# wangxiaohit/GNNPN-SC

Measured on AMD Instinct MI355X. Metric: service-composition problems/sec (ML+2PN inference), higher is better.
Workload: dtype f32-split3xf16 (f32 operands and results; recurrent W_hh.h products: fp32 operands split exactly into 3 x f16, six f16-matrix-core products per term, f32 accumulate; everything else f32 arithmetic)

## Files before the change

### gnnpn-sc_amd/_lib.py

```python
import ctypes
import os
from ctypes import c_char_p, c_double, c_float, c_int, c_int32, c_int64, c_uint32, c_void_p

import torch

_HERE = os.path.dirname(os.path.abspath(__file__))
LIB_PATH = os.environ.get("GNNPN_LIB") or os.path.join(_HERE, "libgnnpn_hip.so")
ABI_VERSION = 9

ACT_NONE, ACT_RELU, ACT_SIGMOID = 0, 1, 2
E_UNSUP = -2
WOA_OK, WOA_ROWS_MISMATCH, WOA_INDEX_ERROR, WOA_NO_SLOTS = 0, 1, 2, 3

_P = c_void_p
_SIGNATURES = {
    "gnnpn_abi_version": (c_int, []),
    "gnnpn_last_error": (c_char_p, []),
    "gnnpn_linear_f32": (c_int, [_P, c_int64, _P, c_int64, _P, _P, _P, c_int, _P, c_int64, c_int64, c_int, c_int, _P]),
    "gnnpn_embed_concat_f32": (c_int, [_P, _P, c_int, c_int, c_int, _P, c_int64, _P]),
    "gnnpn_csr_aggregate_f32": (c_int, [_P, _P, _P, _P, c_int64, _P, _P, _P, _P, c_int, _P, c_int64, c_int32,
                                        c_int32, _P]),
    "gnnpn_csr_aggregate_blocks_f32": (c_int, [_P, _P, _P, _P, c_int64, _P, _P, _P, _P, c_int, _P, c_int64, c_int32,
                                               c_int32, c_int32, _P, _P]),
    "gnnpn_csr_block_row_order": (c_int, [_P, c_int32, c_int32, _P, _P]),
    "gnnpn_csr_tile_plan_geometry": (c_int, [c_int32, c_int32, _P]),
    "gnnpn_csr_tile_plan_rows": (c_int, [_P, _P, _P, c_int32, c_int32, _P, _P, _P, _P, _P, _P]),
    "gnnpn_csr_tile_plan_fill": (c_int, [_P, _P, c_int32, c_int32, _P, _P, _P, _P, c_int64, _P]),
    "gnnpn_csr_aggregate_tiled_f32": (c_int, [_P, _P, _P, _P, _P, c_int64, _P, _P, _P, _P, c_int, _P, c_int64, c_int32, c_int32,
                                              c_int32, _P]),
    "gnnpn_gcn_norm_f32": (c_int, [_P, _P, _P, _P, _P, c_int32, _P]),
    "gnnpn_segment_mean_f32": (c_int, [_P, _P, c_int64, _P, c_int64, c_int32, c_int32, _P]),
    "gnnpn_gin_layer_f32": (c_int, [_P, _P, _P, c_int64, c_int32, _P, _P, _P, _P, _P, c_int32, _P, _P, _P, _P, c_int32, _P, _P, c_int32,
                                    _P, c_int64, c_int64, _P]),
    "gnnpn_split_weights_bytes": (c_int64, [c_int32, c_int32]),
    "gnnpn_lstm_split_weights_bytes": (c_int64, []),
    "gnnpn_lstm_pack_split_weights_f32": (c_int, [_P, _P, _P]),
    "gnnpn_pack_split_weights_f16": (c_int, [_P, c_int64, c_int32, c_int32, _P, _P, _P]),
    "gnnpn_gin_layer_split": (c_int, [_P, _P, _P, c_int64, c_int32, _P, _P, _P, _P, _P, _P, c_int32, _P, _P, _P, _P, _P, c_int32,
                                      _P, _P, _P, c_int32, _P, c_int64, c_int64, _P]),
    "gnnpn_request_branch_f32": (c_int, [_P, c_int32, _P, c_int32, c_int32, _P, _P, _P, c_int32, c_int32, c_int32, _P, c_int32,
                                         _P, _P, _P, _P]),
    "gnnpn_select_candidates": (c_int, [_P, c_int64, _P, _P, _P, _P, _P, _P, _P, c_int32, c_int32, c_int32, _P]),
    "gnnpn_rank_rows": (c_int, [_P, c_int64, _P, c_int32, c_int32, _P]),
    "gnnpn_precision_at_k": (c_int, [_P, c_int64, _P, c_int64, c_int32, c_int32, _P, c_int32, _P, _P]),
    "gnnpn_lstm_encode_f32": (c_int, [c_int, _P, c_int32, c_int32, c_int32, c_int32, c_int32, _P, _P, c_int64, _P]),
    "gnnpn_lstm_encode_workspace_bytes": (c_int64, []),
    "gnnpn_set_option": (c_int, [c_char_p, c_int]),
    "gnnpn_decode_diag": (c_int, [_P, c_int32, c_int32]),
    "gnnpn_coop_reset_staffing": (c_int, []),
    "gnnpn_last_launch_units": (c_int64, []),
    "gnnpn_lds_footprint_kb": (c_int, [c_int]),
    "gnnpn_coop_staffing_count": (c_int, []),
    "gnnpn_bn_train_forward_f32": (c_int, [_P, c_int64, c_int32, _P, _P, c_float, c_float, c_int, _P, _P, _P, _P, _P, _P]),
    "gnnpn_bn_train_backward_f32": (c_int, [_P, _P, _P, _P, _P, c_int64, c_int32, c_int, _P, _P, _P, _P]),
    "gnnpn_bce_sigmoid_f32": (c_int, [_P, _P, c_int64, _P, _P, _P]),
    "gnnpn_dot_f32": (c_int, [_P, _P, c_int64, _P, _P]),
    "gnnpn_embed_grad_f32": (c_int, [_P, c_int64, _P, c_int64, c_int64, c_int32, c_int32, _P, _P]),
    "gnnpn_pointer_decode_f32": (c_int, [c_int, _P, _P, c_float, c_int, c_int32, c_int32, c_int32, c_int32, c_int32,
                                         _P, _P, c_int64, _P]),
    "gnnpn_pointer_decode_workspace_bytes": (c_int64, [c_int32, c_int32, c_int32]),
    "gnnpn_pointer_decode_replicas_f32": (c_int, [_P, _P, c_float, c_int, c_int32, c_int32, c_int32, ctypes.c_uint64, c_int32, c_int32,
                                                  c_int32, _P, _P, c_int64, _P]),
    "gnnpn_replica_seed": (ctypes.c_uint64, [ctypes.c_uint64, c_int32]),
    "gnnpn_best_of_select_f32": (c_int, [c_int32, c_int32, c_int32, _P, _P, _P, _P, _P, _P, _P, _P, _P, _P, _P, _P, _P, _P]),
    "gnnpn_pointer_decode_attn_f32": (c_int, [_P, _P, _P, c_float, c_int, c_int32, c_int32, c_int32, c_int32, _P]),
    "gnnpn_attention_logits_f32": (c_int, [_P, _P, c_int64, _P, c_float, c_int, _P, c_int32, c_int32, c_int32,
                                           c_int32, c_int32, _P]),
    "gnnpn_attention_logits_bahdanau_f32": (c_int, [_P, _P, c_int64, _P, _P, c_float, c_int, _P, c_int32, c_int32, c_int32, c_int32, c_int32, _P]),
    "gnnpn_qos_reward_f32": (c_int, [_P, _P, c_int32, c_int32, c_int, _P]),
    "gnnpn_split3_pieces_f32": (c_int, [_P, c_int64, c_int32, _P, _P, _P, _P]),
    "gnnpn_recurrent_product_f32": (c_int, [_P, _P, c_int32, _P, _P, _P]),
    "gnnpn_gemm_f32": (c_int, [_P, c_int64, c_int, _P, c_int64, c_int, _P, c_int64, c_int64, c_int, c_int, c_int, _P]),
    "gnnpn_colsum_chunks_f32": (c_int, [_P, c_int64, c_int64, c_int32, c_int64, _P, _P]),
    "gnnpn_lstm_train_forward_f32": (c_int, [_P, _P, _P, _P, _P, _P, c_int32, c_int32, c_int32, _P]),
    "gnnpn_decode_train_forward_f32": (c_int, [_P, c_int32, c_int32, c_int32, c_int32, c_float, c_int, _P]),
    "gnnpn_decode_train_backward_f32": (c_int, [_P, _P, _P, _P, _P, _P, _P, c_int32, c_int32, c_int32, c_int32, c_float, c_int, _P]),
    "gnnpn_lstm_train_backward_f32": (c_int, [_P, _P, _P, _P, _P, _P, _P, c_int32, c_int32, c_int32, _P]),
    "gnnpn_decode_attn_train_forward_f32": (c_int, [_P, c_int32, c_int32, c_int32, c_int32, c_float, c_int, _P]),
    "gnnpn_decode_attn_train_backward_f32": (c_int, [_P, _P, _P, _P, _P, _P, _P, c_int32, c_int32, c_int32, c_int32, c_float, c_int, _P]),
    "gnnpn_colsum_f32": (c_int, [_P, c_int64, c_int64, c_int32, _P, _P]),
    "gnnpn_scatter_dx_f32": (c_int, [_P, _P, _P, c_int32, c_int32, c_int32, c_int32, _P]),
    "gnnpn_sumsq_f32": (c_int, [_P, c_int64, _P, _P]),
    "gnnpn_adam_step_f32": (c_int, [_P, _P, _P, _P, c_int64, _P, c_float, c_float, c_float, c_float, c_float, c_int32, _P]),
    "gnnpn_eswoa_f64": (c_int, [c_int32, c_int32, _P, _P, _P, _P, _P, c_int32, c_int32, _P, c_int32, _P, _P, _P, _P, _P]),
    "gnnpn_eswoa_wide_workspace_bytes": (c_int64, [c_int32, c_int32, c_int32]),
    "gnnpn_eswoa_wide_f64": (c_int, [c_int32, c_int32, _P, _P, _P, _P, _P, c_int32, c_int32, _P, _P, c_int64, _P, _P, _P, _P, _P]),
    "gnnpn_eswoa_ragged_workspace_bytes": (c_int64, [c_int32, c_int32, c_int32, c_int32]),
    "gnnpn_eswoa_ragged_f64": (c_int, [c_int32, _P, c_int32, c_int32, c_int32, _P, _P, _P, _P, _P, c_int32, c_int32, _P, c_int32, _P,
                                       c_int64, _P, _P, _P, _P, _P, _P]),
    "gnnpn_woa_candidates_workspace_bytes": (c_int64, [c_int32, c_int32, c_int32]),
    "gnnpn_woa_candidates_count": (c_int, [c_int32, c_int32, _P, c_int32, _P, _P, _P, c_int32, _P, _P, _P, c_int32, c_int32, c_double,
                                           _P, c_int32, c_int32, _P, c_int64, _P, _P, _P, _P, _P, _P]),
    "gnnpn_woa_candidates_fill": (c_int, [c_int32, c_int32, _P, _P, _P, c_int32, _P, c_int64, _P, _P, c_int32, c_int32, _P, _P, _P, _P,
                                          _P]),
    "gnnpn_debug_round5_f64": (c_int, [_P, _P, c_int64, _P]),
    "gnnpn_debug_cell_activations": (c_int, [_P, _P, _P, c_int64, _P]),
    "gnnpn_debug_lds_interferer": (c_int, [c_int32, c_int32, c_int32, _P]),
    "gnnpn_gate_wait": (c_int, [_P, c_uint32, c_int32, _P]),
    "gnnpn_debug_mfma_f16": (c_int, [_P, _P, _P, _P, _P]),
}
EXPORTS = tuple(_SIGNATURES)

class DecodeNet(ctypes.Structure):
    _fields_ = [(n, _P) for n in ("embedded", "enc_out", "h0", "c0", "start", "wih_packed", "whh_packed", "bih",
                                  "bhh", "latent_win", "emb_w", "emb_b", "xw_fold", "xb_fold", "start_fold", "idx", "win_logits", "pick_prob", "actions",
                                  "queries")] + \
               [("latent_from", c_int32), ("sample", c_int32), ("sample_seed", ctypes.c_uint64), ("whh_split", _P)]


class Attention(ctypes.Structure):
    _fields_ = [("attention", c_int32), ("n_glimpses", c_int32)] + \
               [(n, _P) for n in ("pointer_wq", "pointer_bq", "pointer_ref", "pointer_v", "glimpse_wq", "glimpse_bq",
                                  "glimpse_ref", "glimpse_v")]


class LaunchOpts(ctypes.Structure):
    _fields_ = [("impl", c_int32), ("lds_kb", c_int32), ("write_through", c_int32), ("paired_start", c_int32),
                ("sticky_status", _P)]


class TilePlanGeom(ctypes.Structure):
    _fields_ = [(n, c_int32) for n in ("n_blocks", "src_tiles", "src_tile_rows", "dst_tiles", "dst_tile_rows", "units", "wavefronts",
# ... 104 lines not shown
```

### gnnpn-sc_amd/build.py

```python
import os
import subprocess
import sys
from concurrent.futures import ThreadPoolExecutor

HERE = os.path.dirname(os.path.abspath(__file__))
ROOT = os.path.dirname(HERE)
CSRC = os.path.join(HERE, "csrc")
LIB = os.path.join(HERE, "libgnnpn_hip.so")
SOURCES = ["api.hip", "dense.hip", "graph.hip", "graph_tiled.hip", "gin_layer.hip", "gin_layer_split.hip", "request_branch.hip", "select.hip", "lstm.hip", "lstm_coop.hip", "decode.hip", "decode_coop.hip", "decode_lean.hip", "train.hip", "train_attn.hip", "train_ml.hip", "decode_glimpse.hip", "woa.hip", "woa_prep.hip", "split_probe.hip"]
HEADERS = [os.path.join(CSRC, "common.h"), os.path.join(CSRC, "graph_lds.h"), os.path.join(CSRC, "recurrent.h"), os.path.join(CSRC, "lstm_shared.h"), os.path.join(CSRC, "decode_shared.h"), os.path.join(CSRC, "coop_common.h"), os.path.join(CSRC, "train_common.h"),
           os.path.join(ROOT, "include", "gnnpn_hip.h")]
FLAGS = ["-O3", "--offload-arch=gfx950", "-ffp-contract=off", "-fPIC", "-std=c++17",
         "-I" + os.path.join(ROOT, "include"), "-I" + CSRC] + os.environ.get("GNNPN_EXTRA_HIPCC_FLAGS", "").split()


def _stale(target, deps):
    if not os.path.exists(target):
        return True
    t = os.path.getmtime(target)
    return any(os.path.getmtime(d) > t for d in deps)


def _compile(src):
    obj = os.path.join(HERE, "build", src.replace(".hip", ".o"))
    path = os.path.join(CSRC, src)
    if _stale(obj, [path] + HEADERS):
        subprocess.run(["hipcc"] + FLAGS + ["-c", path, "-o", obj], check=True)
    return obj


def _check_compiler():
    try:
        out = subprocess.run(["hipcc", "--version"], capture_output=True, text=True, check=True).stdout
    except (OSError, subprocess.CalledProcessError):
        return
    with open(os.path.join(HERE, "build", "compiler.txt"), "w") as f:
        f.write(out)


def build(force=False):
    os.makedirs(os.path.join(HERE, "build"), exist_ok=True)
    _check_compiler()
    if force:
        for f in os.listdir(os.path.join(HERE, "build")):
            if os.path.isfile(os.path.join(HERE, "build", f)):
                os.remove(os.path.join(HERE, "build", f))
    with ThreadPoolExecutor(max_workers=4) as ex:
        objs = list(ex.map(_compile, SOURCES))
    if force or _stale(LIB, objs):
        subprocess.run(["hipcc", "--offload-arch=gfx950", "-shared", "-fPIC", "-o", LIB] + objs, check=True)
    build_torch_ops(force)
    return LIB


TORCH_LIB = os.path.join(HERE, "libgnnpn_torch.so")


def build_torch_ops(force=False):
    src = os.path.join(CSRC, "torch_ops.cpp")
    if not (force or _stale(TORCH_LIB, [src, os.path.join(ROOT, "include", "gnnpn_hip.h"), LIB])):
        return TORCH_LIB
    import torch
    from torch.utils import cpp_extension
# ... 14 lines not shown
```

### gnnpn-sc_amd/csrc/decode.hip

```cpp
#include <atomic>

#include "common.h"
#include <string.h>
#include "recurrent.h"
#include "decode_shared.h"
#include "lstm_shared.h"

template <int H, int BT, bool REP = false>
__global__ __launch_bounds__((H < 64 ? 64 : H)) void pointer_decode_kernel(
    const float* __restrict__ embedded, const float* __restrict__ enc_out, const float* __restrict__ h0,
    const float* __restrict__ c0, const float* __restrict__ start, const float* __restrict__ wih,
    const float* __restrict__ whh, const float* __restrict__ bih, const float* __restrict__ bhh,
    const float* __restrict__ latent_win, const float* __restrict__ inputs, float tanh_c, int use_tanh,
    int32_t* __restrict__ idx_out, float* __restrict__ win_logits, float* __restrict__ pick_prob,
    float* __restrict__ actions, float* __restrict__ queries, int32_t B, int32_t T, int32_t n_per, int sample,
    unsigned long long sample_seed, int rep_R, int rep_first) {
    constexpr int NT = H < 64 ? 64 : H;
    constexpr int NW = NT / 64;
    __shared__ __attribute__((aligned(16))) float xs[BT][H];
    __shared__ __attribute__((aligned(16))) float hs[2][BT][H];
    __shared__ float lg[BT][64];
    __shared__ int sel[BT];

    const int j = threadIdx.x;
    const bool owner = j < H;
    const int lane = j & 63, wave = j >> 6;
    const int b0 = blockIdx.x * BT;
    const int L = T * n_per;
    const float4* __restrict__ Wi = reinterpret_cast<const float4*>(wih);
    const float4* __restrict__ Wh = reinterpret_cast<const float4*>(whh);
    auto prob_of = [rep_R](int b) { return REP ? b / rep_R : b; };

    float bi[4], bh[4], c[BT], h[BT];
#pragma unroll
    for (int g = 0; g < 4; ++g) {
        bi[g] = owner ? bih[g * H + j] : 0.0f;
        bh[g] = owner ? bhh[g * H + j] : 0.0f;
    }
#pragma unroll
    for (int p = 0; p < BT; ++p) {
        const bool ok = owner && (b0 + p < B);
        c[p] = ok ? c0[(int64_t)prob_of(b0 + p) * H + j] : 0.0f;
        h[p] = ok ? h0[(int64_t)prob_of(b0 + p) * H + j] : 0.0f;
        if (owner) {
            hs[0][p][j] = h[p];
            xs[p][j] = start[j];
        }
    }
    __syncthreads();

    int cur = 0;
    for (int k = 0; k < T; ++k) {
        if (owner) {
            float ai[BT][4], ah[BT][4];
#pragma unroll
            for (int p = 0; p < BT; ++p)
#pragma unroll
                for (int g = 0; g < 4; ++g) ai[p][g] = ah[p][g] = 0.0f;
// ... 38 lines not shown
        __syncthreads();

#pragma unroll
        for (int p = 0; p < BT; ++p) {
            if (b0 + p < B) {
                const int64_t row = (int64_t)prob_of(b0 + p) * L + sel[p];
                if (owner) xs[p][j] = embedded[row * H + j];
                if (j < 8) actions[((int64_t)(b0 + p) * T + k) * 8 + j] = inputs[row * 8 + j];
            }
        }
        __syncthreads();
    }
}

template <int H, bool REP = false>
static void launch_decode(const DecodeArgs& args, const DecodeNet& d, const float* latent, hipStream_t s,
                          ReplicaMap rep = ReplicaMap{0, 0}) {
    constexpr int NT = H < 64 ? 64 : H;
    const int32_t B = args.B;
    int bt = 1;
    while (bt < 4 && B / (bt * 2) >= 256) bt *= 2;
    dim3 grid((B + bt - 1) / bt), block(NT);
#define GNNPN_LAUNCH_DEC(BT_)                                                                                                    \
    hipLaunchKernelGGL((pointer_decode_kernel<H, BT_, REP>), grid, block, 0, s, d.embedded, d.enc_out, d.h0, d.c0, d.start, d.wih, \
                       d.whh, d.bih, d.bhh, latent, args.inputs, args.tanh_c, args.use_tanh, d.idx, d.win_logits, d.pick_prob,   \
                       d.actions, d.queries, B, args.T, args.K, d.sample, (unsigned long long)d.sample_seed, rep.R, rep.first)
    switch (bt) {
        case 1: GNNPN_LAUNCH_DEC(1); break;
        case 2: GNNPN_LAUNCH_DEC(2); break;
        default: GNNPN_LAUNCH_DEC(4); break;
    }
#undef GNNPN_LAUNCH_DEC
}

extern "C" int gnnpn_pointer_decode_f32(int n_nets, const gnnpn_decode_net_t* nets, const float* inputs,
                                        float tanh_c, int use_tanh, int32_t B, int32_t T, int32_t n_per, int32_t H,
                                        int32_t precision, const gnnpn_launch_opts_t* opts_in, void* workspace,
                                        int64_t workspace_bytes, void* stream) {
    g_gnnpn_last_units = 0;
    GNNPN_REQUIRE(B >= 0 && T > 0, "pointer_decode: bad shape");
    if (B == 0) return GNNPN_OK;
    GNNPN_REQUIRE(nets && inputs, "pointer_decode: null input");
    const CoopOpts opts = coop_opts(opts_in);
    GNNPN_REQUIRE(opts.impl >= 0 && opts.impl <= 4 && opts.impl != 3, "pointer_decode: opts.impl must be 0 (auto), 1 (streaming), 2 (cooperative, 8-CU groups) or 4 (8-CU groups, 256-register build) — the 16-CU-group form (3) was removed in ABI version 7");
    GNNPN_REQUIRE(opts.lds_kb >= 0 && opts.lds_kb <= 160, "pointer_decode: opts.lds_kb must be 0..160");
    GNNPN_REQUIRE(precision == GNNPN_PREC_F32 || precision == GNNPN_PREC_SPLIT, "pointer_decode: precision must be GNNPN_PREC_F32 or GNNPN_PREC_SPLIT, got %d", precision);
    GNNPN_REQUIRE(n_nets >= 1 && n_nets <= GNNPN_MAX_DECODE_NETS, "pointer_decode: n_nets must be 1..%d",
                  GNNPN_MAX_DECODE_NETS);
    GNNPN_REQUIRE(n_per >= 1 && n_per <= 64, "pointer_decode: n_per must be in [1,64], got %d", n_per);
    if (H != 256 && H != 32) GNNPN_FAIL(GNNPN_E_UNSUP, "pointer_decode: hidden size %d not built (256, 32)", H);
    DecodeArgs args{};
    for (int n = 0; n < n_nets; ++n) {
        const gnnpn_decode_net_t& d = nets[n];
        if (const int rc = decode_net_check(d, "pointer_decode", n)) return rc;
        GNNPN_REQUIRE(d.embedded || (d.emb_w && d.emb_b) || d.xw_fold,
                      "pointer_decode: net %d needs embedded, (emb_w, emb_b) or the folded input side", n);
        GNNPN_REQUIRE(d.latent_from < n && d.latent_from >= -1, "pointer_decode: latent_from of net %d must name an "
                      "earlier net of the call", n);
        GNNPN_REQUIRE(!(d.latent_win && d.latent_from >= 0), "pointer_decode: net %d has two latent sources", n);
        GNNPN_REQUIRE(!d.whh_split || gnnpn_aligned(d.whh_split, 16), "pointer_decode: whh_split must be 16-byte aligned");
        static_assert(sizeof(DecodeNet) == sizeof(gnnpn_decode_net_t), "layout");
        memcpy(&args.net[n], &d, sizeof(DecodeNet));
    }
    args.inputs = inputs;
    args.tanh_c = tanh_c;
    args.use_tanh = use_tanh;
    args.B = B;
    args.T = T;
    args.K = n_per;
    hipStream_t s = (hipStream_t)stream;
    bool any_sample = false;
    for (int n = 0; n < n_nets; ++n) any_sample |= nets[n].sample != 0;
    if (any_sample && (precision != GNNPN_PREC_F32 || opts.impl > 2))
        GNNPN_FAIL(GNNPN_E_UNSUP, "pointer_decode: sampling is built in the streaming and the 8-CU-group fp32 forms (impl 0-2, "
                   "GNNPN_PREC_F32)");
    const int impl = opts.impl;
    if (impl != 1 && gnnpn_decode_coop_supported(H, n_per) && (workspace != nullptr || impl >= 2)) {
        const int rc = gnnpn_launch_decode_coop(args, n_nets, precision, impl == 4, opts, workspace, workspace_bytes, s);
        const bool fall_through = rc == GNNPN_E_UNSUP && impl == 0 && precision == GNNPN_PREC_F32;
        if (rc != GNNPN_OK && !fall_through) return rc;
        if (fall_through) {
            static std::atomic<bool> said{false};
            if (!said.exchange(true))
                fprintf(stderr, "[gnnpn] pointer_decode: %s — taking the per-workgroup streaming form (about 10 x slower per step)\n", gnnpn_last_error());
        }
        if (rc == GNNPN_OK) {
            GNNPN_CHECK_LAUNCH("pointer_decode_f32(coop)");
            return GNNPN_OK;
        }
    }
    if (precision == GNNPN_PREC_SPLIT)
        GNNPN_FAIL(GNNPN_E_UNSUP, "pointer_decode: the split-operand precision needs the cooperative form (H = 256)");
    for (int n = 0; n < n_nets; ++n) {
        const DecodeNet& d = args.net[n];
        if (!d.embedded) GNNPN_FAIL(GNNPN_E_UNSUP, "pointer_decode: the streaming form needs the embedded tensor");
        const float* latent = d.latent_from >= 0 ? args.net[d.latent_from].win_logits : d.latent_win;
        GNNPN_FOR_H(H, launch_decode<HH>(args, d, latent, s));
    }
    GNNPN_CHECK_LAUNCH("pointer_decode_f32");
    return GNNPN_OK;
}

extern "C" uint64_t gnnpn_replica_seed(uint64_t seed, int32_t replica) {
    return replica_seed(seed, (unsigned long long)(long long)replica);
}

extern "C" int gnnpn_pointer_decode_replicas_f32(const gnnpn_decode_net_t* net, const float* inputs, float tanh_c, int use_tanh,
                                                 int32_t B, int32_t R, int32_t first, uint64_t seed, int32_t T, int32_t n_per,
                                                 int32_t H, const gnnpn_launch_opts_t* opts_in, void* workspace,
                                                 int64_t workspace_bytes, void* stream) {
    g_gnnpn_last_units = 0;
    GNNPN_REQUIRE(R >= 1, "pointer_decode_replicas: R must be >= 1, got %d", R);
    GNNPN_REQUIRE(first >= 0, "pointer_decode_replicas: first replica must be >= 0, got %d", first);
    GNNPN_REQUIRE(B >= 0 && T > 0 && n_per >= 1 && n_per <= 64, "pointer_decode_replicas: bad shape (B %d, T %d, n_per %d)", B, T, n_per);
    const int64_t rows = (int64_t)B * R;
    GNNPN_REQUIRE(rows <= (1 << 30), "pointer_decode_replicas: B*R = %lld rows exceed 2^30", (long long)rows);
    if (H != 256 && H != 32) GNNPN_FAIL(GNNPN_E_UNSUP, "pointer_decode_replicas: hidden size %d not built (256, 32)", H);
    if (B == 0) return GNNPN_OK;
    GNNPN_REQUIRE(net && inputs, "pointer_decode_replicas: null input");
    const CoopOpts opts = coop_opts(opts_in);
    GNNPN_REQUIRE(opts.impl >= 0 && opts.impl <= 2, "pointer_decode_replicas: opts.impl must be 0 (auto), 1 (streaming) or 2 (cooperative)");
    GNNPN_REQUIRE(opts.lds_kb >= 0 && opts.lds_kb <= 160, "pointer_decode_replicas: opts.lds_kb must be 0..160");
    const gnnpn_decode_net_t& d = *net;
    if (const int rc = decode_net_check(d, "pointer_decode_replicas", 0)) return rc;
    GNNPN_REQUIRE(d.embedded || d.xw_fold, "pointer_decode_replicas: the net needs embedded or the folded input side");
    GNNPN_REQUIRE(!d.queries, "pointer_decode_replicas: queries are not written (must be NULL)");
    GNNPN_REQUIRE(d.latent_from == -1, "pointer_decode_replicas: latent_from must be -1 (Low's window logits come from latent_win)");
    DecodeArgs args{};
    memcpy(&args.net[0], &d, sizeof(DecodeNet));
    args.net[0].sample = 1;
    args.net[0].sample_seed = seed;
    args.net[0].whh_split = nullptr;
// ... 62 lines not shown
    if (use_tanh) u = __fmul_rn(tanh_c, tanhf(u));
    if (lane == 0) logits[row] = u;
}

__global__ void mask_logits_kernel(const int32_t* __restrict__ masked_idx, float* __restrict__ logits, int32_t B,
                                   int32_t L, int32_t n_masked, int32_t ld_idx) {
    const int i = blockIdx.x * blockDim.x + threadIdx.x;
    if (i >= B * n_masked) return;
    const int b = i / n_masked, m = i - b * n_masked;
    const int pos = masked_idx[(int64_t)b * ld_idx + m];
    if (pos >= 0 && pos < L) logits[(int64_t)b * L + pos] = -INFINITY;
}

extern "C" int gnnpn_attention_logits_f32(const float* enc_out, const float* queries, int64_t ld_q,
                                          const int32_t* masked_idx, float tanh_c, int use_tanh, float* logits,
                                          int32_t B, int32_t L, int32_t H, int32_t n_masked, int32_t ld_idx,
                                          void* stream) {
    GNNPN_REQUIRE(B >= 0 && L > 0 && H > 0 && H % 4 == 0 && ld_q >= H && ld_q % 4 == 0, "attention_logits: bad shape");
    if (B == 0) return GNNPN_OK;
    GNNPN_REQUIRE(enc_out && queries && logits, "attention_logits: null operand");
    GNNPN_REQUIRE(n_masked == 0 || (masked_idx && ld_idx >= n_masked), "attention_logits: bad mask list");
    GNNPN_REQUIRE(gnnpn_aligned(enc_out, 16) && gnnpn_aligned(queries, 16), "attention_logits: 16-byte alignment");
    if (B == 0) return GNNPN_OK;
    hipStream_t s = (hipStream_t)stream;
    const int64_t n_rows = (int64_t)B * L;
    hipLaunchKernelGGL(attention_logits_kernel, dim3((unsigned)((n_rows + 3) / 4)), dim3(256), 0, s, enc_out, queries,
                       ld_q, tanh_c, use_tanh, logits, n_rows, L, H);
    if (n_masked > 0)
        hipLaunchKernelGGL(mask_logits_kernel, dim3((B * n_masked + 255) / 256), dim3(256), 0, s, masked_idx, logits,
                           B, L, n_masked, ld_idx);
    GNNPN_CHECK_LAUNCH("attention_logits_f32");
    return GNNPN_OK;
}

extern "C" int gnnpn_attention_logits_bahdanau_f32(const float* ref, const float* qp, int64_t ld_q, const float* v,
                                                   const int32_t* masked_idx, float tanh_c, int use_tanh, float* logits, int32_t B,
                                                   int32_t L, int32_t H, int32_t n_masked, int32_t ld_idx, void* stream) {
    GNNPN_REQUIRE(ref && qp && v && logits && B >= 0 && L > 0 && H > 0 && ld_q >= H, "attention_logits_bahdanau: bad argument");
    GNNPN_REQUIRE(n_masked == 0 || (masked_idx && ld_idx >= n_masked), "attention_logits_bahdanau: bad mask");
    if (B == 0) return GNNPN_OK;
    hipStream_t s = (hipStream_t)stream;
    const int64_t n_rows = (int64_t)B * L;
    hipLaunchKernelGGL(attention_logits_bahdanau_kernel, dim3((unsigned)((n_rows + 3) / 4)), dim3(256), 0, s, ref, qp, ld_q, v,
                       tanh_c, use_tanh, logits, n_rows, L, H);
    if (n_masked > 0)
        hipLaunchKernelGGL(mask_logits_kernel, dim3((B * n_masked + 255) / 256), dim3(256), 0, s, masked_idx, logits, B, L,
                           n_masked, ld_idx);
    GNNPN_CHECK_LAUNCH("attention_logits_bahdanau_f32");
    return GNNPN_OK;
}

__global__ __launch_bounds__(256) void qos_reward_kernel(const float* __restrict__ actions, float* __restrict__ R, int32_t B,
                                                        int32_t T, int level) {
    const int lane = threadIdx.x & 63;
    const int b = blockIdx.x * 4 + (threadIdx.x >> 6);
    if (b >= B) return;
    const float* a = actions + (int64_t)b * T * 8;
    const float lo0 = a[4], hi0 = a[5], lo1 = a[6], hi1 = a[7];
    float prod2 = 1.0f, prod3 = 1.0f, mn = INFINITY;
    double sum0 = 0.0;
    int n_real = 0;
    auto fetch = [&](int t) { return *reinterpret_cast<const float4*>(a + (int64_t)min(t, T - 1) * 8); };
    auto consume = [&](float4 q, int t0) {
        if (t0 + lane >= T) q = make_float4(0.0f, INFINITY, 1.0f, 1.0f);
        n_real += q.x > 0.0f;
        mn = fminf(mn, q.y);
        const double xd = (double)q.x;
        const int lo = __double2loint(xd), hi = __double2hiint(xd);
        const int zi = __float_as_int(q.z), wi = __float_as_int(q.w);
        const int cnt = min(64, T - t0);
#define GNNPN_REWARD_STEP(i)                                                                                      \
    prod2 = __fmul_rn(prod2, __int_as_float(__builtin_amdgcn_readlane(zi, i)));                                   \
    prod3 = __fmul_rn(prod3, __int_as_float(__builtin_amdgcn_readlane(wi, i)));                                   \
    sum0 += __hiloint2double(__builtin_amdgcn_readlane(hi, i), __builtin_amdgcn_readlane(lo, i));
        if (cnt == 64) {
#pragma unroll
            for (int i = 0; i < 64; ++i) { GNNPN_REWARD_STEP(i) }
        } else {
            for (int i = 0; i < cnt; ++i) { GNNPN_REWARD_STEP(i) }
        }
#undef GNNPN_REWARD_STEP
    };
    float4 qa = fetch(lane), qb;
    for (int t0 = 0; t0 < T; t0 += 128) {
        qb = fetch(t0 + 64 + lane);
        consume(qa, t0);
        if (t0 + 64 >= T) break;
        qa = fetch(t0 + 128 + lane);
        consume(qb, t0 + 64);
    }
#pragma unroll
    for (int off = 32; off > 0; off >>= 1) {
        n_real += __shfl_xor(n_real, off, 64);
        mn = fminf(mn, __shfl_xor(mn, off, 64));
    }
    if (lane != 0) return;
    int violate = 0;
    if (prod2 < lo0 || prod2 > hi0) ++violate;
    if (prod3 < lo1 || prod3 > hi1) ++violate;
    if (level == 0) {
        R[b] = (float)violate;
        return;
    }
    float obj = (float)sum0 / (float)n_real;
    obj = __fadd_rn(obj, 1.0f);
    obj = __fsub_rn(obj, mn);
    obj = obj / 2.0f;
    const double v = (double)violate + (double)obj;
    R[b] = (float)(rint(v * 1e5) / 1e5);
}

extern "C" int gnnpn_qos_reward_f32(const float* actions, float* R, int32_t B, int32_t T, int level,
                                    void* stream) {
    GNNPN_REQUIRE(B >= 0 && T > 0 && (level == 0 || level == 1), "qos_reward: bad argument");
    if (B == 0) return GNNPN_OK;
    GNNPN_REQUIRE(actions && R, "qos_reward: null operand");
    hipLaunchKernelGGL(qos_reward_kernel, dim3((B + 3) / 4), dim3(256), 0, (hipStream_t)stream, actions, R, B, T,
                       level);
    GNNPN_CHECK_LAUNCH("qos_reward_f32");
    return GNNPN_OK;
}

__global__ __launch_bounds__(256) void best_of_select_kernel(int32_t B, int32_t N, int32_t T, const float* __restrict__ R0,
                                                             const int32_t* __restrict__ idx0, const float* __restrict__ act0,
                                                             const float* __restrict__ prob0, const float* __restrict__ Rs,
                                                             const int32_t* __restrict__ idxs, const float* __restrict__ acts,
                                                             const float* __restrict__ probs, float* __restrict__ R_out,
                                                             int32_t* __restrict__ idx_out, float* __restrict__ act_out,
                                                             float* __restrict__ prob_out, int32_t* __restrict__ winner) {
    const int lane = threadIdx.x & 63;
    const int b = blockIdx.x * 4 + (threadIdx.x >> 6);
    if (b >= B) return;
    const int S = N - 1;
    unsigned long long best = ~0ull;
    for (int j = lane; j < N; j += 64) {
        float r = j == 0 ? R0[b] : Rs[(int64_t)b * S + (j - 1)];
        if (r == 0.0f) r = 0.0f;
        const unsigned hi = r != r ? 0xFFFFFFFFu : float_order_key(r);
        const unsigned long long key = ((unsigned long long)hi << 32) | (unsigned)j;
        best = key < best ? key : best;
    }
#pragma unroll
    for (int off = 32; off > 0; off >>= 1) {
        const unsigned lo = __shfl_xor((unsigned)(best & 0xffffffffu), off, 64);
        const unsigned hi = __shfl_xor((unsigned)(best >> 32), off, 64);
        const unsigned long long o = ((unsigned long long)hi << 32) | lo;
        best = o < best ? o : best;
    }
    const int w = (int)(best & 0xffffffffu);
    const int64_t src = w == 0 ? (int64_t)b : (int64_t)b * S + (w - 1);
    const int32_t* si = (w == 0 ? idx0 : idxs) + src * T;
    const float* sp = (w == 0 ? prob0 : probs) + src * T;
    const float* sa = (w == 0 ? act0 : acts) + src * T * 8;
    for (int t = lane; t < T; t += 64) {
        idx_out[(int64_t)b * T + t] = si[t];
        prob_out[(int64_t)b * T + t] = sp[t];
    }
    for (int i = lane; i < T * 8; i += 64) act_out[(int64_t)b * T * 8 + i] = sa[i];
    if (lane == 0) {
        winner[b] = w;
        R_out[b] = w == 0 ? R0[b] : Rs[src];
    }
// ... 17 lines not shown
```

### gnnpn-sc_amd/csrc/decode_lean.hip

```cpp
#include "common.h"
#include "recurrent.h"
#include "decode_shared.h"
#include "coop_common.h"
#include "lstm_shared.h"

namespace {
constexpr int H = COOP_H;
constexpr int G = COOP_G;
constexpr int ROWS = COOP_ROWS;
constexpr int UNITS = H / G;
constexpr int KW = 16;
constexpr unsigned SPIN_LIMIT = 400000;
constexpr int XP_GRANULES = ROWS * KW * G;

typedef unsigned u32x2 __attribute__((ext_vector_type(2)));
constexpr int AUX_SC1 = 16;


__device__ __forceinline__ __amdgpu_buffer_rsrc_t make_rsrc(const void* p, unsigned bytes) {
    return __builtin_amdgcn_make_buffer_rsrc(const_cast<void*>(p), 0, (int)bytes, 0x00020000);
}
__device__ __forceinline__ float dpp_ror(float v, int n) {
    switch (n) {
        case 1: return __int_as_float(__builtin_amdgcn_update_dpp(0, __float_as_int(v), 0x121, 0xF, 0xF, true));
        case 2: return __int_as_float(__builtin_amdgcn_update_dpp(0, __float_as_int(v), 0x122, 0xF, 0xF, true));
        case 4: return __int_as_float(__builtin_amdgcn_update_dpp(0, __float_as_int(v), 0x124, 0xF, 0xF, true));
        default: return __int_as_float(__builtin_amdgcn_update_dpp(0, __float_as_int(v), 0x128, 0xF, 0xF, true));
    }
}
__device__ __forceinline__ void store_granule(__amdgpu_buffer_rsrc_t r, unsigned voff, unsigned soff, u64 g, bool same_xcd) {
    const u32x2 v = {(unsigned)g, (unsigned)(g >> 32)};
    if (same_xcd) __builtin_amdgcn_raw_buffer_store_b64(v, r, voff, soff, 0);
    else __builtin_amdgcn_raw_buffer_store_b64(v, r, voff, soff, AUX_SC1);
}
__device__ __forceinline__ void record_failure(unsigned* diag, const unsigned* err, int group, int member, int tile, int k, int wave,
                                               unsigned tag, unsigned h_miss, unsigned p_miss, unsigned l_miss, int gpx) {
    if ((threadIdx.x & 63) != 0 || !diag) return;
    const unsigned n = atomicAdd(diag, 1u);
    if (n >= 31) return;
    unsigned* rec = diag + 16 * (n + 1);
    const unsigned* cnt = err + COOP_XCDCNT_OFFSET / 4;
    unsigned c0 = 0, c1 = 0;
    for (int x = 0; x < 4; ++x) {
        c0 |= (cnt[COOP_XCD_STRIDE * x] & 0xffu) << (8 * x);
        c1 |= (cnt[COOP_XCD_STRIDE * (4 + x)] & 0xffu) << (8 * x);
    }
    const unsigned long long t = __builtin_amdgcn_s_memrealtime();
    rec[0] = group; rec[1] = member; rec[2] = tile; rec[3] = k; rec[4] = wave; rec[5] = tag;
    rec[6] = h_miss; rec[7] = p_miss; rec[8] = l_miss; rec[9] = c0; rec[10] = c1;
    rec[11] = (unsigned)t; rec[12] = (unsigned)(t >> 32); rec[13] = gpx; rec[14] = blockIdx.x; rec[15] = err[0];
}
}

template <bool SPLIT, int OCC, int EVH, bool DIAG = false>
__global__ __launch_bounds__(256, OCC) void pointer_decode_lean_kernel(DecodeArgs a, u64* xh, u64* xp,
// ... 328 lines not shown
                    __builtin_amdgcn_raw_buffer_store_b32(__float_as_uint(hl.x), r_q, vo_q, (unsigned)k * (H * 4), 0);
                    __builtin_amdgcn_raw_buffer_store_b32(__float_as_uint(hl.y), r_q, vo_q, (unsigned)(k + T) * (H * 4), 0);
                }
            }
            if constexpr (DIAG) {
                asm volatile("" ::"v"(hl.y));
                st[6] = phase_stamp();
            }
            __syncthreads();
            {
                float p = 0.0f;
                if (pdot) {
#pragma unroll
                    for (int j = 0; j < EVN; ++j) {
                        const float4 hv = *reinterpret_cast<const float4*>(&hsl[prow][phalf * (4 * EVN) + 4 * j]);
                        p = fmaf(__uint_as_float(ev[j].x), hv.x, p);
                        p = fmaf(__uint_as_float(ev[j].y), hv.y, p);
                        p = fmaf(__uint_as_float(ev[j].z), hv.z, p);
                        p = fmaf(__uint_as_float(ev[j].w), hv.w, p);
                    }
                }
                if constexpr (EVH == 2)
                    p = __fadd_rn(p, __int_as_float(__builtin_amdgcn_update_dpp(0, __float_as_int(p), 0xB1 , 0xF, 0xF, false)));
                if (pdot && phalf == 0)
                    store_granule(r_p, vo_ppub, (step & 1) * (XP_GRANULES * 8), ((u64)(step + 1) << 32) | __float_as_uint(p), same_xcd);
            }
            if (wr_live) {
                *reinterpret_cast<u32x4*>(&win[wr_row][wr_cand][0]) = wv0;
                *reinterpret_cast<u32x4*>(&win[wr_row][wr_cand][4]) = wv1;
            }
            if constexpr (DIAG) {
                st[7] = phase_stamp();
                if (blockIdx.x == 0 && tid == 0 && k > 0) {
                    u64* prof = reinterpret_cast<u64*>(err) + 4;
                    prof[0] += st[1] - st[0];
                    prof[1] += st[2] - st[1];
                    prof[2] += st[3] - st[2];
                    prof[3] += st[4] - st[3];
                    prof[4] += st[5] - st[4];
                    prof[5] += st[6] - st[5];
                    prof[6] += st[7] - st[6];
                    prof[7] += 1;
                }
            }
            ++step;
        }
        if (abort_flag) break;
        ++tiles_done;
    }
    if (tid == 0) {
        if (abort_flag) coop_raise(err, sticky, 2u, seats);
        coop_note_finished(sticky, GNNPN_STATUS_DEC_FINISHED, tiles_done);
    }
}

struct PickProbArgs {
    const float* win[2];
    const float* lat[2];
    const int32_t* idx[2];
    float* out[2];
};
__global__ __launch_bounds__(256) void pick_prob_kernel(PickProbArgs a, int64_t rows, int T, int K) {
    const int net = blockIdx.y;
    const float* __restrict__ win = a.win[net];
    const float* __restrict__ lat = a.lat[net];
    const int32_t* __restrict__ idx = a.idx[net];
    float* __restrict__ out = a.out[net];
    const int64_t row = blockIdx.x * 256ll + threadIdx.x;
    if (row >= rows) return;
    const unsigned t_base = (unsigned)__builtin_amdgcn_readfirstlane((int)((blockIdx.x * 256ll) % T));
    const int t = (int)((t_base + threadIdx.x) % (unsigned)T);
    float v[16];
#pragma unroll
    for (int j = 0; j < 16; ++j) {
        v[j] = 0.0f;
        if (j < K) {
            v[j] = win[row * K + j];
            if (lat) v[j] = __fadd_rn(v[j], lat[row * K + j]);
        }
    }
    const int pick_r = min(max(idx[row] - t * K, 0), 15);
    float best = v[0];
#pragma unroll
    for (int j = 1; j < 16; ++j) best = j == pick_r ? v[j] : best;
#pragma unroll
    for (int j = 0; j < 16; ++j) v[j] = j < K ? expf(__fsub_rn(v[j], best)) : 0.0f;
#pragma unroll
    for (int n = 8; n >= 1; n >>= 1)
#pragma unroll
        for (int j = 0; j < n; ++j) v[j] = __fadd_rn(v[j], v[j + n]);
    out[row] = 1.0f / v[0];
}

static DecodeWorkspace lean_workspace(int64_t groups, int64_t rows, int32_t T, int32_t K) {
    return decode_workspace(groups, rows, T, K, XP_GRANULES);
}

int64_t gnnpn_decode_lean_workspace_bytes(int32_t B, int32_t T, int32_t n_per) { return lean_workspace(64, B, T, n_per).total(); }

int gnnpn_launch_decode_lean(const DecodeArgs& args, int n_nets, int precision, bool shared_cu, const CoopOpts& opts,
                             void* workspace, int64_t workspace_bytes, hipStream_t s) {
    if (args.K > KW) GNNPN_FAIL(GNNPN_E_UNSUP, "pointer_decode: the cooperative form is built for n_per <= %d", KW);
    if ((int64_t)ROWS * args.T * args.K * H * 4 >= (1ll << 32) || (int64_t)args.T * ROWS * args.K * 8 >= (1ll << 32))
        GNNPN_FAIL(GNNPN_E_UNSUP, "pointer_decode: a tile of 16 problems must stay below 4 GB of encoder output");
    const bool split = precision == GNNPN_PREC_SPLIT;
    const bool wide = args.K > 8;
    const bool stamps = (gnnpn_option_lstm_ablate() & 0x800) != 0;
    if (stamps && wide) GNNPN_FAIL(GNNPN_E_UNSUP, "pointer_decode: the stamped build exists for n_per <= 8");
    CoopLaunch c;
    const auto need = [&](int groups) { return lean_workspace(groups, args.B, args.T, args.K).total(); };
    if (const int rc = coop_begin("pointer_decode", n_nets, args.B, need, GNNPN_STATUS_DEC_EXPECTED, opts, workspace, workspace_bytes, s, c))
        return rc;
    const DecodeWorkspace w = lean_workspace(c.groups, args.B, args.T, args.K);
    u64* p_h = reinterpret_cast<u64*>(c.buffers);
    u64* p_p = reinterpret_cast<u64*>(c.buffers + w.h_bytes);
    u64* p_l = reinterpret_cast<u64*>(c.buffers + w.h_bytes + w.p_bytes);
    static unsigned* p_diag = gnnpn_decode_diag_buffer();
    const int wt = (opts.write_through ? 1 : 0) | (opts.paired_start ? 2 : 0);
#define GNNPN_LEAN(SPLIT_, OCC_, EVH_, ...)                                                                                           \
    hipLaunchKernelGGL((pointer_decode_lean_kernel<SPLIT_, OCC_, EVH_, ##__VA_ARGS__>), dim3(COOP_OVERSUB * c.groups * G), dim3(256),       \
                       gnnpn_lds_padding((const void*)pointer_decode_lean_kernel<SPLIT_, OCC_, EVH_, ##__VA_ARGS__>, opts.lds_kb), s, args, \
                       p_h, p_p, p_l, c.status, opts.sticky, n_nets, c.groups_per_net, c.gpx, wt, c.seats, p_diag)
    if (stamps) {
        if (split) GNNPN_LEAN(true, 1, 2, true);
        else GNNPN_LEAN(false, 1, 2, true);
    } else if (split && shared_cu && wide) GNNPN_LEAN(true, 2, 1);
    else if (split && shared_cu) GNNPN_LEAN(true, 2, 2);
    else if (split && wide) GNNPN_LEAN(true, 1, 1);
    else if (split) GNNPN_LEAN(true, 1, 2);
    else if (shared_cu && wide) GNNPN_LEAN(false, 2, 1);
    else if (shared_cu) GNNPN_LEAN(false, 2, 2);
    else if (wide) GNNPN_LEAN(false, 1, 1);
    else GNNPN_LEAN(false, 1, 2);
#undef GNNPN_LEAN
    if (hipGetLastError() != hipSuccess) GNNPN_FAIL(GNNPN_E_LAUNCH, "pointer_decode: launch of the cooperative kernel failed");
    const int64_t rows = (int64_t)args.B * args.T;
    for (int n0 = 0; n0 < n_nets; n0 += 2) {
        PickProbArgs pa = {};
        const int cnt = n_nets - n0 < 2 ? n_nets - n0 : 2;
        for (int n = 0; n < cnt; ++n) {
            const DecodeNet& d = args.net[n0 + n];
            pa.win[n] = d.win_logits;
            pa.lat[n] = d.latent_from >= 0 ? args.net[d.latent_from].win_logits : d.latent_win;
            pa.idx[n] = d.idx;
            pa.out[n] = d.pick_prob;
        }
        hipLaunchKernelGGL(pick_prob_kernel, dim3((unsigned)((rows + 255) / 256), (unsigned)cnt), dim3(256), 0, s, pa, rows, args.T, args.K);
    }
    return GNNPN_OK;
}
```

### gnnpn-sc_amd/csrc/decode_shared.h

```cpp
#pragma once
#include "common.h"
#include "lstm_shared.h"

struct DecodeNet {
    const float* embedded;
    const float* enc_out;
    const float* h0;
    const float* c0;
    const float* start;
    const float* wih;
    const float* whh;
    const float* bih;
    const float* bhh;
    const float* latent_win;
    const float* emb_w;
    const float* emb_b;
    const float* xw_fold;
    const float* xb_fold;
    const float* start_fold;
    int32_t* idx;
    float* win_logits;
    float* pick_prob;
    float* actions;
    float* queries;
    int32_t latent_from;
    int32_t sample;
    uint64_t sample_seed;
    const void* whh_split;
};
static_assert(sizeof(DecodeNet) == sizeof(gnnpn_decode_net_t), "DecodeNet must mirror gnnpn_decode_net_t");

inline int decode_net_check(const gnnpn_decode_net_t& d, const char* who, int n) {
    GNNPN_REQUIRE(d.enc_out && d.h0 && d.c0 && d.start && d.wih_packed && d.whh_packed && d.bih && d.bhh,
                  "%s: null input of net %d (enc_out, h0, c0, start and the decoder weights are required)", who, n);
    GNNPN_REQUIRE(d.idx && d.win_logits && d.pick_prob && d.actions, "%s: null output of net %d", who, n);
    GNNPN_REQUIRE((d.xw_fold != nullptr) == (d.xb_fold != nullptr) && (d.xw_fold != nullptr) == (d.start_fold != nullptr),
                  "%s: net %d: xw_fold, xb_fold and start_fold go together", who, n);
    GNNPN_REQUIRE(d.sample == 0 || d.sample == 1, "%s: net %d: sample must be 0 (greedy) or 1 (multinomial)", who, n);
    GNNPN_REQUIRE(gnnpn_aligned(d.wih_packed, 16) && gnnpn_aligned(d.whh_packed, 16) && gnnpn_aligned(d.enc_out, 16) &&
                      (!d.embedded || gnnpn_aligned(d.embedded, 16)),
                  "%s: weights / enc_out / embedded must be 16-byte aligned", who);
    return GNNPN_OK;
}

template <int H>
__device__ __forceinline__ float lane_dot4(const float* __restrict__ row, const float* q) {
    float part = 0.0f;
    for (int e = (threadIdx.x & 63) * 4; e < H; e += 256) {
        const float4 rv = *reinterpret_cast<const float4*>(row + e);
        const float4 qv = *reinterpret_cast<const float4*>(q + e);
        part = fmaf(rv.x, qv.x, part);
        part = fmaf(rv.y, qv.y, part);
        part = fmaf(rv.z, qv.z, part);
        part = fmaf(rv.w, qv.w, part);
    }
    return part;
}

__device__ __forceinline__ int window_pick(float* lg, int K, float tanh_c, int use_tanh, float* __restrict__ win_logits, int64_t wbase,
                                           const float* __restrict__ latent_win, int64_t lbase, int sample, unsigned long long seed,
                                           unsigned long long ctr, float& prob) {
    float best = 0.0f;
    int best_r = -1;
    for (int r = 0; r < K; ++r) {
        float v = lg[r];
        if (use_tanh) v = __fmul_rn(tanh_c, tanhf(v));
        win_logits[wbase + r] = v;
        if (latent_win) v = __fadd_rn(v, latent_win[lbase + r]);
        lg[r] = v;
        if (best_r < 0 || v > best) {
            best = v;
            best_r = r;
        }
    }
    float denom = 0.0f;
    for (int r = 0; r < K; ++r) denom = __fadd_rn(denom, expf(__fsub_rn(lg[r], best)));
    prob = 1.0f / denom;
    if (sample) {
        const float u = stream_uniform24(seed, ctr);
        float cdf = 0.0f;
        int pick = -1, last_pos = 0;
        for (int r = 0; r < K; ++r) {
            const float pr = expf(__fsub_rn(lg[r], best)) / denom;
            cdf = __fadd_rn(cdf, pr);
            if (pr > 0.0f) last_pos = r;
            if (pick < 0 && u < cdf) pick = r;
        }
        if (pick < 0) pick = last_pos;
// ... 30 lines not shown
```

### gnnpn-sc_amd/csrc/dense.hip

```cpp
#include "common.h"

typedef float f32x16 __attribute__((ext_vector_type(16)));

template <int BM, int BN>
struct DenseCfg {
    static constexpr int BK = 32;
    static constexpr int LDA = BM + 1;
    static constexpr int LDB = BN + 1;
    static constexpr int A_F4 = BM * BK / 4 / 256;
    static constexpr int B_F4 = BN * BK / 4 / 256;
    static constexpr int TM = BM / 64;
    static constexpr int TN = BN / 64;
};

struct __attribute__((packed, aligned(4))) f4_align4 { float v[4]; };

template <int NF4>
__device__ __forceinline__ void tile_load(const float* __restrict__ P, int64_t ld, int64_t r0,
                                          int64_t n_rows, int k0, int K, bool vec_ok, float4 (&reg)[NF4]) {
#pragma unroll
    for (int i = 0; i < NF4; ++i) {
        int f = threadIdx.x + i * 256;
        int r = f >> 3, kc = f & 7;
        int64_t row = r0 + r;
        int k = k0 + kc * 4;
        float4 v = make_float4(0.f, 0.f, 0.f, 0.f);
        if (row < n_rows) {
            const float* src = P + row * ld + k;
            if (vec_ok && k + 3 < K) {
                const f4_align4 t = *reinterpret_cast<const f4_align4*>(src);
                v = make_float4(t.v[0], t.v[1], t.v[2], t.v[3]);
            } else {
                if (k + 0 < K) v.x = src[0];
                if (k + 1 < K) v.y = src[1];
                if (k + 2 < K) v.z = src[2];
                if (k + 3 < K) v.w = src[3];
            }
        }
        reg[i] = v;
    }
}

template <int NF4, int LD>
__device__ __forceinline__ void tile_store(float* S, const float4 (&reg)[NF4]) {
#pragma unroll
    for (int i = 0; i < NF4; ++i) {
        int f = threadIdx.x + i * 256;
        int r = f >> 3, kc = f & 7;
        S[(kc * 4 + 0) * LD + r] = reg[i].x;
        S[(kc * 4 + 1) * LD + r] = reg[i].y;
        S[(kc * 4 + 2) * LD + r] = reg[i].z;
        S[(kc * 4 + 3) * LD + r] = reg[i].w;
    }
}

template <int BM, int BN>
__global__ __launch_bounds__(256) void linear_f32_kernel(
    const float* __restrict__ A, int64_t lda, const float* __restrict__ W, int64_t ldw,
    const float* __restrict__ bias, const float* __restrict__ scale, const float* __restrict__ shift,
    int act, float* __restrict__ C, int64_t ldc, int64_t M, int N, int K, int vec_a, int vec_w) {
    using Cfg = DenseCfg<BM, BN>;
    __shared__ float As[Cfg::BK * Cfg::LDA];
    __shared__ float Bs[Cfg::BK * Cfg::LDB];

    const int wave = threadIdx.x >> 6, lane = threadIdx.x & 63;
    const int wm = wave >> 1, wn = wave & 1;
    const int64_t m0 = (int64_t)blockIdx.y * BM;
    const int n0 = blockIdx.x * BN;

    f32x16 acc[Cfg::TM][Cfg::TN];
#pragma unroll
    for (int i = 0; i < Cfg::TM; ++i)
#pragma unroll
        for (int j = 0; j < Cfg::TN; ++j)
#pragma unroll
            for (int r = 0; r < 16; ++r) acc[i][j][r] = 0.0f;

    float4 ra[Cfg::A_F4], rb[Cfg::B_F4];
    tile_load<Cfg::A_F4>(A, lda, m0, M, 0, K, vec_a, ra);
    tile_load<Cfg::B_F4>(W, ldw, n0, N, 0, K, vec_w, rb);

    const int half = lane >> 5, l32 = lane & 31;
    for (int k0 = 0; k0 < K; k0 += Cfg::BK) {
        tile_store<Cfg::A_F4, Cfg::LDA>(As, ra);
        tile_store<Cfg::B_F4, Cfg::LDB>(Bs, rb);
        __syncthreads();
        if (k0 + Cfg::BK < K) {
            tile_load<Cfg::A_F4>(A, lda, m0, M, k0 + Cfg::BK, K, vec_a, ra);
            tile_load<Cfg::B_F4>(W, ldw, n0, N, k0 + Cfg::BK, K, vec_w, rb);
        }
#pragma unroll
        for (int kk = 0; kk < Cfg::BK; kk += 2) {
            float a[Cfg::TM], b[Cfg::TN];
#pragma unroll
            for (int i = 0; i < Cfg::TM; ++i)
                a[i] = As[(kk + half) * Cfg::LDA + wm * (BM / 2) + i * 32 + l32];
#pragma unroll
            for (int j = 0; j < Cfg::TN; ++j)
                b[j] = Bs[(kk + half) * Cfg::LDB + wn * (BN / 2) + j * 32 + l32];
#pragma unroll
            for (int i = 0; i < Cfg::TM; ++i)
#pragma unroll
                for (int j = 0; j < Cfg::TN; ++j)
                    acc[i][j] = __builtin_amdgcn_mfma_f32_32x32x2f32(a[i], b[j], acc[i][j], 0, 0, 0);
        }
        __syncthreads();
    }
// ... 165 lines not shown
```

### gnnpn-sc_amd/csrc/select.hip

```cpp
#include <vector>

#include "common.h"

__device__ __forceinline__ unsigned long long rank_key(float score, uint32_t id) {
    return ((unsigned long long)float_order_key(score) << 32) | (0xffffffffu - id);
}

__global__ __launch_bounds__(256) void select_candidates_kernel(
    const float* __restrict__ scores, int64_t ld_scores, const int32_t* __restrict__ cat_ptr,
    const double* __restrict__ qos, const double* __restrict__ local_bounds, const uint8_t* __restrict__ present,
    const double* __restrict__ global_bounds, float* __restrict__ out_rows, int32_t* __restrict__ out_ids,
    int32_t B, int32_t T, int32_t n_per) {
    const int lane = threadIdx.x & 63;
    const int64_t seg = (int64_t)blockIdx.x * 4 + (threadIdx.x >> 6);
    if (seg >= (int64_t)B * T) return;
    const int b = (int)(seg / T), c = (int)(seg - (int64_t)b * T);
    const int s_begin = cat_ptr[c], s_end = cat_ptr[c + 1];
    const bool pres = present[seg] != 0;
    const double* lb = local_bounds + seg * 4;
    const double lo_c = lb[0], hi_c = lb[1], lo_q = lb[2], hi_q = lb[3];
    const float* srow = scores + (int64_t)b * ld_scores;

    unsigned long long last = ~0ull;
    int my_pick = -1;
    int n_found = 0;
    if (pres) {
        for (int r = 0; r < n_per; ++r) {
            unsigned long long best = 0ull;
            for (int s = s_begin + lane; s < s_end; s += 64) {
                const double cost = qos[(int64_t)s * 4 + 2], qual = qos[(int64_t)s * 4 + 3];
                const bool feas = lo_c <= cost && cost <= hi_c && lo_q <= qual && qual <= hi_q;
                const unsigned long long key = rank_key(srow[s], (uint32_t)s);
                if (feas && key < last && key > best) best = key;
            }
            best = wave_max_u64(best);
            if (best == 0ull) break;
            if (lane == r) my_pick = (int)(0xffffffffu - (uint32_t)(best & 0xffffffffu));
            last = best;
            ++n_found;
        }
    }
    const int src_lane = n_found > 0 ? lane % n_found : 0;
    const int id = __shfl(my_pick, src_lane, 64);
    if (lane < n_per) {
        const int64_t pos = (int64_t)b * T * n_per + (int64_t)c * n_per + lane;
        float4 q, tail = make_float4(0.f, 0.f, 0.f, 0.f);
        if (n_found > 0) {
            const double* qs = qos + (int64_t)id * 4;
            q = make_float4((float)qs[0], (float)qs[1], (float)qs[2], (float)qs[3]);
        } else {
            q = make_float4(0.f, 1.f, 1.f, 1.f);
        }
        if (c == 0) {
            const double* g = global_bounds + (int64_t)b * 4;
            tail = make_float4((float)g[0], (float)g[1], (float)g[2], (float)g[3]);
        }
        float4* dst = reinterpret_cast<float4*>(out_rows + pos * 8);
        dst[0] = q;
        dst[1] = tail;
        out_ids[pos] = n_found > 0 ? id : -1;
    }
}

__device__ __forceinline__ unsigned long long row16_max_u64(unsigned long long v) {
#define GNNPN_MAX_STEP(CTRL)                                                                                       \
    {                                                                                                              \
        const unsigned lo = __builtin_amdgcn_update_dpp(0, (int)(unsigned)v, CTRL, 0xF, 0xF, true);                \
        const unsigned hi = __builtin_amdgcn_update_dpp(0, (int)(unsigned)(v >> 32), CTRL, 0xF, 0xF, true);        \
        const unsigned long long o = ((unsigned long long)hi << 32) | lo;                                          \
        v = o > v ? o : v;                                                                                         \
    }
    GNNPN_MAX_STEP(0x121) GNNPN_MAX_STEP(0x122) GNNPN_MAX_STEP(0x124) GNNPN_MAX_STEP(0x128)
    return v;
}
__device__ __forceinline__ unsigned long long row8_max_u64(unsigned long long v) {
    GNNPN_MAX_STEP(0xB1) GNNPN_MAX_STEP(0x4E) GNNPN_MAX_STEP(0x141)
    return v;
#undef GNNPN_MAX_STEP
}

template <int W>
__global__ __launch_bounds__(256) void select_candidates16_kernel(
    const float* __restrict__ scores, int64_t ld_scores, const int32_t* __restrict__ cat_ptr,
    const double* __restrict__ qos, const double* __restrict__ local_bounds, const uint8_t* __restrict__ present,
    const double* __restrict__ global_bounds, float* __restrict__ out_rows, int32_t* __restrict__ out_ids,
    int32_t B, int32_t T, int32_t n_per) {
    const int lane = threadIdx.x & 63, sub = lane & (W - 1);
    const int64_t seg = ((int64_t)blockIdx.x * 4 + (threadIdx.x >> 6)) * (64 / W) + lane / W;
    if (seg >= (int64_t)B * T) return;
    const int b = (int64_t)B * T <= 0x7fffffffll ? (int)((unsigned)seg / (unsigned)T) : (int)(seg / T);
    const int c = (int)(seg - (int64_t)b * T);
    const int s_begin = cat_ptr[c], s_end = cat_ptr[c + 1];
    const bool pres = present[seg] != 0;
    const double* lb = local_bounds + seg * 4;
    const double lo_c = lb[0], hi_c = lb[1], lo_q = lb[2], hi_q = lb[3];
    const float* srow = scores + (int64_t)b * ld_scores;

    auto group_max = [](unsigned long long v) { return W == 16 ? row16_max_u64(v) : row8_max_u64(v); };
    unsigned long long last = ~0ull;
    int my_pick = -1;
    int n_found = 0;
    const bool small = s_end - s_begin <= W;
    float4 own = make_float4(0.f, 1.f, 1.f, 1.f);
    if (pres && small) {
        unsigned long long key = 0ull;
        const int s = s_begin + sub;
        if (s < s_end) {
            const double* qs = qos + (int64_t)s * 4;
            const double q0 = qs[0], q1 = qs[1], cost = qs[2], qual = qs[3];
            own = make_float4((float)q0, (float)q1, (float)cost, (float)qual);
            if (lo_c <= cost && cost <= hi_c && lo_q <= qual && qual <= hi_q) key = rank_key(srow[s], (uint32_t)s);
        }
        for (int r = 0; r < n_per; ++r) {
            const unsigned long long best = group_max(key < last ? key : 0ull);
            if (best == 0ull) break;
            if (sub == r) my_pick = (int)(0xffffffffu - (uint32_t)(best & 0xffffffffu));
            last = best;
            ++n_found;
        }
    } else if (pres) {
        for (int r = 0; r < n_per; ++r) {
            unsigned long long best = 0ull;
            for (int s = s_begin + sub; s < s_end; s += W) {
                const double cost = qos[(int64_t)s * 4 + 2], qual = qos[(int64_t)s * 4 + 3];
                const bool feas = lo_c <= cost && cost <= hi_c && lo_q <= qual && qual <= hi_q;
                const unsigned long long key = rank_key(srow[s], (uint32_t)s);
                if (feas && key < last && key > best) best = key;
            }
            best = group_max(best);
            if (best == 0ull) break;
            if (sub == r) my_pick = (int)(0xffffffffu - (uint32_t)(best & 0xffffffffu));
            last = best;
            ++n_found;
        }
    }
    const int src_lane = (lane & ~(W - 1)) + (n_found > 0 ? sub % n_found : 0);
    const int id = __shfl(my_pick, src_lane, 64);
    float4 q = make_float4(0.f, 1.f, 1.f, 1.f);
    if (small) {
        const int owner = n_found > 0 ? (lane & ~(W - 1)) + (id - s_begin) : lane;
        const float4 g = make_float4(__shfl(own.x, owner, 64), __shfl(own.y, owner, 64), __shfl(own.z, owner, 64), __shfl(own.w, owner, 64));
        if (n_found > 0) q = g;
    } else if (n_found > 0 && sub < n_per) {
        const double* qs = qos + (int64_t)id * 4;
        q = make_float4((float)qs[0], (float)qs[1], (float)qs[2], (float)qs[3]);
    }
    if (sub < n_per) {
        const int64_t pos = (int64_t)b * T * n_per + (int64_t)c * n_per + sub;
        float4 tail = make_float4(0.f, 0.f, 0.f, 0.f);
        if (c == 0) {
            const double* g = global_bounds + (int64_t)b * 4;
            tail = make_float4((float)g[0], (float)g[1], (float)g[2], (float)g[3]);
        }
        float4* dst = reinterpret_cast<float4*>(out_rows + pos * 8);
        dst[0] = q;
        dst[1] = tail;
        out_ids[pos] = n_found > 0 ? id : -1;
    }
}

extern "C" int gnnpn_select_candidates(const float* scores, int64_t ld_scores, const int32_t* cat_ptr,
                                       const double* qos, const double* local_bounds, const uint8_t* present,
                                       const double* global_bounds, float* out_rows, int32_t* out_ids, int32_t B,
                                       int32_t T, int32_t n_per, void* stream) {
    GNNPN_REQUIRE(B >= 0 && T > 0, "select_candidates: bad shape");
    if (B == 0) return GNNPN_OK;
    GNNPN_REQUIRE(scores && cat_ptr && qos && local_bounds && present && global_bounds && out_rows && out_ids,
                  "select_candidates: null operand");
    GNNPN_REQUIRE(n_per >= 1 && n_per <= 64, "select_candidates: n_per must be in [1,64], got %d", n_per);
    GNNPN_REQUIRE(gnnpn_aligned(out_rows, 16), "select_candidates: out_rows must be 16-byte aligned");
    if (B == 0) return GNNPN_OK;
    const int64_t n_seg = (int64_t)B * T;
    if (n_per <= 8 && ld_scores <= 8ll * T)
        hipLaunchKernelGGL(select_candidates16_kernel<8>, dim3((unsigned)((n_seg + 31) / 32)), dim3(256), 0,
                           (hipStream_t)stream, scores, ld_scores, cat_ptr, qos, local_bounds, present, global_bounds,
                           out_rows, out_ids, B, T, n_per);
    else if (n_per <= 16)
        hipLaunchKernelGGL(select_candidates16_kernel<16>, dim3((unsigned)((n_seg + 15) / 16)), dim3(256), 0,
                           (hipStream_t)stream, scores, ld_scores, cat_ptr, qos, local_bounds, present, global_bounds,
                           out_rows, out_ids, B, T, n_per);
    else
        hipLaunchKernelGGL(select_candidates_kernel, dim3((unsigned)((n_seg + 3) / 4)), dim3(256), 0,
                           (hipStream_t)stream, scores, ld_scores, cat_ptr, qos, local_bounds, present, global_bounds,
                           out_rows, out_ids, B, T, n_per);
    GNNPN_CHECK_LAUNCH("select_candidates");
    return GNNPN_OK;
}

__global__ __launch_bounds__(1024) void rank_rows_kernel(const float* __restrict__ scores, int64_t ld_scores,
                                                         int32_t* __restrict__ ranking, int32_t S, int32_t P) {
    extern __shared__ __attribute__((aligned(16))) unsigned long long keys[];
    const float* srow = scores + (int64_t)blockIdx.x * ld_scores;
    for (int i = threadIdx.x; i < P; i += blockDim.x) keys[i] = i < S ? rank_key(srow[i], (uint32_t)i) : 0ull;
    __syncthreads();
    for (int k = 2; k <= P; k <<= 1) {
        for (int j = k >> 1; j > 0; j >>= 1) {
            for (int t = threadIdx.x; t < (P >> 1); t += blockDim.x) {
                const int i = 2 * t - (t & (j - 1));
                const int p = i + j;
                const bool desc = (i & k) == 0;
                const unsigned long long a = keys[i], b = keys[p];
                if ((a < b) == desc) {
                    keys[i] = b;
                    keys[p] = a;
                }
            }
            __syncthreads();
        }
    }
    int32_t* out = ranking + (int64_t)blockIdx.x * S;
    for (int i = threadIdx.x; i < S; i += blockDim.x) out[i] = (int32_t)(0xffffffffu - (uint32_t)(keys[i] & 0xffffffffu));
}

__global__ __launch_bounds__(1024) void rank_rows_indirect_kernel(const float* __restrict__ scores, int64_t ld_scores,
                                                                  int32_t* __restrict__ ranking, int32_t S, int32_t P) {
    extern __shared__ __attribute__((aligned(16))) unsigned int ids[];
    const float* srow = scores + (int64_t)blockIdx.x * ld_scores;
    auto key_of = [&](unsigned int i) { return i < (unsigned)S ? rank_key(srow[i], i) : 0ull; };
    for (int i = threadIdx.x; i < P; i += blockDim.x) ids[i] = (unsigned)i;
    __syncthreads();
    for (int k = 2; k <= P; k <<= 1) {
        for (int j = k >> 1; j > 0; j >>= 1) {
            for (int t = threadIdx.x; t < (P >> 1); t += blockDim.x) {
                const int i = 2 * t - (t & (j - 1));
                const int p = i + j;
                const bool desc = (i & k) == 0;
                const unsigned int ia = ids[i], ib = ids[p];
                if ((key_of(ia) < key_of(ib)) == desc) {
                    ids[i] = ib;
                    ids[p] = ia;
                }
            }
            __syncthreads();
        }
    }
    int32_t* out = ranking + (int64_t)blockIdx.x * S;
    for (int i = threadIdx.x; i < S; i += blockDim.x) out[i] = (int32_t)ids[i];
}
// ... 66 lines not shown
```

### gnnpn-sc_amd/csrc/torch_ops.cpp

```cpp
#include <ATen/ATen.h>
#include <c10/core/DeviceGuard.h>
#include <c10/hip/HIPStream.h>
#include <torch/library.h>

#include <string>
#include <vector>

#include "gnnpn_hip.h"

namespace {

using at::Tensor;
using OptTensor = std::optional<Tensor>;

#define GNNPN_ON_DEVICE_OF(t)                          \
    TORCH_CHECK((t).is_cuda(), "gnnpn: expected a CUDA tensor (the hot path has no CPU implementation)"); \
    const c10::DeviceGuard device_guard_((t).device()); \
    void* const stream_ = (void*)c10::hip::getCurrentHIPStream((t).device().index()).stream()
#define cur_stream() stream_

void check_rc(int rc, const char* what) { TORCH_CHECK(rc == GNNPN_OK, what, " failed (", rc, "): ", gnnpn_last_error()); }

template <typename T>
const T* cptr(const Tensor& t, at::ScalarType dt, const char* name) {
// ... 129 lines not shown
                 const OptTensor& w3, const OptTensor& b3) {
    GNNPN_ON_DEVICE_OF(x);
    rows2d(x, "gin_layer.x");
    const int64_t n = x.size(0), c_in = x.size(1);
    const bool lin3 = w3.has_value() && w3->defined();
    TORCH_CHECK(w1.dim() == 3 && w2.dim() == 3 && (!lin3 || w3->dim() == 3) && w1.size(1) * 2 == (c_in + 31) / 32 * 32,
                "gin_layer: weights must be packed with ops.pack_mfma_b32 (and w1 for this many input channels)");
    const int64_t h1 = w1.size(0) * 32, h2 = w2.size(0) * 32, h3 = lin3 ? w3->size(0) * 32 : 0;
    Tensor out = new_f32(x, {n, lin3 ? h3 : h2});
    check_rc(gnnpn_gin_layer_f32(i32(rowptr, "rowptr"), i32(col, "col"), f32(x, "x"), c_in, (int32_t)c_in, f32(eps, "eps"), f32(w1, "w1"),
                                 f32(b1, "b1"), f32(a1, "a1"), f32(s1, "s1"), (int32_t)h1, f32(w2, "w2"), f32(b2, "b2"), f32(a2, "a2"),
                                 f32(s2, "s2"), (int32_t)h2, f32(w3, "w3"), f32(b3, "b3"), (int32_t)h3, out_f32(out), out.size(1), n,
                                 cur_stream()), "gnnpn_gin_layer_f32");
    return out;
}

Tensor gin_layer_split(const Tensor& rowptr, const Tensor& col, const Tensor& x, const Tensor& eps, const Tensor& w1, const Tensor& i1,
                       const OptTensor& b1, const OptTensor& a1, const OptTensor& s1, const Tensor& w2, const Tensor& i2, const OptTensor& b2,
                       const OptTensor& a2, const OptTensor& s2, const OptTensor& w3, const OptTensor& i3, const OptTensor& b3) {
    GNNPN_ON_DEVICE_OF(x);
    rows2d(x, "gin_layer_split.x");
    const int64_t n = x.size(0), c_in = x.size(1), k1 = (c_in + 31) / 32 * 32;
    const bool lin3 = w3.has_value() && w3->defined();
    const int64_t h1 = i1.numel(), h2 = i2.numel(), h3 = lin3 ? (i3.has_value() ? i3->numel() : 0) : 0;
    TORCH_CHECK(w1.numel() == gnnpn_split_weights_bytes((int32_t)h1, (int32_t)k1) && w2.numel() == gnnpn_split_weights_bytes((int32_t)h2, (int32_t)h1) &&
                    (!lin3 || w3->numel() == gnnpn_split_weights_bytes((int32_t)h3, (int32_t)h2)),
                "gin_layer_split: packed weights do not chain (c_in -> h1 -> h2 [-> h3]); pack with ops.pack_split_weights");
    Tensor out = new_f32(x, {n, lin3 ? h3 : h2});
    check_rc(gnnpn_gin_layer_split(i32(rowptr, "rowptr"), i32(col, "col"), f32(x, "x"), c_in, (int32_t)c_in, f32(eps, "eps"),
                                   cptr<uint8_t>(w1, at::kByte, "w1"), f32(i1, "i1"), f32(b1, "b1"), f32(a1, "a1"), f32(s1, "s1"), (int32_t)h1,
                                   cptr<uint8_t>(w2, at::kByte, "w2"), f32(i2, "i2"), f32(b2, "b2"), f32(a2, "a2"), f32(s2, "s2"), (int32_t)h2,
                                   cptr<uint8_t>(w3, at::kByte, "w3"), f32(i3, "i3"), f32(b3, "b3"), (int32_t)h3, out_f32(out), out.size(1), n,
                                   cur_stream()), "gnnpn_gin_layer_split");
    return out;
}

std::tuple<Tensor, Tensor> segment_topk_feasible(const Tensor& scores, const Tensor& cat_ptr, const Tensor& qos, const Tensor& local_bounds,
                                                 const Tensor& present, const Tensor& global_bounds, int64_t n_per) {
    GNNPN_ON_DEVICE_OF(scores);
    rows2d(scores, "select.scores");
    const int64_t B = scores.size(0), S = scores.size(1), T = cat_ptr.numel() - 1;
    TORCH_CHECK(qos.sizes() == at::IntArrayRef({S, 4}) && local_bounds.sizes() == at::IntArrayRef({B, T, 4}) &&
                    present.sizes() == at::IntArrayRef({B, T}) && global_bounds.sizes() == at::IntArrayRef({B, 4}),
                "select_candidates: inconsistent shapes");
    Tensor rows = new_f32(scores, {B, T * n_per, 8}), ids = new_i32(scores, {B, T * n_per});
    check_rc(gnnpn_select_candidates(f32(scores, "scores"), S, i32(cat_ptr, "cat_ptr"), cptr<double>(qos, at::kDouble, "qos"),
                                     cptr<double>(local_bounds, at::kDouble, "local_bounds"), cptr<uint8_t>(present, at::kByte, "present"),
                                     cptr<double>(global_bounds, at::kDouble, "global_bounds"), out_f32(rows),
                                     static_cast<int32_t*>(ids.data_ptr()), (int32_t)B, (int32_t)T, (int32_t)n_per, cur_stream()),
             "gnnpn_select_candidates");
    return {rows, ids};
}

Tensor rank_rows(const Tensor& scores) {
    GNNPN_ON_DEVICE_OF(scores);
    rows2d(scores, "rank_rows.scores");
    const int64_t B = scores.size(0), S = scores.size(1);
    Tensor ranking = new_i32(scores, {B, S});
    check_rc(gnnpn_rank_rows(f32(scores, "scores"), S, static_cast<int32_t*>(ranking.data_ptr()), (int32_t)B, (int32_t)S, cur_stream()),
             "gnnpn_rank_rows");
    return ranking;
}

Tensor precision_at_k(const Tensor& ranking, const Tensor& labels, at::IntArrayRef ks) {
    GNNPN_ON_DEVICE_OF(labels);
    const int64_t B = labels.size(0), S = labels.size(1);
    std::vector<int32_t> k32(ks.begin(), ks.end());
    Tensor kt = at::tensor(k32, at::TensorOptions().dtype(at::kInt)).to(labels.device());
    Tensor out = new_f32(labels, {B, (int64_t)ks.size()});
    check_rc(gnnpn_precision_at_k(i32(ranking, "ranking"), ranking.size(1), f32(labels, "labels"), S, (int32_t)B, (int32_t)S, i32(kt, "ks"),
                                  (int32_t)ks.size(), out_f32(out), cur_stream()), "gnnpn_precision_at_k");
    return out;
}

Tensor attention_logits(const Tensor& enc_out, const Tensor& queries, int64_t step, const Tensor& idx, double tanh_c, bool use_tanh) {
    GNNPN_ON_DEVICE_OF(enc_out);
    const int64_t B = enc_out.size(0), L = enc_out.size(1), H = enc_out.size(2), T = queries.size(1);
    f32(enc_out, "enc_out"), f32(queries, "queries");
    Tensor out = new_f32(enc_out, {B, L});
    check_rc(gnnpn_attention_logits_f32(f32(enc_out, "enc_out"), static_cast<const float*>(queries.data_ptr()) + step * H, T * H,
                                        i32(idx, "idx"), (float)tanh_c, use_tanh ? 1 : 0, out_f32(out), (int32_t)B, (int32_t)L, (int32_t)H,
                                        (int32_t)step, (int32_t)T, cur_stream()), "gnnpn_attention_logits_f32");
    return out;
}

Tensor qos_reward(const Tensor& actions, int64_t level) {
    GNNPN_ON_DEVICE_OF(actions);
    const int64_t B = actions.size(0), T = actions.size(1);
    Tensor R = new_f32(actions, {B});
    check_rc(gnnpn_qos_reward_f32(f32(actions, "actions"), out_f32(R), (int32_t)B, (int32_t)T, (int)level, cur_stream()), "gnnpn_qos_reward_f32");
    return R;
}

int precision_code(const std::string& p, const char* what) {
    if (p == "f32") return GNNPN_PREC_F32;
    if (p == "f16") return GNNPN_PREC_F16;
    if (p == "split") return GNNPN_PREC_SPLIT;
    TORCH_CHECK(false, what, ": unknown precision '", p, "'");
}
bool coop_supported(int64_t H, int64_t n_per, int64_t impl) { return H == 256 && n_per <= 16 && impl != 1; }
gnnpn_launch_opts_t launch_opts(int64_t impl, int64_t lds_kb, bool write_through, bool paired_start, const OptTensor& status) {
    gnnpn_launch_opts_t o{};
    o.impl = (int32_t)impl, o.lds_kb = (int32_t)lds_kb, o.write_through = write_through ? 1 : 0, o.paired_start = paired_start ? 1 : 0;
    TORCH_CHECK(!(status.has_value() && status->defined()) || status->numel() >= GNNPN_STATUS_WORDS,
                "status: a block of ", GNNPN_STATUS_WORDS, " int32 words (ops.Workspaces.status)");
    o.sticky_status = (status.has_value() && status->defined())
                          ? const_cast<uint32_t*>(reinterpret_cast<const uint32_t*>(cptr<int32_t>(*status, at::kInt, "status")))
                          : nullptr;
    return o;
}

std::vector<Tensor> lstm_encode(const c10::List<OptTensor>& net_tensors, int64_t n_nets, std::string precision, int64_t impl, int64_t lds_kb,
                                bool write_through, const OptTensor& workspace, const OptTensor& status, bool paired_start) {
    constexpr size_t EK = 7;
    TORCH_CHECK(n_nets >= 1 && net_tensors.size() == EK * (size_t)n_nets, "lstm_encode: seven tensors per net (custom_ops.ENCODE_KEYS)");
    std::vector<OptTensor> t(net_tensors.size());
    for (size_t i = 0; i < t.size(); ++i) t[i] = net_tensors.get(i);
    auto has = [&](size_t i) { return t[i].has_value() && t[i]->defined(); };
    TORCH_CHECK(has(5), "lstm_encode: nets[0].bhh required");
    GNNPN_ON_DEVICE_OF(*t[5]);
    const int64_t H = t[5]->numel() / 4;
    const Tensor& first = has(0) ? *t[0] : *t[1];
    TORCH_CHECK(first.dim() == 3, "lstm_encode: pregates / inputs must be [B, L, .]");
    const int64_t B = first.size(0), L = first.size(1);
    const bool coop = coop_supported(H, 1, impl);
    const int prec = precision_code(precision, "lstm_encode");
    TORCH_CHECK(prec == GNNPN_PREC_F32 || coop, "lstm_encode: precision='", precision, "' needs the cooperative form (H = 256)");
    std::vector<gnnpn_encode_net_t> nets(n_nets);
    std::vector<Tensor> enc, hn, cn, keep;
    for (int64_t i = 0; i < n_nets; ++i)
        if (has(EK * i + 6) && has(EK * i + 4)) lstm_split(*t[EK * i + 6], *t[EK * i + 4], "nets.whh_split");
    for (int64_t i = 0; i < n_nets; ++i) {
        const size_t o = EK * i;
        Tensor pre = has(o) ? *t[o] : Tensor();
        if (!pre.defined() && !coop) {
            TORCH_CHECK(has(o + 1) && has(o + 2) && has(o + 3), "lstm_encode: nets[", i, "] needs pregates or inputs + w_in + b_in");
            const Tensor& x = *t[o + 1];
            pre = linear(x.reshape({B * L, x.size(2)}), *t[o + 2], t[o + 3], std::nullopt, std::nullopt, 0).view({B, L, 4 * H});
            keep.push_back(pre);
        }
        enc.push_back(new_f32(first, {B, L, H})), hn.push_back(new_f32(first, {B, H})), cn.push_back(new_f32(first, {B, H}));
        gnnpn_encode_net_t& a = nets[i];
        a = gnnpn_encode_net_t{};
        a.pregates = pre.defined() ? f32(pre, "nets.pregates") : nullptr;
        if (!pre.defined()) {
            TORCH_CHECK(has(o + 1) && has(o + 2) && has(o + 3), "lstm_encode: nets[", i, "] needs pregates or inputs + w_in + b_in");
            a.inputs = f32(*t[o + 1], "nets.inputs"), a.w_in = f32(*t[o + 2], "nets.w_in"), a.b_in = f32(*t[o + 3], "nets.b_in");
        }
        TORCH_CHECK(has(o + 4) && has(o + 5), "lstm_encode: nets[", i, "].whh / bhh required");
        a.whh_packed = f32(*t[o + 4], "nets.whh"), a.bhh = f32(*t[o + 5], "nets.bhh");
        a.whh_split = has(o + 6) ? lstm_split(*t[o + 6], *t[o + 4], "nets.whh_split") : nullptr;
        a.enc_out = out_f32(enc.back()), a.h_n = out_f32(hn.back()), a.c_n = out_f32(cn.back());
    }
    const bool ws = coop && workspace.has_value() && workspace->defined();
    TORCH_CHECK(!coop || ws, "lstm_encode: the cooperative form (H = 256) needs a workspace (ops.Workspaces.encode())");
    const gnnpn_launch_opts_t opts = launch_opts(impl, lds_kb, write_through, paired_start, coop ? status : OptTensor());
    check_rc(gnnpn_lstm_encode_f32((int)n_nets, nets.data(), (int32_t)B, (int32_t)L, (int32_t)H, 8, prec, &opts,
                                   ws ? const_cast<uint8_t*>(cptr<uint8_t>(*workspace, at::kByte, "workspace")) : nullptr,
                                   ws ? workspace->numel() : 0, cur_stream()), "gnnpn_lstm_encode_f32");
    std::vector<Tensor> out;
    out.insert(out.end(), enc.begin(), enc.end()), out.insert(out.end(), hn.begin(), hn.end()), out.insert(out.end(), cn.begin(), cn.end());
    return out;
}

std::vector<Tensor> pointer_decode(const c10::List<OptTensor>& net_tensors, at::IntArrayRef latent_from, const Tensor& inputs, int64_t n_cat,
                                   int64_t n_per, double tanh_c, bool use_tanh, bool want_queries, std::string precision, int64_t impl,
                                   int64_t lds_kb, bool write_through, const OptTensor& workspace, const OptTensor& status,
                                   at::IntArrayRef sample_seeds, bool paired_start) {
    GNNPN_ON_DEVICE_OF(inputs);
    constexpr size_t NK = 16;
    const size_t n_nets = latent_from.size();
    TORCH_CHECK(n_nets >= 1 && n_nets <= 2 && net_tensors.size() == NK * n_nets, "pointer_decode: sixteen tensors per net (custom_ops.DECODE_KEYS), 1 or 2 nets");
    std::vector<OptTensor> t(net_tensors.size());
    for (size_t i = 0; i < t.size(); ++i) t[i] = net_tensors.get(i);
    auto has = [&](size_t i) { return t[i].has_value() && t[i]->defined(); };
    TORCH_CHECK(has(0) && t[0]->dim() == 3, "pointer_decode: nets[0].enc_out [B, L, H] required");
    const int64_t B = t[0]->size(0), L = t[0]->size(1), H = t[0]->size(2);
    const int prec = precision_code(precision, "pointer_decode");
    TORCH_CHECK(L == n_cat * n_per, "pointer_decode: seq_len ", L, " != ", n_cat, "*", n_per);
    const bool coop = coop_supported(H, n_per, impl);
    for (size_t i = 0; i < n_nets; ++i)
        if (has(NK * i + 15) && has(NK * i + 5)) lstm_split(*t[NK * i + 15], *t[NK * i + 5], "whh_split");
    std::vector<gnnpn_decode_net_t> nets(n_nets);
    std::vector<Tensor> out, keep;
    for (size_t i = 0; i < n_nets; ++i) {
        const size_t o = NK * i;
        gnnpn_decode_net_t& a = nets[i];
        a = gnnpn_decode_net_t{};
        for (size_t j = 0; j < 8; ++j) TORCH_CHECK(has(o + j), "pointer_decode: nets[", i, "] operand ", j, " required");
        a.enc_out = f32(*t[o + 0], "enc_out"), a.h0 = f32(*t[o + 1], "h0"), a.c0 = f32(*t[o + 2], "c0"), a.start = f32(*t[o + 3], "start");
        a.wih_packed = f32(*t[o + 4], "wih"), a.whh_packed = f32(*t[o + 5], "whh"), a.bih = f32(*t[o + 6], "bih"), a.bhh = f32(*t[o + 7], "bhh");
        if (has(o + 11) && coop) {
            TORCH_CHECK(has(o + 12) && has(o + 13), "pointer_decode: xw_fold needs xb_fold and start_fold");
            a.xw_fold = f32(*t[o + 11], "xw_fold"), a.xb_fold = f32(*t[o + 12], "xb_fold"), a.start_fold = f32(*t[o + 13], "start_fold");
        }
        Tensor emb = has(o + 8) ? *t[o + 8] : Tensor();
        if (!emb.defined() && !coop) {
            TORCH_CHECK(has(o + 9) && has(o + 10), "pointer_decode: nets[", i, "] needs embedded or emb_w + emb_b");
            emb = linear(inputs.reshape({B * L, inputs.size(2)}), *t[o + 9], t[o + 10], std::nullopt, std::nullopt, 0).view({B, L, H});
            keep.push_back(emb);
        }
        a.embedded = emb.defined() ? f32(emb, "embedded") : nullptr;
        if (!emb.defined()) {
            TORCH_CHECK(has(o + 9) && has(o + 10), "pointer_decode: nets[", i, "] needs embedded or emb_w + emb_b");
            a.emb_w = f32(*t[o + 9], "emb_w"), a.emb_b = f32(*t[o + 10], "emb_b");
        }
        a.latent_win = has(o + 14) ? f32(*t[o + 14], "latent_win") : nullptr;
        a.whh_split = has(o + 15) ? lstm_split(*t[o + 15], *t[o + 5], "whh_split") : nullptr;
        a.latent_from = (int32_t)latent_from[i];
        const int64_t seed = i < sample_seeds.size() ? sample_seeds[i] : -1;
        a.sample = seed >= 0 ? 1 : 0;
        a.sample_seed = seed >= 0 ? (uint64_t)seed : 0;
        Tensor idx = new_i32(inputs, {B, n_cat}), win = new_f32(inputs, {B, n_cat, n_per}), prob = new_f32(inputs, {B, n_cat});
        Tensor actions = new_f32(inputs, {B, n_cat, 8}), q = want_queries ? new_f32(inputs, {B, n_cat, H}) : new_f32(inputs, {0});
        a.idx = static_cast<int32_t*>(idx.data_ptr()), a.win_logits = out_f32(win), a.pick_prob = out_f32(prob), a.actions = out_f32(actions);
        a.queries = want_queries ? out_f32(q) : nullptr;
        out.push_back(idx), out.push_back(win), out.push_back(prob), out.push_back(actions), out.push_back(q);
    }
    const bool ws = coop && workspace.has_value() && workspace->defined();
    TORCH_CHECK(!coop || ws, "pointer_decode: the cooperative form needs a workspace (ops.Workspaces.decode(B, T, n_per))");
    const gnnpn_launch_opts_t opts = launch_opts(impl, lds_kb, write_through, paired_start, coop ? status : OptTensor());
    check_rc(gnnpn_pointer_decode_f32((int)n_nets, nets.data(), f32(inputs, "inputs"), (float)tanh_c, use_tanh ? 1 : 0, (int32_t)B, (int32_t)n_cat,
                                      (int32_t)n_per, (int32_t)H, prec == GNNPN_PREC_SPLIT ? GNNPN_PREC_SPLIT : GNNPN_PREC_F32, &opts,
                                      ws ? const_cast<uint8_t*>(cptr<uint8_t>(*workspace, at::kByte, "workspace")) : nullptr,
                                      ws ? workspace->numel() : 0, cur_stream()), "gnnpn_pointer_decode_f32");
    return out;
}

}

TORCH_LIBRARY(gnnpn, m) {
    m.def("linear(Tensor a, Tensor weight, Tensor? bias=None, Tensor? scale=None, Tensor? shift=None, int act=0) -> Tensor");
    m.def("embed_concat(Tensor x, Tensor table) -> Tensor");
    m.def("csr_aggregate(Tensor rowptr, Tensor col, Tensor? w, Tensor x, Tensor? self_coef=None, Tensor? bias=None, Tensor? scale=None, "
          "Tensor? shift=None, int act=0) -> Tensor");
    m.def("csr_aggregate_blocks(Tensor rowptr, Tensor col, Tensor? w, Tensor x, Tensor? self_coef, Tensor? bias, Tensor? scale, "
          "Tensor? shift, int act, int block_rows, Tensor? row_order=None) -> Tensor");
    m.def("csr_aggregate_tiled(Tensor header, Tensor order, Tensor selfw, Tensor batches, Tensor x, Tensor? self_coef, Tensor? bias, "
          "Tensor? scale, Tensor? shift, int act, int n_rows, int block_rows) -> Tensor");
    m.def("gcn_norm(Tensor rowptr, Tensor col, Tensor w_raw) -> Tensor");
    m.def("segment_mean(Tensor segptr, Tensor x) -> Tensor");
    m.def("request_branch(Tensor x, Tensor table, Tensor rowptr, Tensor col, Tensor seg_ptr, int max_nodes, Tensor[] layer_tensors, "
          "Tensor lin_w_packed, Tensor lin_b, int hidden) -> Tensor");
    m.def("gin_layer(Tensor rowptr, Tensor col, Tensor x, Tensor eps, Tensor w1, Tensor? b1, Tensor? a1, Tensor? s1, Tensor w2, Tensor? b2, "
          "Tensor? a2, Tensor? s2, Tensor? w3=None, Tensor? b3=None) -> Tensor");
    m.def("gin_layer_split(Tensor rowptr, Tensor col, Tensor x, Tensor eps, Tensor w1, Tensor i1, Tensor? b1, Tensor? a1, Tensor? s1, "
          "Tensor w2, Tensor i2, Tensor? b2, Tensor? a2, Tensor? s2, Tensor? w3=None, Tensor? i3=None, Tensor? b3=None) -> Tensor");
    m.def("segment_topk_feasible(Tensor scores, Tensor cat_ptr, Tensor qos, Tensor local_bounds, Tensor present, Tensor global_bounds, "
          "int n_per) -> (Tensor, Tensor)");
    m.def("rank_rows(Tensor scores) -> Tensor");
    m.def("precision_at_k(Tensor ranking, Tensor labels, int[] ks) -> Tensor");
    m.def("attention_logits(Tensor enc_out, Tensor queries, int step, Tensor idx, float tanh_c, bool use_tanh) -> Tensor");
    m.def("qos_reward(Tensor actions, int level) -> Tensor");
    m.def("lstm_encode(Tensor?[] net_tensors, int n_nets, str precision='f32', int impl=0, int lds_kb=0, bool write_through=False, "
          "Tensor? workspace=None, Tensor? status=None, bool paired_start=False) -> Tensor[]");
    m.def("pointer_decode(Tensor?[] net_tensors, int[] latent_from, Tensor inputs, int n_cat, int n_per, float tanh_c=10.0, "
          "bool use_tanh=True, bool want_queries=False, str precision='f32', int impl=0, int lds_kb=0, bool write_through=False, "
          "Tensor? workspace=None, Tensor? status=None, int[] sample_seeds=[], bool paired_start=False) -> Tensor[]");
}

TORCH_LIBRARY_IMPL(gnnpn, CUDA, m) {
    m.impl("linear", linear);
    m.impl("embed_concat", embed_concat);
    m.impl("csr_aggregate", csr_aggregate);
    m.impl("csr_aggregate_blocks", csr_aggregate_blocks);
    m.impl("csr_aggregate_tiled", csr_aggregate_tiled);
    m.impl("gcn_norm", gcn_norm);
    m.impl("segment_mean", segment_mean);
    m.impl("request_branch", request_branch);
    m.impl("gin_layer", gin_layer);
    m.impl("gin_layer_split", gin_layer_split);
    m.impl("segment_topk_feasible", segment_topk_feasible);
    m.impl("rank_rows", rank_rows);
    m.impl("precision_at_k", precision_at_k);
    m.impl("attention_logits", attention_logits);
    m.impl("qos_reward", qos_reward);
    m.impl("lstm_encode", lstm_encode);
    m.impl("pointer_decode", pointer_decode);
}
```

### gnnpn-sc_amd/custom_ops.py

```python
import os

import torch

from . import _lib, ops

DECODE_KEYS = ("enc_out", "h0", "c0", "start", "wih", "whh", "bih", "bhh", "embedded", "emb_w", "emb_b",
               "xw_fold", "xb_fold", "start_fold", "latent_win", "whh_split")
DECODE_OUTS = ("idx", "win_logits", "pick_prob", "actions", "queries")
ENCODE_KEYS = ("pregates", "inputs", "w_in", "b_in", "whh", "bhh", "whh_split")
REQUEST_LAYER_KEYS = ("w0p", "b0", "a1", "s1", "w3p", "b3", "a2", "s2", "eps")

TORCH_LIB_PATH = os.environ.get("GNNPN_TORCH_LIB") or os.path.join(os.path.dirname(os.path.abspath(__file__)), "libgnnpn_torch.so")


def _load():
    _lib.load()
    if not os.path.exists(TORCH_LIB_PATH):
        raise _lib.GnnpnError(f"{TORCH_LIB_PATH} is missing: build it with `python gnnpn-sc_amd/build.py` (the gnnpn:: operators are "
                              "registered from C++; there is no Python or CPU fallback)")
    torch.ops.load_library(TORCH_LIB_PATH)


_load()



def _gnnpn_errors(fn):
    import functools

    @functools.wraps(fn)
    def call(*a, **k):
        try:
            return fn(*a, **k)
        except _lib.GnnpnError:
            raise
        except RuntimeError as e:
            raise _lib.GnnpnError(str(e).split("\nException raised from")[0]) from None
    return call


def _coop_ws(device, H, n_per, impl, ws):
    return ops.workspaces(device, ws) if ops.coop_supported(H, n_per, impl) else None


@_gnnpn_errors
def lstm_encode(nets, precision="f32", impl=0, lds_kb=0, write_through=False, ws=None, paired_start=False):
    flat = [d.get(k) for d in nets for k in ENCODE_KEYS]
    first = nets[0]["pregates"] if nets[0].get("pregates") is not None else nets[0]["inputs"]
    wsp = _coop_ws(first.device, nets[0]["bhh"].numel() // 4, 1, impl, ws)
    out = torch.ops.gnnpn.lstm_encode(flat, len(nets), precision, impl, lds_kb, bool(write_through),
                                      None if wsp is None else wsp.encode(), None if wsp is None else wsp.status, bool(paired_start))
    if wsp is not None:
        wsp.note_launch(0, _lib.load().gnnpn_last_launch_units())
    n = len(nets)
    return out[:n], out[n:2 * n], out[2 * n:]


@_gnnpn_errors
def pointer_decode(nets, inputs, n_cat, n_per, tanh_c=10.0, use_tanh=True, want_queries=False, precision="f32", impl=0,
                   lds_kb=0, write_through=False, ws=None, paired_start=False):
    flat = [d.get(k) for d in nets for k in DECODE_KEYS]
    lf = [int(d.get("latent_from", -1)) for d in nets]
    seeds = [int(d["sample_seed"]) & 0x7FFFFFFFFFFFFFFF if d.get("sample") else -1 for d in nets]
    B, L, H = nets[0]["enc_out"].shape
    wsp = _coop_ws(inputs.device, H, n_per, impl, ws)
    out = torch.ops.gnnpn.pointer_decode(flat, lf, inputs, n_cat, n_per, float(tanh_c), bool(use_tanh), bool(want_queries),
                                         precision, impl, lds_kb, bool(write_through),
                                         None if wsp is None else wsp.decode(B, n_cat, n_per), None if wsp is None else wsp.status,
                                         seeds, bool(paired_start))
    if wsp is not None:
        wsp.note_launch(1, _lib.load().gnnpn_last_launch_units())
    m = len(DECODE_OUTS)
    res = []
    for i in range(len(nets)):
        d = dict(zip(DECODE_OUTS, out[i * m:(i + 1) * m]))
        if d["queries"].numel() == 0 and not want_queries:
            d["queries"] = None
        res.append(d)
    return res


@_gnnpn_errors
def request_branch(x, table, rowptr, col, seg_ptr, max_nodes, layers, lin_w_packed, lin_b, hidden):
    flat = [lp[k] for lp in layers for k in REQUEST_LAYER_KEYS]
    return torch.ops.gnnpn.request_branch(x, table, rowptr, col, seg_ptr, int(max_nodes), flat, lin_w_packed, lin_b, int(hidden))


@_gnnpn_errors
def csr_aggregate(rowptr, col, w, x, self_coef=None, bias=None, scale=None, shift=None, act=0, block_rows=0):
    form, aux = ops.csr_aggregate_form(rowptr, col, w, x, block_rows)
    if form == "tiled":
        return torch.ops.gnnpn.csr_aggregate_tiled(aux.header, aux.order, aux.selfw, aux.batches, x, self_coef, bias, scale, shift, act,
                                                   aux.n_rows, aux.block_rows)
    if form == "blocks":
        return torch.ops.gnnpn.csr_aggregate_blocks(rowptr, col, w, x, self_coef, bias, scale, shift, act, int(block_rows), aux)
    return torch.ops.gnnpn.csr_aggregate(rowptr, col, w, x, self_coef, bias, scale, shift, act)
```

### gnnpn-sc_amd/modelML.py

```python
import os

import torch
from torch import nn

from . import custom_ops, graph, ops
from .ops import ACT_NONE, ACT_RELU, ACT_SIGMOID

BN_EPS = 1e-5


class NodeEncoder(nn.Module):

    def __init__(self, hiddenChannels, vocab=100):
        super().__init__()
        self.embeddings = nn.ModuleList(nn.Embedding(vocab, hiddenChannels) for _ in range(9))

    def reset_parameters(self):
        for e in self.embeddings:
            e.reset_parameters()


class GINConv(nn.Module):

    def __init__(self, mlp):
# ... 140 lines not shown
        n_lin = self.nodeLin.weight.shape[0]
        fused = self.fuse_gin_layers and h.shape[0] >= 4096 and all(
            "w0q" in lp and ops.gin_layer_supported(lp["w0"].shape[1], lp["w0"].shape[0], lp["w3"].shape[0]) for lp in p["gin"])
        last = len(p["gin"]) - 1
        lin_done = False
        prec = self.dense_precision if dense_precision is None else dense_precision
        if prec not in ("f32", "split"):
            raise ops.GnnpnError(f"dense_precision must be 'f32' or 'split', got {prec!r}")
        split = fused and prec == "split" and all("w0s" in lp for lp in p["gin"])
        for i, lp in enumerate(p["gin"]):
            if fused:
                with_lin = i == last and "nodeLin_q" in p and ops.gin_layer_supported(lp["w0"].shape[1], 256, 128, n_lin)
                if split and ops.gin_layer_split_supported(lp["w0"].shape[1], 256, 128):
                    with_lin = with_lin and "nodeLin_s" in p
                    h = torch.ops.gnnpn.gin_layer_split(wf_csr.rowptr, wf_csr.col, h, lp["eps"], *lp["w0s"], lp["b0"], lp["a1"], lp["s1"],
                                                        *lp["w3s"], lp["b3"], lp["a2"], lp["s2"],
                                                        *(p["nodeLin_s"] if with_lin else (None, None)),
                                                        p["nodeLin"][1] if with_lin else None)
                    lin_done = with_lin
                    continue
                h = torch.ops.gnnpn.gin_layer(wf_csr.rowptr, wf_csr.col, h, lp["eps"], lp["w0q"], lp["b0"], lp["a1"], lp["s1"],
                                              lp["w3q"], lp["b3"], lp["a2"], lp["s2"],
                                              p["nodeLin_q"] if with_lin else None, p["nodeLin"][1] if with_lin else None)
                lin_done = with_lin
                continue
            agg = torch.ops.gnnpn.csr_aggregate(wf_csr.rowptr, wf_csr.col, None, h, self_coef=lp["eps"])
            t = torch.ops.gnnpn.linear(agg, lp["w0"], lp["b0"], lp["a1"], lp["s1"], ACT_RELU)
            h = torch.ops.gnnpn.linear(t, lp["w3"], lp["b3"], lp["a2"], lp["s2"], ACT_RELU)
        if not lin_done:
            h = torch.ops.gnnpn.linear(h, *p["nodeLin"])
        return torch.ops.gnnpn.segment_mean(seg_ptr, h)

    @torch.no_grad()
    def service_embedding(self, x_service, svc_csr):
        p = self.prepared(x_service.device)
        xs = torch.ops.gnnpn.embed_concat(x_service, p["service_table"])
        if not self.isService:
            for lp in p["nolin"]:
                xs = torch.ops.gnnpn.linear(xs, lp["w"], lp["bias"], lp["a"], lp["s"], ACT_RELU)
            return torch.ops.gnnpn.linear(xs, *p["serviceLin"])
        norm = getattr(svc_csr, "_gcn_norm", None)
        if norm is None:
            norm = torch.ops.gnnpn.gcn_norm(svc_csr.rowptr, svc_csr.col, svc_csr.w)
            if not torch.cuda.is_current_stream_capturing():
                svc_csr._gcn_norm = norm
        for lp in p["gcn"]:
            xw = torch.ops.gnnpn.linear(xs, lp["wt"])
            xs = custom_ops.csr_aggregate(svc_csr.rowptr, svc_csr.col, norm, xw, bias=lp["bias"], scale=lp["a"],
                                          shift=lp["s"], act=ACT_RELU, block_rows=svc_csr.block_rows)
        return torch.ops.gnnpn.linear(xs, *p["serviceLin"])

    @torch.no_grad()
    def scores(self, x, wf_csr, seg_ptr, x_service, svc_csr, service_emb=None, max_nodes=0, dense_precision=None):
        if service_emb is not None:
            xr = self.request_embedding(x, wf_csr, seg_ptr, max_nodes, dense_precision)
            return torch.ops.gnnpn.linear(xr, service_emb, act=ACT_SIGMOID)
        if not self.parallel_branches:
            xr = self.request_embedding(x, wf_csr, seg_ptr, max_nodes, dense_precision)
            xs = self.service_embedding(x_service, svc_csr)
            return torch.ops.gnnpn.linear(xr, xs, act=ACT_SIGMOID)
        cur = torch.cuda.current_stream(x.device)
        side = self._side_streams.get(x.device)
        if side is None:
            side = self._side_streams[x.device] = torch.cuda.Stream(x.device)
        side.wait_stream(cur)
        with torch.cuda.stream(side):
            xs = self.service_embedding(x_service, svc_csr)
        xr = self.request_embedding(x, wf_csr, seg_ptr, max_nodes, dense_precision)
        cur.wait_stream(side)
        xs.record_stream(cur)
        return torch.ops.gnnpn.linear(xr, xs, act=ACT_SIGMOID)

    def forward(self, data):
        if self.training:
            raise NotImplementedError("Net.forward is the inference forward; the training step (BatchNorm on batch statistics, "
                                      "BCE, backward, Adam) is gnnpn_sc_amd.trainML.ml_train_step / TrainML.train")
        x = data.x.squeeze().float().contiguous()
        cache = getattr(data, "_gnnpn_csr", None)
        if cache is None:
            S = self.outChannels
            n_graphs = int(data.batch.max().item()) + 1
            xs = data.x_service.squeeze().float().contiguous()
            n_svc = xs.shape[0]
            if n_svc != S and n_svc != n_graphs * S:
                raise ValueError(f"x_service has {n_svc} rows: expected outChannels = {S} (one copy) or one copy per "
                                 f"graph = {n_graphs * S}")
            copies = n_svc // S
            b = data.batch.long()
            inside = bool((b[data.edge_index[0].long()] == b[data.edge_index[1].long()]).all().item()) if data.edge_index.numel() else True
            cache = {"wf": graph.csr_by_destination(data.edge_index, x.shape[0]),
                     "seg": graph.segment_ptr(data.batch, n_graphs),
                     "svc": graph.gcn_csr(data.edge_index_service, data.edge_attr_service, n_svc),
                     "xs": xs, "copies": copies,
                     "max_nodes": int(torch.bincount(b).max().item()) if inside else 0}
            if graph.block_local(data.edge_index_service, S):
                cache["svc"].block_rows = S
            if copies > 1:
                dev = xs.device
                cache["mean_rowptr"] = (torch.arange(S + 1, device=dev, dtype=torch.int32) * copies).contiguous()
                cache["mean_col"] = (torch.arange(S, device=dev, dtype=torch.int32).view(S, 1) +
                                     S * torch.arange(copies, device=dev, dtype=torch.int32).view(1, copies)).reshape(-1).contiguous()
            try:
                data._gnnpn_csr = cache
            except AttributeError:
                pass
        if cache["copies"] == 1:
            return self.scores(x, cache["wf"], cache["seg"], cache["xs"], cache["svc"], max_nodes=cache["max_nodes"])
        emb_all = self.service_embedding(cache["xs"], cache["svc"])
        total = torch.ops.gnnpn.csr_aggregate(cache["mean_rowptr"], cache["mean_col"], None, emb_all)
        emb = total / float(cache["copies"])
        return self.scores(x, cache["wf"], cache["seg"], None, None, service_emb=emb, max_nodes=cache["max_nodes"])
```

### gnnpn-sc_amd/modelPN.py

```python
import math

import os

import torch
from torch import nn

from . import custom_ops, ops

FOLD_INPUT_PROJECTION = True

qosandcons = 8
qosNum = 4
consNum = 2


class LatentWindows:

    def __init__(self, win, idx, enc_out, queries, tanh_c, use_tanh, bahdanau=None):
        self.win, self.idx = win, idx
        self._enc_out, self._queries = enc_out, queries
        self._tanh_c, self._use_tanh = tanh_c, use_tanh
        self._bahdanau, self._ref = bahdanau, None

    def __len__(self):
        return self.win.shape[1]

    def __getitem__(self, k):
        if isinstance(k, slice):
            return [self[i] for i in range(*k.indices(len(self)))]
        if k < 0:
            k += len(self)
        if self._bahdanau is not None:
            from . import ops
            a = {n: v.detach().float().contiguous() for n, v in self._bahdanau.items()}
            B, L, H = self._enc_out.shape
            if self._ref is None:
                self._ref = ops.linear(self._enc_out.reshape(B * L, H), a["wref"].reshape(H, H).contiguous(), a["bref"]).view(B, L, H)
            qp = ops.linear(self._queries[:, k, :].contiguous(), a["wq"], a["bq"])
            return ops.attention_logits_bahdanau(self._ref, qp, a["v"], k, self.idx, self._tanh_c, self._use_tanh)
        return torch.ops.gnnpn.attention_logits(self._enc_out, self._queries, k, self.idx, self._tanh_c, self._use_tanh)

    def __iter__(self):
        return (self[k] for k in range(len(self)))

    def copy(self):
        return self


def _window_tensor(latent, n_cat, n_per):
    if latent is None:
        return None
    if isinstance(latent, LatentWindows):
        return latent.win
    if len(latent) != n_cat:
        raise ValueError(f"latent has {len(latent)} steps, expected {n_cat}")
    return torch.stack([latent[k][:, k * n_per:(k + 1) * n_per] for k in range(n_cat)], 1).contiguous()


class Attention(nn.Module):

    def __init__(self, hidden_size, use_tanh=False, C=10, name="Bahdanau", use_cuda=True):
        super().__init__()
# ... 228 lines not shown
        out = self.actor.run(inputs, latent, want_queries=True,
                             sample_seed=None if sample == "greedy" else self.actor.next_sample_seed())
        T = self.serCategory
        action_idxs = [out["idx"][:, k].long() for k in range(T)]
        actions = [out["actions"][:, k, :] for k in range(T)]
        action_probs = [out["pick_prob"][:, k] for k in range(T)]
        latent_p = LatentWindows(out["win_logits"], out["idx"], out["enc_out"], out["queries"], self.actor.C,
                                 self.actor.use_tanh, self.actor.pointer.side())
        if training == "RL":
            R = self.reward(actions, labs, self.serCategory, USE_CUDA=self.use_cuda, level=self.level,
                            embedding_size=self.embedding_size)
            return R, action_probs, actions, action_idxs, latent_p
        return (_ProbList(out, latent, T, self.sNumber), action_probs, actions, action_idxs, latent_p)


@torch.no_grad()
def default_precision(low, high, fold=None, sampling=False, decode_impl=0):
    la, ha = low.actor, high.actor
    fits = all(a.hidden_size == 256 and a.serNumber <= 16 and a.embedding_size == 0 and not a.general for a in (la, ha))
    folded = FOLD_INPUT_PROJECTION if fold is None else bool(fold)
    return "split" if fits and folded and not sampling and decode_impl != 1 else "f32"


def two_level_greedy(low, high, inputs, fold=None, precision=None, decode_impl=0, lds_kb=0, write_through=False, ws=None,
                     sample_high_seed=None, paired_start=False):
    inputs = inputs.contiguous()
    la, ha = low.actor, high.actor
    if precision is None:
        precision = default_precision(low, high, fold, sample_high_seed is not None, decode_impl)
    if la.general or ha.general or la.embedding_size != 0 or ha.embedding_size != 0:
        dl = la.run(inputs, None, fold=fold, encoder_precision=precision)
        dh = ha.run(inputs, LatentWindows(dl["win_logits"], dl["idx"], None, None, la.C, la.use_tanh), fold=fold,
                    sample_seed=sample_high_seed, encoder_precision=precision)
        R = torch.ops.gnnpn.qos_reward(dh["actions"][..., -qosandcons:].contiguous(), 0 if high.level == "Low" else 1)
        return {"idx_low": dl["idx"], "idx_high": dh["idx"], "R": R, "actions": dh["actions"],
                "action_probs": dh["pick_prob"], "win_low": dl["win_logits"], "win_high_raw": dh["win_logits"]}
    for name in ("C", "use_tanh", "serNumber", "serCategory", "hidden_size", "seq_len"):
        if getattr(la, name) != getattr(ha, name):
            raise ops.GnnpnError(f"two_level_greedy: Low and High nets differ in {name} ({getattr(la, name)!r} vs "
                                 f"{getattr(ha, name)!r}); decode them with separate CombinatorialRL.forward calls")
    return _two_level_fused(low, high, inputs, fold, precision, decode_impl, lds_kb, write_through, ws, sample_high_seed,
                            paired_start)[0]


def _two_level_fused(low, high, inputs, fold, precision, decode_impl, lds_kb, write_through, ws, sample_high_seed, paired_start):
    la, ha = low.actor, high.actor
    la.check_precision(precision)
    ha.check_precision(precision)
    enc_l, emb_l = la.encode_args(inputs, fold)
    enc_h, emb_h = ha.encode_args(inputs, fold)
    enc, h_n, c_n = custom_ops.lstm_encode([enc_l, enc_h], precision=precision, lds_kb=lds_kb, write_through=write_through, ws=ws,
                                           paired_start=paired_start)
    del enc_l, enc_h
    dl, dh = custom_ops.pointer_decode([la.decode_args(emb_l, enc[0], h_n[0], c_n[0], fold=fold),
                                 ha.decode_args(emb_h, enc[1], h_n[1], c_n[1], latent_from=0, fold=fold,
                                                sample_seed=sample_high_seed)],
                                inputs, la.serCategory, la.serNumber, la.C, la.use_tanh,
                                precision="split" if precision == "split" else "f32", impl=decode_impl, lds_kb=lds_kb,
                                write_through=write_through, ws=ws, paired_start=paired_start)
    R = torch.ops.gnnpn.qos_reward(dh["actions"], 0 if high.level == "Low" else 1)
    return ({"idx_low": dl["idx"], "idx_high": dh["idx"], "R": R, "actions": dh["actions"],
             "action_probs": dh["pick_prob"], "win_low": dl["win_logits"], "win_high_raw": dh["win_logits"]},
            (enc[1], h_n[1], c_n[1], emb_h))


def fresh_seed():
    return int.from_bytes(os.urandom(8), "little") & 0x7FFFFFFFFFFFFFFF


def two_level_best_of(low, high, inputs, samples, seed=None, precision=None, fold=None, decode_impl=0, lds_kb=0, write_through=False,
                      ws=None):
    samples = int(samples)
    if samples < 1:
        raise ops.GnnpnError(f"two_level_best_of: samples must be >= 1, got {samples}")
    seed = fresh_seed() if seed is None else int(seed)
    inputs = inputs.contiguous()
    la, ha = low.actor, high.actor
    B = inputs.shape[0]
    T, K = ha.serCategory, ha.serNumber
    level = 0 if high.level == "Low" else 1
    general = la.general or ha.general or la.embedding_size != 0 or ha.embedding_size != 0
    if general:
        g = two_level_greedy(low, high, inputs, fold=fold, precision=precision, decode_impl=decode_impl, lds_kb=lds_kb,
                             write_through=write_through, ws=ws)
        if precision is None:
            precision = default_precision(low, high, fold, False, decode_impl)
        rep = None
        if samples > 1:
            lat = LatentWindows(g["win_low"], g["idx_low"], None, None, la.C, la.use_tanh)
            outs = [ha.run(inputs, lat, fold=fold, sample_seed=ops.replica_seed(seed, j), encoder_precision=precision)
                    for j in range(1, samples)]
            rep = {"idx": torch.stack([o["idx"] for o in outs], 1).contiguous(),
                   "actions": torch.stack([o["actions"] for o in outs], 1).contiguous(),
                   "pick_prob": torch.stack([o["pick_prob"] for o in outs], 1).contiguous()}
    else:
        if precision is None:
            precision = default_precision(low, high, fold, False, decode_impl)
        g, (enc_h, h_h, c_h, emb_h) = _two_level_fused(low, high, inputs, fold, precision, decode_impl, lds_kb, write_through, ws,
                                                        None, False)
        rep = None
        if samples > 1:
            net = ha.decode_args(emb_h, enc_h, h_h, c_h, latent_win=g["win_low"], fold=fold)
            rep = ops.pointer_decode_replicas(net, inputs, T, K, samples - 1, seed, first=1, tanh_c=ha.C, use_tanh=ha.use_tanh,
                                              impl=decode_impl, lds_kb=lds_kb, write_through=write_through, ws=ws)
    sam = None
    if rep is not None:
        act = rep["actions"]
        R_s = torch.ops.gnnpn.qos_reward(act[..., -qosandcons:].reshape(B * (samples - 1), T, qosandcons).contiguous(), level)
        sam = {"R": R_s.view(B, samples - 1), "idx": rep["idx"], "actions": act, "probs": rep["pick_prob"]}
    sel = _select(g, sam, g["actions"].shape[-1])
    if ops.coop_supported(ha.hidden_size, K, decode_impl):
        ops.workspaces(inputs.device, ws).check()
    out = dict(g)
# ... 22 lines not shown
```

### gnnpn-sc_amd/ops.py

```python
import itertools
import weakref

import torch

from . import _lib
from ._lib import ACT_NONE, ACT_RELU, ACT_SIGMOID, GnnpnError, check, dev_ptr, ptr_array, stream_ptr

F32, I32, F64, U8 = torch.float32, torch.int32, torch.float64, torch.uint8


def _rows2d(t, name):
    if t.dim() != 2:
        raise GnnpnError(f"{name}: expected a 2-D tensor, got shape {tuple(t.shape)}")
    return t


def linear(a, weight, bias=None, scale=None, shift=None, act=ACT_NONE, out=None):
    a, weight = _rows2d(a, "linear.a"), _rows2d(weight, "linear.weight")
    M, K = a.shape
    N = weight.shape[0]
    if weight.shape[1] != K:
        raise GnnpnError(f"linear: K mismatch {a.shape} x {weight.shape}")
    if out is None:
        out = torch.empty((M, N), dtype=F32, device=a.device)
# ... 215 lines not shown
    if (w1.numel() != lib.gnnpn_split_weights_bytes(h1, k1) or w2.numel() != lib.gnnpn_split_weights_bytes(h2, h1) or
            (w3 is not None and w3.numel() != lib.gnnpn_split_weights_bytes(h3, h2))):
        raise GnnpnError("gin_layer_split: packed weights do not chain (c_in -> h1 -> h2 [-> h3])")
    out = torch.empty((n, h3 if w3 is not None else h2), dtype=F32, device=x.device)
    u8 = lambda t, name, opt=False: None if (t is None and opt) else dev_ptr(t, torch.uint8, name)
    check(lib.gnnpn_gin_layer_split(
        dev_ptr(rowptr, I32, "rowptr"), dev_ptr(col, I32, "col"), dev_ptr(x, F32, "x"), c_in, c_in, dev_ptr(eps, F32, "eps"),
        u8(w1, "w1"), dev_ptr(i1, F32, "i1"), dev_ptr(b1, F32, "b1", True), dev_ptr(a1, F32, "a1", True), dev_ptr(s1, F32, "s1", True), h1,
        u8(w2, "w2"), dev_ptr(i2, F32, "i2"), dev_ptr(b2, F32, "b2", True), dev_ptr(a2, F32, "a2", True), dev_ptr(s2, F32, "s2", True), h2,
        u8(w3, "w3", True), dev_ptr(i3, F32, "i3", True), dev_ptr(b3, F32, "b3", True), h3, dev_ptr(out, F32, "out"), out.shape[1], n,
        stream_ptr()), "gnnpn_gin_layer_split")
    return out


def gin_layer_split_supported(c_in, h1, h2, h3=None):
    return h1 == 256 and h2 == 128 and (h3 is None or h3 == 128) and 0 < c_in <= 128 and (c_in % 4 == 0 or c_in <= 32)


def gin_layer_supported(c_in, h1, h2, h3=None):
    return h1 == 256 and h2 == 128 and (h3 is None or h3 == 128) and 0 < c_in <= 256


def pack_mfma_b32(w):
    N, K = w.shape
    if N % 32:
        raise GnnpnError(f"pack_mfma_b32: output features {N} must be a multiple of 32")
    Kp = (K + 31) // 32 * 32
    wp = torch.zeros((N, Kp), dtype=w.dtype, device=w.device)
    wp[:, :K] = w
    v = wp.view(N // 32, 32, Kp // 2, 2)
    return v.permute(0, 2, 3, 1).reshape(N // 32, Kp // 2, 64).contiguous()


REQUEST_BRANCH_MAX_NODES = 16


def request_branch(x, table, rowptr, col, seg_ptr, max_nodes, layers, lin_w_packed, lin_b, hidden):
    x = _rows2d(x, "request_branch.x")
    vocab, emb = table.shape
    B = seg_ptr.numel() - 1
    out = torch.empty((B, hidden), dtype=F32, device=x.device)
    arr = (_lib.GinLayer * len(layers))()
    for i, lp in enumerate(layers):
        a = arr[i]
        for field, key in (("w0_packed", "w0p"), ("b0", "b0"), ("bn1_scale", "a1"), ("bn1_shift", "s1"), ("w3_packed", "w3p"),
                           ("b3", "b3"), ("bn2_scale", "a2"), ("bn2_shift", "s2"), ("eps", "eps")):
            setattr(a, field, dev_ptr(lp[key], F32, f"layers[{i}].{key}").value)
    check(_lib.load().gnnpn_request_branch_f32(
        dev_ptr(x, F32, "x"), x.shape[1] - 1, dev_ptr(table, F32, "table"), vocab, emb, dev_ptr(rowptr, I32, "rowptr"),
        dev_ptr(col, I32, "col"), dev_ptr(seg_ptr, I32, "seg_ptr"), B, int(max_nodes), len(layers), arr, int(hidden),
        dev_ptr(lin_w_packed, F32, "lin_w_packed"), dev_ptr(lin_b, F32, "lin_b"), dev_ptr(out, F32, "out"), stream_ptr()),
        "gnnpn_request_branch_f32")
    return out


def select_candidates(scores, cat_ptr, qos, local_bounds, present, global_bounds, n_per):
    scores = _rows2d(scores, "select.scores")
    B, S = scores.shape
    T = cat_ptr.numel() - 1
    if qos.shape != (S, 4) or local_bounds.shape != (B, T, 4) or present.shape != (B, T) \
            or global_bounds.shape != (B, 4):
        raise GnnpnError("select_candidates: inconsistent shapes")
    rows = torch.empty((B, T * n_per, 8), dtype=F32, device=scores.device)
    ids = torch.empty((B, T * n_per), dtype=I32, device=scores.device)
    check(_lib.load().gnnpn_select_candidates(
        dev_ptr(scores, F32, "scores"), S, dev_ptr(cat_ptr, I32, "cat_ptr"), dev_ptr(qos, F64, "qos"),
        dev_ptr(local_bounds, F64, "local_bounds"), dev_ptr(present, U8, "present"),
        dev_ptr(global_bounds, F64, "global_bounds"), dev_ptr(rows, F32, "rows"), dev_ptr(ids, I32, "ids"), B, T,
        n_per, stream_ptr()), "gnnpn_select_candidates")
    return rows, ids


def rank_rows(scores):
    scores = _rows2d(scores, "rank_rows.scores")
    B, S = scores.shape
    ranking = torch.empty((B, S), dtype=I32, device=scores.device)
    check(_lib.load().gnnpn_rank_rows(dev_ptr(scores, F32, "scores"), S, dev_ptr(ranking, I32, "ranking"), B, S,
                                      stream_ptr()), "gnnpn_rank_rows")
    return ranking


def precision_at_k(ranking, labels, ks=(1, 5)):
    B, S = labels.shape
    ks = [int(k) for k in ks]
    if not ks or min(ks) < 1:
        raise GnnpnError(f"precision_at_k: every k must be >= 1, got {ks}")
    if ranking.dim() != 2 or ranking.shape[0] != B or ranking.shape[1] < min(max(ks), S):
        raise GnnpnError(f"precision_at_k: ranking [B={B}, >= {min(max(ks), S)}] expected, got {tuple(ranking.shape)}")
    kt = torch.tensor(list(ks), dtype=I32, device=labels.device)
    out = torch.empty((B, len(ks)), dtype=F32, device=labels.device)
    check(_lib.load().gnnpn_precision_at_k(dev_ptr(ranking, I32, "ranking"), ranking.shape[1],
                                           dev_ptr(labels, F32, "labels"), S, B, S, dev_ptr(kt, I32, "ks"), len(ks),
                                           dev_ptr(out, F32, "out"), stream_ptr()), "gnnpn_precision_at_k")
    return out


def pack_lstm_weight(w):
    H = w.shape[1]
    if w.shape[0] != 4 * H or H % 4:
        raise GnnpnError(f"pack_lstm_weight: expected [4H,H], got {tuple(w.shape)}")
    return w.reshape(4, H, H // 4, 4).permute(2, 0, 1, 3).contiguous()


def lstm_split_ptr(split, whh_packed, name):
    if split is None:
        return None
# ... 916 lines not shown
```

### gnnpn-sc_amd/pipeline.py

```python
import ctypes
import os
from dataclasses import dataclass

import numpy as np
import torch

from . import _lib, custom_ops, graph, ops
from .modelPN import two_level_best_of, two_level_greedy


@dataclass
class DeviceServices:
    x_service: torch.Tensor
    csr: graph.CSR
    cat_ptr: torch.Tensor
    qos: torch.Tensor
    emb_cache: tuple = None

    @staticmethod
    def from_table(table, device):
        ei = torch.from_numpy(np.ascontiguousarray(table.edge_index))
        ea = torch.from_numpy(np.ascontiguousarray(table.edge_attr))
        csr = graph.gcn_csr(ei, ea, table.n_services).to(device)
        return DeviceServices(torch.from_numpy(table.x_service).to(device), csr,
                              torch.from_numpy(np.ascontiguousarray(table.cat_ptr)).to(device),
                              torch.from_numpy(np.ascontiguousarray(table.qos)).to(device))


@dataclass
class DeviceBatch:
    x: torch.Tensor
    wf_csr: graph.CSR
    seg_ptr: torch.Tensor
    local_bounds: torch.Tensor
    present: torch.Tensor
    global_bounds: torch.Tensor
    max_nodes: int = 0

    @property
    def n_problems(self):
        return self.present.shape[0]

    @staticmethod
    def from_problems(pb, device):
        ei = torch.from_numpy(np.ascontiguousarray(pb.edge_index))
        batch = torch.from_numpy(np.ascontiguousarray(pb.batch))
        n = pb.x.shape[0]
        inside = bool((pb.batch[pb.edge_index[0]] == pb.batch[pb.edge_index[1]]).all()) if pb.edge_index.size else True
        max_nodes = int(np.bincount(pb.batch, minlength=1).max()) if inside and n else 0
        return DeviceBatch(torch.from_numpy(pb.x).to(device), graph.csr_by_destination(ei, n).to(device),
                           graph.segment_ptr(batch, pb.n_problems).to(device),
                           torch.from_numpy(np.ascontiguousarray(pb.local_bounds)).to(device),
                           torch.from_numpy(np.ascontiguousarray(pb.present)).to(device),
                           torch.from_numpy(np.ascontiguousarray(pb.global_bounds)).to(device), max_nodes)

    def shard(self, rank, world):
        B = self.n_problems
        lo, hi = B * rank // world, B * (rank + 1) // world
        seg = self.seg_ptr.cpu()
        n0, n1 = int(seg[lo]), int(seg[hi])
        rp = self.wf_csr.rowptr.cpu()
        e0, e1 = int(rp[n0]), int(rp[n1])
        dev = self.x.device
        csr = graph.CSR((rp[n0:n1 + 1] - e0).to(dev), (self.wf_csr.col[e0:e1] - n0).contiguous(), None, n1 - n0)
        return DeviceBatch(self.x[n0:n1].contiguous(), csr, (seg[lo:hi + 1] - n0).to(dev),
                           self.local_bounds[lo:hi].contiguous(), self.present[lo:hi].contiguous(),
                           self.global_bounds[lo:hi].contiguous(), self.max_nodes)


DEFAULT_WRITE_THROUGH = os.environ.get("GNNPN_PIPE_WRITE_THROUGH", "0") == "1"
HOST_COPY_ON_ITS_OWN_STREAM = os.environ.get("GNNPN_HOST_COPY_INLINE") != "1"
COMMON_START_US = 0.0


def half_batch_split(n_problems):
    half = ((int(n_problems) + 31) // 32) * 16
    return half if 0 < half < n_problems else 0


_warned_partitioned = set()


def warn_partitioned_device(device, precision):
    import warnings
    if device.type != "cuda":
        return
    idx = device.index if device.index is not None else torch.cuda.current_device()
    if idx in _warned_partitioned:
        return
    _warned_partitioned.add(idx)
    n_cu = torch.cuda.get_device_properties(idx).multi_processor_count
    if n_cu < 256:
        warnings.warn(f"gnnpn: cuda:{idx} shows {n_cu} compute units; the cooperative recurrent kernels are built for 8 XCDs x 32 CUs (MI355X, SPX "
                      f"mode). precision={precision!r}: " + ("the recurrent launches will raise GNNPN_E_UNSUP — " if precision != "f32" else "") +
                      "only the per-workgroup streaming forms (precision='f32', impl=1) run here, about 10 x slower per recurrent step.",
                      RuntimeWarning, stacklevel=3)


@torch.no_grad()
def refine(services, batch, out, popSize, MAX_Iter, reduct=0, seeds=None, min_cost=None, patches=()):
    actions = out["actions"]
    dev = actions.device
    B = batch.n_problems
    tabs = ops.woa_candidates(services.cat_ptr, services.qos, batch.x, batch.seg_ptr, batch.local_bounds, batch.global_bounds,
                              actions, reduct=reduct, patches=patches)
    if seeds is None:
        seeds = np.frombuffer(os.urandom(8 * B), dtype=np.int64).copy()
    if not isinstance(seeds, torch.Tensor):
        seeds = torch.from_numpy(np.asarray(seeds, dtype=np.uint64).reshape(B).view(np.int64).copy())
    seeds = seeds.to(device=dev, dtype=torch.int64).contiguous()
    fit, pos, hist, draws, rows = ops.eswoa_ragged(tabs["prob_ptr"], tabs["cand_ptr"], tabs["len_init"], tabs["cand"],
                                                   tabs["bounds"], tabs["start_pos"], popSize, MAX_Iter, seeds,
                                                   max_slots=tabs["max_slots"], max_cand=tabs["max_cand"])
    res = {"best_fitness": fit, "best_rows": rows, "n_slots": tabs["n_slots"], "best_pos": pos, "history": hist, "draws": draws}
    if min_cost is not None:
        mc = min_cost if isinstance(min_cost, torch.Tensor) else torch.as_tensor(np.asarray(min_cost, dtype=np.float64))
        res["quality"] = mc.to(device=dev, dtype=torch.float64) / fit
    return res


class ML2PNPipeline:

    def __init__(self, net, low, high, n_per, precision=None):
        from .modelPN import default_precision
        self.net, self.low, self.high, self.n_per = net, low, high, n_per
        self.precision = default_precision(low, high) if precision is None else precision
        self.cache_service_embedding = True
        self._side_streams = {}
        warn_partitioned_device(next(low.parameters()).device, self.precision)

    @torch.no_grad()
    def service_embedding(self, services):
        prep = self.net.prepared(services.x_service.device)
        c = services.emb_cache
        if c is None or c[0] is not prep:
            c = services.emb_cache = (prep, self.net.service_embedding(services.x_service, services.csr))
        return c[1]

    @torch.no_grad()
    def scores(self, services, batch):
        return self.net.scores(batch.x, batch.wf_csr, batch.seg_ptr, services.x_service, services.csr,
                               service_emb=self.service_embedding(services) if self.cache_service_embedding else None,
                               max_nodes=batch.max_nodes, dense_precision="split" if self.precision == "split" else "f32")

    @torch.no_grad()
    def candidates(self, services, batch, scores):
        return torch.ops.gnnpn.segment_topk_feasible(scores, services.cat_ptr, services.qos, batch.local_bounds,
                                                     batch.present, batch.global_bounds, self.n_per)

    @torch.no_grad()
    def run(self, services, batch, decode_impl=0, lds_kb=0, ws=None, paired_start=False, write_through=False):
        scores = self.scores(services, batch)
        rows, ids = self.candidates(services, batch, scores)
        if isinstance(ws, (tuple, list)):
            B = rows.shape[0]
            half = half_batch_split(B)
            if len(ws) != 2 or not half:
                raise ops.GnnpnError(f"ML2PNPipeline.run: two half-batches need 2 workspaces and more than 16 problems (got {len(ws)}, {B})")
            cur = torch.cuda.current_stream(rows.device)
            side = self._side_streams.get(rows.device)
            if side is None:
                side = self._side_streams[rows.device] = torch.cuda.Stream(rows.device)
            for net in (self.low, self.high):
                net.actor.packed()
                net.actor.check_precision(self.precision)
            n_cat = rows.shape[1] // self.n_per
            for w in ws:
                w.encode()
                w.decode(max(half, B - half), n_cat, self.n_per)
            side.wait_stream(cur)
            with torch.cuda.stream(side):
                out_b = two_level_greedy(self.low, self.high, rows[half:], precision=self.precision, decode_impl=decode_impl,
                                         lds_kb=lds_kb, ws=ws[1], paired_start=True, write_through=write_through)
            out_a = two_level_greedy(self.low, self.high, rows[:half], precision=self.precision, decode_impl=decode_impl,
                                     lds_kb=lds_kb, ws=ws[0], paired_start=True, write_through=write_through)
            cur.wait_stream(side)
            for v in out_b.values():
                v.record_stream(cur)
            out = {k: torch.cat([out_a[k], out_b[k]]) for k in out_a}
        else:
            out = two_level_greedy(self.low, self.high, rows, precision=self.precision, decode_impl=decode_impl,
                                   lds_kb=lds_kb, ws=ws, paired_start=paired_start, write_through=write_through)
        out.update(scores=scores, pn_inputs=rows, candidate_ids=ids)
        return out

    @torch.no_grad()
    def best_of(self, services, batch, samples, seed=None, decode_impl=0, lds_kb=0, ws=None, write_through=False):
        scores = self.scores(services, batch)
        rows, ids = self.candidates(services, batch, scores)
        out = two_level_best_of(self.low, self.high, rows, samples, seed=seed, precision=self.precision, decode_impl=decode_impl,
                                lds_kb=lds_kb, write_through=write_through, ws=ws)
        out.update(scores=scores, pn_inputs=rows, candidate_ids=ids)
        return out

    def refine(self, services, batch, out, popSize, MAX_Iter, reduct=0, seeds=None, min_cost=None, patches=()):
        return refine(services, batch, out, popSize, MAX_Iter, reduct=reduct, seeds=seeds, min_cost=min_cost, patches=patches)

    def capture(self, services, batch, warmup=2, decode_impl=0, lds_kb=0, ws=None, paired_start=False, pool=None, write_through=False):
        ws = ops.new_workspaces(batch.x.device) if ws is None else ws
        all_ws = list(ws) if isinstance(ws, (tuple, list)) else [ws]
        stream = torch.cuda.Stream()
        stream.wait_stream(torch.cuda.current_stream())
        with torch.cuda.stream(stream):
            for _ in range(warmup):
                self.run(services, batch, decode_impl, lds_kb, ws, paired_start, write_through)
        torch.cuda.current_stream().wait_stream(stream)
        torch.cuda.synchronize()
        graph = torch.cuda.CUDAGraph()
        with torch.cuda.graph(graph, pool=pool, capture_error_mode="thread_local"):
            out = self.run(services, batch, decode_impl, lds_kb, ws, paired_start, write_through)
        for w in all_ws:
            w.frozen = True
        booked_replay = ops.graph_replay(graph, all_ws)

        def replay():
            booked_replay()
            return out
        replay.graph, replay.outputs, replay.workspaces = graph, out, ws
        return replay

    @torch.no_grad()
    def rankings(self, services, batch):
        return torch.ops.gnnpn.rank_rows(self.scores(services, batch))

    @torch.no_grad()
    def test(self, services, batch, labels):
        ranking = self.rankings(services, batch)
        pk = torch.ops.gnnpn.precision_at_k(ranking, labels.float().contiguous(), [1, 5])
        return ranking, [float(v) for v in pk.mean(0).tolist()]


_last_runner_on_device = {}


def _has_collective_stream():
    import torch.distributed as td
    if not (td.is_available() and td.is_initialized()):
        return False
    try:
        return "nccl" in str(td.get_backend()).lower()
    except Exception:
        return True
# ... 288 lines not shown
```

### include/gnnpn_hip.h

```cpp
#ifndef GNNPN_HIP_H
#define GNNPN_HIP_H

#include <stdint.h>

#ifdef __cplusplus
extern "C" {
#endif

#define GNNPN_ABI_VERSION 9

#define GNNPN_OK 0
#define GNNPN_E_ARG (-1)
#define GNNPN_E_UNSUP (-2)
#define GNNPN_E_LAUNCH (-3)

#define GNNPN_ACT_NONE 0
#define GNNPN_ACT_RELU 1
#define GNNPN_ACT_SIGMOID 2

int gnnpn_abi_version(void);
const char* gnnpn_last_error(void);

int gnnpn_linear_f32(const float* A, int64_t lda, const float* W, int64_t ldw, const float* bias,
                     const float* scale, const float* shift, int act, float* C, int64_t ldc,
// ... 28 lines not shown
    int64_t tstart_bytes;
    int64_t selfw_bytes;
    int64_t meta_bytes;
} gnnpn_tile_plan_geom_t;
int gnnpn_csr_tile_plan_geometry(int32_t n_rows, int32_t block_rows, gnnpn_tile_plan_geom_t* out);
int gnnpn_csr_tile_plan_rows(const int32_t* rowptr, const int32_t* col, const float* w, int32_t n_rows, int32_t block_rows,
                             int32_t* header, int32_t* order, int32_t* tstart, float* selfw, int32_t* meta, void* stream);
int gnnpn_csr_tile_plan_fill(const int32_t* col, const float* w, int32_t n_rows, int32_t block_rows, const int32_t* header,
                             const int32_t* order, const int32_t* tstart, void* batches, int64_t n_quads, void* stream);
int gnnpn_csr_aggregate_tiled_f32(const int32_t* header, const int32_t* order, const float* selfw, const void* batches,
                                  const float* x, int64_t ldx, const float* self_coef, const float* bias,
                                  const float* scale, const float* shift, int act, float* y, int64_t ldy,
                                  int32_t n_rows, int32_t C, int32_t block_rows, void* stream);

int gnnpn_gcn_norm_f32(const int32_t* rowptr, const int32_t* col, const float* w_raw,
                       float* deg_inv_sqrt, float* norm, int32_t n_rows, void* stream);

int gnnpn_segment_mean_f32(const int32_t* segptr, const float* x, int64_t ldx, float* out,
                           int64_t ldo, int32_t n_seg, int32_t C, void* stream);

int gnnpn_gin_layer_f32(const int32_t* rowptr, const int32_t* col, const float* x, int64_t ldx, int32_t c_in, const float* eps,
                        const float* w1, const float* b1, const float* bn1_scale, const float* bn1_shift, int32_t h1,
                        const float* w2, const float* b2, const float* bn2_scale, const float* bn2_shift, int32_t h2,
                        const float* w3, const float* b3, int32_t h3, float* out, int64_t ldo, int64_t n_rows, void* stream);

int64_t gnnpn_split_weights_bytes(int32_t n_out, int32_t k);
int gnnpn_pack_split_weights_f16(const float* w, int64_t ldw, int32_t n_out, int32_t k, void* packed, float* col_inv, void* stream);
int gnnpn_gin_layer_split(const int32_t* rowptr, const int32_t* col, const float* x, int64_t ldx, int32_t c_in, const float* eps,
                          const void* w1, const float* inv1, const float* b1, const float* bn1_scale, const float* bn1_shift, int32_t h1,
                          const void* w2, const float* inv2, const float* b2, const float* bn2_scale, const float* bn2_shift, int32_t h2,
                          const void* w3, const float* inv3, const float* b3, int32_t h3, float* out, int64_t ldo, int64_t n_rows,
                          void* stream);

typedef struct {
    const float* w0_packed;
    const float* b0;
    const float* bn1_scale;
    const float* bn1_shift;
    const float* w3_packed;
    const float* b3;
    const float* bn2_scale;
    const float* bn2_shift;
    const float* eps;
} gnnpn_gin_layer_t;
int gnnpn_request_branch_f32(const float* x, int32_t nfeat, const float* table, int32_t vocab, int32_t emb,
                             const int32_t* rowptr, const int32_t* col, const int32_t* seg_ptr, int32_t n_graphs,
                             int32_t max_nodes, int32_t n_layers, const gnnpn_gin_layer_t* layers, int32_t hidden,
                             const float* lin_w_packed, const float* lin_b, float* out, void* stream);

int gnnpn_select_candidates(const float* scores, int64_t ld_scores, const int32_t* cat_ptr,
                            const double* qos, const double* local_bounds,
                            const uint8_t* present, const double* global_bounds, float* out_rows,
                            int32_t* out_ids, int32_t B, int32_t T, int32_t n_per, void* stream);

int gnnpn_rank_rows(const float* scores, int64_t ld_scores, int32_t* ranking, int32_t B, int32_t S,
                    void* stream);

int gnnpn_precision_at_k(const int32_t* ranking, int64_t ld_rank, const float* labels, int64_t ld_lab,
                         int32_t B, int32_t S, const int32_t* ks, int32_t n_k, float* out, void* stream);

typedef struct {
    const float* pregates;
    const float* inputs;
    const float* w_in;
    const float* b_in;
    const float* whh_packed;
    const float* bhh;
    float* enc_out;
    float* h_n;
    float* c_n;
    const void* whh_split;
} gnnpn_encode_net_t;

#define GNNPN_PREC_F32 0
#define GNNPN_PREC_F16 1
#define GNNPN_PREC_SPLIT 2

#define GNNPN_STATUS_WORDS 8
#define GNNPN_STATUS_CODE 0
#define GNNPN_STATUS_DECLINED_SEATS 1
#define GNNPN_STATUS_OFF_CANONICAL_SEATS 2
#define GNNPN_STATUS_ENC_EXPECTED 4
#define GNNPN_STATUS_ENC_FINISHED 5
#define GNNPN_STATUS_DEC_EXPECTED 6
#define GNNPN_STATUS_DEC_FINISHED 7
#define GNNPN_COOP_ENC_TIMEOUT 1
#define GNNPN_COOP_DEC_TIMEOUT 2
#define GNNPN_COOP_MEMBER_MISSING 4
#define GNNPN_COOP_DIRTY 8
#define GNNPN_COOP_SHORTFALL 16
typedef struct {
    int32_t impl;
    int32_t lds_kb;
    int32_t write_through;
    int32_t paired_start;
    uint32_t* sticky_status;
} gnnpn_launch_opts_t;

int64_t gnnpn_lstm_split_weights_bytes(void);
int gnnpn_lstm_pack_split_weights_f32(const float* whh_packed, void* split, void* stream);

int gnnpn_lstm_encode_f32(int n_nets, const gnnpn_encode_net_t* nets, int32_t B, int32_t L, int32_t H,
                          int32_t F, int32_t precision, const gnnpn_launch_opts_t* opts, void* workspace,
                          int64_t workspace_bytes, void* stream);

int64_t gnnpn_lstm_encode_workspace_bytes(void);
// ... 27 lines not shown
    int32_t* idx;
    float* win_logits;
    float* pick_prob;
    float* actions;
    float* queries;
    int32_t latent_from;
    int32_t sample;
    uint64_t sample_seed;
    const void* whh_split;
} gnnpn_decode_net_t;

int gnnpn_pointer_decode_f32(int n_nets, const gnnpn_decode_net_t* nets, const float* inputs,
                             float tanh_c, int use_tanh, int32_t B, int32_t T, int32_t n_per, int32_t H,
                             int32_t precision, const gnnpn_launch_opts_t* opts, void* workspace,
                             int64_t workspace_bytes, void* stream);

typedef struct {
    int32_t attention;
    int32_t n_glimpses;
    const float* pointer_wq;
    const float* pointer_bq;
    const float* pointer_ref;
    const float* pointer_v;
    const float* glimpse_wq;
    const float* glimpse_bq;
    const float* glimpse_ref;
    const float* glimpse_v;
} gnnpn_attention_t;

int gnnpn_pointer_decode_attn_f32(const gnnpn_decode_net_t* net, const gnnpn_attention_t* attn, const float* inputs,
                                  float tanh_c, int use_tanh, int32_t B, int32_t T, int32_t n_per, int32_t H, void* stream);

int64_t gnnpn_pointer_decode_workspace_bytes(int32_t B, int32_t T, int32_t n_per);

int gnnpn_pointer_decode_replicas_f32(const gnnpn_decode_net_t* net, const float* inputs, float tanh_c, int use_tanh, int32_t B,
                                      int32_t R, int32_t first, uint64_t seed, int32_t T, int32_t n_per, int32_t H,
                                      const gnnpn_launch_opts_t* opts, void* workspace, int64_t workspace_bytes, void* stream);
uint64_t gnnpn_replica_seed(uint64_t seed, int32_t replica);

int gnnpn_best_of_select_f32(int32_t B, int32_t N, int32_t T, const float* R0, const int32_t* idx0, const float* actions0,
                             const float* probs0, const float* Rs, const int32_t* idxs, const float* actionss, const float* probss,
                             float* R_out, int32_t* idx_out, float* actions_out, float* probs_out, int32_t* winner, void* stream);

int gnnpn_attention_logits_f32(const float* enc_out, const float* queries, int64_t ld_q,
                               const int32_t* masked_idx, float tanh_c, int use_tanh, float* logits,
                               int32_t B, int32_t L, int32_t H, int32_t n_masked, int32_t ld_idx,
                               void* stream);
int gnnpn_attention_logits_bahdanau_f32(const float* ref, const float* qp, int64_t ld_q, const float* v,
                                        const int32_t* masked_idx, float tanh_c, int use_tanh, float* logits,
                                        int32_t B, int32_t L, int32_t H, int32_t n_masked, int32_t ld_idx, void* stream);

int gnnpn_qos_reward_f32(const float* actions, float* R, int32_t B, int32_t T, int level,
                         void* stream);

typedef struct {
    const float* embedded;
    const float* enc_out;
    const float* h0;
    const float* c0;
    const float* start;
    const float* wih;
    const float* whh;
    const float* bih;
    const float* bhh;
    const float* latent_win;
    const int32_t* idx;
    float* x_all;
    float* gates_pre;
    float* c_all;
    float* h_all;
    float* z0;
    float* probs;
    float* logp;
} gnnpn_decode_train_t;
int gnnpn_gemm_f32(const float* A, int64_t lda, int a_kmajor, const float* B, int64_t ldb, int b_kmajor, float* C,
                   int64_t ldc, int64_t M, int N, int K, int split_k, void* stream);
int gnnpn_lstm_train_forward_f32(const float* pregates, const float* whh, const float* bhh, float* enc_out,
                                 float* gates_pre, float* c_all, int32_t B, int32_t L, int32_t H, void* stream);
int gnnpn_decode_train_forward_f32(const gnnpn_decode_train_t* t, int32_t B, int32_t T, int32_t n_per, int32_t H,
                                   float tanh_c, int use_tanh, void* stream);
int gnnpn_decode_train_backward_f32(const gnnpn_decode_train_t* t, const float* gscale, float* d_enc_out, float* dgates,
                                    float* dx, float* dh0, float* dc0, int32_t B, int32_t T, int32_t n_per, int32_t H,
                                    float tanh_c, int use_tanh, void* stream);
int gnnpn_lstm_train_backward_f32(const float* whh, const float* gates_pre, const float* c_all, const float* d_enc_out,
                                  const float* dh0, const float* dc0, float* dgates, int32_t B, int32_t L, int32_t H,
                                  void* stream);

typedef struct {
    gnnpn_decode_train_t base;
    int32_t bahdanau;
    int32_t n_glimpses;
    const float* p_wq_t;
    const float* p_wq;
    const float* p_bq;
    const float* p_v;
    const float* p_ref;
    const float* g_wq_t;
    const float* g_wq;
    const float* g_bq;
    const float* g_v;
    const float* g_ref;
    float* q_all;
    float* a_all;
    float* d_p_ref;
    float* d_g_ref;
    float* d_p_qp;
// ... 80 lines not shown
```

Measured before the change: 476,200.

## Fuse score GEMM with candidate selection and merge decode tail kernels

Adds a fused score+select kernel that computes request-service scores tile by tile per category group and runs feasible top-k selection on them, using a host-precomputed tile plan cached on the service table. It also fuses the pick-probability and QoS-reward kernels into one two-level tail launch, so the cooperative decode can skip its own pick_prob pass. The aim is fewer kernel launches and no round trip of the full score matrix through global memory between scoring and selection. The cost is new code paths gated on device CU count and category widths, with a fallback to the old path when those gates fail.

```diff
diff --git a/gnnpn-sc_amd/_lib.py b/gnnpn-sc_amd/_lib.py
--- a/gnnpn-sc_amd/_lib.py
+++ b/gnnpn-sc_amd/_lib.py
@@ -41,6 +41,9 @@
     "gnnpn_request_branch_f32": (c_int, [_P, c_int32, _P, c_int32, c_int32, _P, _P, _P, c_int32, c_int32, c_int32, _P, c_int32,
                                          _P, _P, _P, _P]),
     "gnnpn_select_candidates": (c_int, [_P, c_int64, _P, _P, _P, _P, _P, _P, _P, c_int32, c_int32, c_int32, _P]),
+    "gnnpn_score_select_tile_cols": (c_int, []),
+    "gnnpn_score_select_f32": (c_int, [_P, c_int64, _P, c_int64, _P, c_int64, _P, c_int32, _P, _P, _P, _P, _P, _P, _P, c_int32, c_int32,
+                                       c_int32, c_int32, c_int32, _P]),
     "gnnpn_rank_rows": (c_int, [_P, c_int64, _P, c_int32, c_int32, _P]),
     "gnnpn_precision_at_k": (c_int, [_P, c_int64, _P, c_int64, c_int32, c_int32, _P, c_int32, _P, _P]),
     "gnnpn_lstm_encode_f32": (c_int, [c_int, _P, c_int32, c_int32, c_int32, c_int32, c_int32, _P, _P, c_int64, _P]),
@@ -68,6 +71,7 @@
                                            c_int32, c_int32, _P]),
     "gnnpn_attention_logits_bahdanau_f32": (c_int, [_P, _P, c_int64, _P, _P, c_float, c_int, _P, c_int32, c_int32, c_int32, c_int32, c_int32, _P]),
     "gnnpn_qos_reward_f32": (c_int, [_P, _P, c_int32, c_int32, c_int, _P]),
+    "gnnpn_two_level_tail_f32": (c_int, [_P, _P, _P, _P, _P, _P, _P, _P, c_int32, c_int32, c_int32, c_int, _P]),
     "gnnpn_split3_pieces_f32": (c_int, [_P, c_int64, c_int32, _P, _P, _P, _P]),
     "gnnpn_recurrent_product_f32": (c_int, [_P, _P, c_int32, _P, _P, _P]),
     "gnnpn_gemm_f32": (c_int, [_P, c_int64, c_int, _P, c_int64, c_int, _P, c_int64, c_int64, c_int, c_int, c_int, _P]),
diff --git a/gnnpn-sc_amd/build.py b/gnnpn-sc_amd/build.py
--- a/gnnpn-sc_amd/build.py
+++ b/gnnpn-sc_amd/build.py
@@ -7,8 +7,9 @@
 ROOT = os.path.dirname(HERE)
 CSRC = os.path.join(HERE, "csrc")
 LIB = os.path.join(HERE, "libgnnpn_hip.so")
-SOURCES = ["api.hip", "dense.hip", "graph.hip", "graph_tiled.hip", "gin_layer.hip", "gin_layer_split.hip", "request_branch.hip", "select.hip", "lstm.hip", "lstm_coop.hip", "decode.hip", "decode_coop.hip", "decode_lean.hip", "train.hip", "train_attn.hip", "train_ml.hip", "decode_glimpse.hip", "woa.hip", "woa_prep.hip", "split_probe.hip"]
+SOURCES = ["api.hip", "dense.hip", "graph.hip", "graph_tiled.hip", "gin_layer.hip", "gin_layer_split.hip", "request_branch.hip", "select.hip", "lstm.hip", "lstm_coop.hip", "decode.hip", "decode_coop.hip", "decode_lean.hip", "decode_tail.hip", "train.hip", "train_attn.hip", "train_ml.hip", "decode_glimpse.hip", "woa.hip", "woa_prep.hip", "split_probe.hip"]
 HEADERS = [os.path.join(CSRC, "common.h"), os.path.join(CSRC, "graph_lds.h"), os.path.join(CSRC, "recurrent.h"), os.path.join(CSRC, "lstm_shared.h"), os.path.join(CSRC, "decode_shared.h"), os.path.join(CSRC, "coop_common.h"), os.path.join(CSRC, "train_common.h"),
+           os.path.join(CSRC, "dense_tile.h"), os.path.join(CSRC, "select_shared.h"), os.path.join(CSRC, "score_select.h"), os.path.join(CSRC, "decode_tail.h"),
            os.path.join(ROOT, "include", "gnnpn_hip.h")]
 FLAGS = ["-O3", "--offload-arch=gfx950", "-ffp-contract=off", "-fPIC", "-std=c++17",
          "-I" + os.path.join(ROOT, "include"), "-I" + CSRC] + os.environ.get("GNNPN_EXTRA_HIPCC_FLAGS", "").split()
diff --git a/gnnpn-sc_amd/csrc/decode.hip b/gnnpn-sc_amd/csrc/decode.hip
--- a/gnnpn-sc_amd/csrc/decode.hip
+++ b/gnnpn-sc_amd/csrc/decode.hip
@@ -4,6 +4,7 @@
 #include <string.h>
 #include "recurrent.h"
 #include "decode_shared.h"
+#include "decode_tail.h"
 #include "lstm_shared.h"
 
 template <int H, int BT, bool REP = false>
@@ -148,7 +149,8 @@
     DecodeArgs args{};
     for (int n = 0; n < n_nets; ++n) {
         const gnnpn_decode_net_t& d = nets[n];
-        if (const int rc = decode_net_check(d, "pointer_decode", n)) return rc;
+        if (const int rc = decode_net_check(d, "pointer_decode", n, true)) return rc;
+        GNNPN_REQUIRE((d.pick_prob == nullptr) == (nets[0].pick_prob == nullptr), "pointer_decode: pick_prob is NULL in every net of a call or in none");
         GNNPN_REQUIRE(d.embedded || (d.emb_w && d.emb_b) || d.xw_fold,
                       "pointer_decode: net %d needs embedded, (emb_w, emb_b) or the folded input side", n);
         GNNPN_REQUIRE(d.latent_from < n && d.latent_from >= -1, "pointer_decode: latent_from of net %d must name an "
@@ -171,9 +173,16 @@
         GNNPN_FAIL(GNNPN_E_UNSUP, "pointer_decode: sampling is built in the streaming and the 8-CU-group fp32 forms (impl 0-2, "
                    "GNNPN_PREC_F32)");
     const int impl = opts.impl;
+    const bool no_prob = nets[0].pick_prob == nullptr;
+    if (no_prob) {
+        bool fold = true;
+        for (int n = 0; n < n_nets; ++n) fold = fold && nets[n].xw_fold != nullptr;
+        GNNPN_REQUIRE(impl != 1 && gnnpn_decode_coop_supported(H, n_per) && n_per <= 16 && workspace != nullptr && fold && !any_sample,
+                      "pointer_decode: pick_prob may be NULL only in the cooperative form with the folded input side and greedy picks");
+    }
     if (impl != 1 && gnnpn_decode_coop_supported(H, n_per) && (workspace != nullptr || impl >= 2)) {
         const int rc = gnnpn_launch_decode_coop(args, n_nets, precision, impl == 4, opts, workspace, workspace_bytes, s);
-        const bool fall_through = rc == GNNPN_E_UNSUP && impl == 0 && precision == GNNPN_PREC_F32;
+        const bool fall_through = rc == GNNPN_E_UNSUP && impl == 0 && precision == GNNPN_PREC_F32 && !no_prob;
         if (rc != GNNPN_OK && !fall_through) return rc;
         if (fall_through) {
             static std::atomic<bool> said{false};
@@ -342,62 +351,7 @@
 
 __global__ __launch_bounds__(256) void qos_reward_kernel(const float* __restrict__ actions, float* __restrict__ R, int32_t B,
                                                         int32_t T, int level) {
-    const int lane = threadIdx.x & 63;
-    const int b = blockIdx.x * 4 + (threadIdx.x >> 6);
-    if (b >= B) return;
-    const float* a = actions + (int64_t)b * T * 8;
-    const float lo0 = a[4], hi0 = a[5], lo1 = a[6], hi1 = a[7];
-    float prod2 = 1.0f, prod3 = 1.0f, mn = INFINITY;
-    double sum0 = 0.0;
-    int n_real = 0;
-    auto fetch = [&](int t) { return *reinterpret_cast<const float4*>(a + (int64_t)min(t, T - 1) * 8); };
-    auto consume = [&](float4 q, int t0) {
-        if (t0 + lane >= T) q = make_float4(0.0f, INFINITY, 1.0f, 1.0f);
-        n_real += q.x > 0.0f;
-        mn = fminf(mn, q.y);
-        const double xd = (double)q.x;
-        const int lo = __double2loint(xd), hi = __double2hiint(xd);
-        const int zi = __float_as_int(q.z), wi = __float_as_int(q.w);
-        const int cnt = min(64, T - t0);
-#define GNNPN_REWARD_STEP(i)                                                                                      \
-    prod2 = __fmul_rn(prod2, __int_as_float(__builtin_amdgcn_readlane(zi, i)));                                   \
-    prod3 = __fmul_rn(prod3, __int_as_float(__builtin_amdgcn_readlane(wi, i)));                                   \
-    sum0 += __hiloint2double(__builtin_amdgcn_readlane(hi, i), __builtin_amdgcn_readlane(lo, i));
-        if (cnt == 64) {
-#pragma unroll
-            for (int i = 0; i < 64; ++i) { GNNPN_REWARD_STEP(i) }
-        } else {
-            for (int i = 0; i < cnt; ++i) { GNNPN_REWARD_STEP(i) }
-        }
-#undef GNNPN_REWARD_STEP
-    };
-    float4 qa = fetch(lane), qb;
-    for (int t0 = 0; t0 < T; t0 += 128) {
-        qb = fetch(t0 + 64 + lane);
-        consume(qa, t0);
-        if (t0 + 64 >= T) break;
-        qa = fetch(t0 + 128 + lane);
-        consume(qb, t0 + 64);
-    }
-#pragma unroll
-    for (int off = 32; off > 0; off >>= 1) {
-        n_real += __shfl_xor(n_real, off, 64);
-        mn = fminf(mn, __shfl_xor(mn, off, 64));
-    }
-    if (lane != 0) return;
-    int violate = 0;
-    if (prod2 < lo0 || prod2 > hi0) ++violate;
-    if (prod3 < lo1 || prod3 > hi1) ++violate;
-    if (level == 0) {
-        R[b] = (float)violate;
-        return;
-    }
-    float obj = (float)sum0 / (float)n_real;
-    obj = __fadd_rn(obj, 1.0f);
-    obj = __fsub_rn(obj, mn);
-    obj = obj / 2.0f;
-    const double v = (double)violate + (double)obj;
-    R[b] = (float)(rint(v * 1e5) / 1e5);
+    qos_reward_block(actions, R, B, T, level, blockIdx.x);
 }
 
 extern "C" int gnnpn_qos_reward_f32(const float* actions, float* R, int32_t B, int32_t T, int level,
diff --git a/gnnpn-sc_amd/csrc/decode_lean.hip b/gnnpn-sc_amd/csrc/decode_lean.hip
--- a/gnnpn-sc_amd/csrc/decode_lean.hip
+++ b/gnnpn-sc_amd/csrc/decode_lean.hip
@@ -1,6 +1,7 @@
 #include "common.h"
 #include "recurrent.h"
 #include "decode_shared.h"
+#include "decode_tail.h"
 #include "coop_common.h"
 #include "lstm_shared.h"
 
@@ -435,44 +436,6 @@
         if (abort_flag) coop_raise(err, sticky, 2u, seats);
         coop_note_finished(sticky, GNNPN_STATUS_DEC_FINISHED, tiles_done);
     }
-}
-
-struct PickProbArgs {
-    const float* win[2];
-    const float* lat[2];
-    const int32_t* idx[2];
-    float* out[2];
-};
-__global__ __launch_bounds__(256) void pick_prob_kernel(PickProbArgs a, int64_t rows, int T, int K) {
-    const int net = blockIdx.y;
-    const float* __restrict__ win = a.win[net];
-    const float* __restrict__ lat = a.lat[net];
-    const int32_t* __restrict__ idx = a.idx[net];
-    float* __restrict__ out = a.out[net];
-    const int64_t row = blockIdx.x * 256ll + threadIdx.x;
-    if (row >= rows) return;
-    const unsigned t_base = (unsigned)__builtin_amdgcn_readfirstlane((int)((blockIdx.x * 256ll) % T));
-    const int t = (int)((t_base + threadIdx.x) % (unsigned)T);
-    float v[16];
-#pragma unroll
-    for (int j = 0; j < 16; ++j) {
-        v[j] = 0.0f;
-        if (j < K) {
-            v[j] = win[row * K + j];
-            if (lat) v[j] = __fadd_rn(v[j], lat[row * K + j]);
-        }
-    }
-    const int pick_r = min(max(idx[row] - t * K, 0), 15);
-    float best = v[0];
-#pragma unroll
-    for (int j = 1; j < 16; ++j) best = j == pick_r ? v[j] : best;
-#pragma unroll
-    for (int j = 0; j < 16; ++j) v[j] = j < K ? expf(__fsub_rn(v[j], best)) : 0.0f;
-#pragma unroll
-    for (int n = 8; n >= 1; n >>= 1)
-#pragma unroll
-        for (int j = 0; j < n; ++j) v[j] = __fadd_rn(v[j], v[j + n]);
-    out[row] = 1.0f / v[0];
 }
 
 static DecodeWorkspace lean_workspace(int64_t groups, int64_t rows, int32_t T, int32_t K) {
@@ -518,7 +481,7 @@
 #undef GNNPN_LEAN
     if (hipGetLastError() != hipSuccess) GNNPN_FAIL(GNNPN_E_LAUNCH, "pointer_decode: launch of the cooperative kernel failed");
     const int64_t rows = (int64_t)args.B * args.T;
-    for (int n0 = 0; n0 < n_nets; n0 += 2) {
+    for (int n0 = 0; n0 < n_nets && args.net[0].pick_prob; n0 += 2) {
         PickProbArgs pa = {};
         const int cnt = n_nets - n0 < 2 ? n_nets - n0 : 2;
         for (int n = 0; n < cnt; ++n) {
@@ -528,7 +491,7 @@
             pa.idx[n] = d.idx;
             pa.out[n] = d.pick_prob;
         }
-        hipLaunchKernelGGL(pick_prob_kernel, dim3((unsigned)((rows + 255) / 256), (unsigned)cnt), dim3(256), 0, s, pa, rows, args.T, args.K);
+        gnnpn_launch_pick_prob(pa, cnt, rows, args.T, args.K, nullptr, nullptr, 0, 0, s);
     }
     return GNNPN_OK;
 }
diff --git a/gnnpn-sc_amd/csrc/decode_shared.h b/gnnpn-sc_amd/csrc/decode_shared.h
--- a/gnnpn-sc_amd/csrc/decode_shared.h
+++ b/gnnpn-sc_amd/csrc/decode_shared.h
@@ -30,10 +30,10 @@
 };
 static_assert(sizeof(DecodeNet) == sizeof(gnnpn_decode_net_t), "DecodeNet must mirror gnnpn_decode_net_t");
 
-inline int decode_net_check(const gnnpn_decode_net_t& d, const char* who, int n) {
+inline int decode_net_check(const gnnpn_decode_net_t& d, const char* who, int n, bool prob_optional = false) {
     GNNPN_REQUIRE(d.enc_out && d.h0 && d.c0 && d.start && d.wih_packed && d.whh_packed && d.bih && d.bhh,
                   "%s: null input of net %d (enc_out, h0, c0, start and the decoder weights are required)", who, n);
-    GNNPN_REQUIRE(d.idx && d.win_logits && d.pick_prob && d.actions, "%s: null output of net %d", who, n);
+    GNNPN_REQUIRE(d.idx && d.win_logits && (d.pick_prob || prob_optional) && d.actions, "%s: null output of net %d", who, n);
     GNNPN_REQUIRE((d.xw_fold != nullptr) == (d.xb_fold != nullptr) && (d.xw_fold != nullptr) == (d.start_fold != nullptr),
                   "%s: net %d: xw_fold, xb_fold and start_fold go together", who, n);
     GNNPN_REQUIRE(d.sample == 0 || d.sample == 1, "%s: net %d: sample must be 0 (greedy) or 1 (multinomial)", who, n);
diff --git a/gnnpn-sc_amd/csrc/decode_tail.h b/gnnpn-sc_amd/csrc/decode_tail.h
--- /dev/null
+++ b/gnnpn-sc_amd/csrc/decode_tail.h
@@ -0,0 +1,102 @@
+#pragma once
+#include "common.h"
+
+struct PickProbArgs {
+    const float* win[2];
+    const float* lat[2];
+    const int32_t* idx[2];
+    float* out[2];
+};
+__device__ __forceinline__ void pick_prob_block(const PickProbArgs& a, int64_t rows, int T, int K, int net, unsigned block) {
+    const float* __restrict__ win = a.win[net];
+    const float* __restrict__ lat = a.lat[net];
+    const int32_t* __restrict__ idx = a.idx[net];
+    float* __restrict__ out = a.out[net];
+    const int64_t row = block * 256ll + threadIdx.x;
+    if (row >= rows) return;
+    const unsigned t_base = (unsigned)__builtin_amdgcn_readfirstlane((int)((block * 256ll) % T));
+    const int t = (int)((t_base + threadIdx.x) % (unsigned)T);
+    float v[16];
+#pragma unroll
+    for (int j = 0; j < 16; ++j) {
+        v[j] = 0.0f;
+        if (j < K) {
+            v[j] = win[row * K + j];
+            if (lat) v[j] = __fadd_rn(v[j], lat[row * K + j]);
+        }
+    }
+    const int pick_r = min(max(idx[row] - t * K, 0), 15);
+    float best = v[0];
+#pragma unroll
+    for (int j = 1; j < 16; ++j) best = j == pick_r ? v[j] : best;
+#pragma unroll
+    for (int j = 0; j < 16; ++j) v[j] = j < K ? expf(__fsub_rn(v[j], best)) : 0.0f;
+#pragma unroll
+    for (int n = 8; n >= 1; n >>= 1)
+#pragma unroll
+        for (int j = 0; j < n; ++j) v[j] = __fadd_rn(v[j], v[j + n]);
+    out[row] = 1.0f / v[0];
+}
+
+__device__ __forceinline__ void qos_reward_block(const float* __restrict__ actions, float* __restrict__ R, int32_t B, int32_t T, int level,
+                                                 unsigned block) {
+    const int lane = threadIdx.x & 63;
+    const int b = block * 4 + (threadIdx.x >> 6);
+    if (b >= B) return;
+    const float* a = actions + (int64_t)b * T * 8;
+    const float lo0 = a[4], hi0 = a[5], lo1 = a[6], hi1 = a[7];
+    float prod2 = 1.0f, prod3 = 1.0f, mn = INFINITY;
+    double sum0 = 0.0;
+    int n_real = 0;
+    auto fetch = [&](int t) { return *reinterpret_cast<const float4*>(a + (int64_t)min(t, T - 1) * 8); };
+    auto consume = [&](float4 q, int t0) {
+        if (t0 + lane >= T) q = make_float4(0.0f, INFINITY, 1.0f, 1.0f);
+        n_real += q.x > 0.0f;
+        mn = fminf(mn, q.y);
+        const double xd = (double)q.x;
+        const int lo = __double2loint(xd), hi = __double2hiint(xd);
+        const int zi = __float_as_int(q.z), wi = __float_as_int(q.w);
+        const int cnt = min(64, T - t0);
+#define GNNPN_REWARD_STEP(i)                                                                                      \
+    prod2 = __fmul_rn(prod2, __int_as_float(__builtin_amdgcn_readlane(zi, i)));                                   \
+    prod3 = __fmul_rn(prod3, __int_as_float(__builtin_amdgcn_readlane(wi, i)));                                   \
+    sum0 += __hiloint2double(__builtin_amdgcn_readlane(hi, i), __builtin_amdgcn_readlane(lo, i));
+        if (cnt == 64) {
+#pragma unroll
+            for (int i = 0; i < 64; ++i) { GNNPN_REWARD_STEP(i) }
+        } else {
+            for (int i = 0; i < cnt; ++i) { GNNPN_REWARD_STEP(i) }
+        }
+#undef GNNPN_REWARD_STEP
+    };
+    float4 qa = fetch(lane), qb;
+    for (int t0 = 0; t0 < T; t0 += 128) {
+        qb = fetch(t0 + 64 + lane);
+        consume(qa, t0);
+        if (t0 + 64 >= T) break;
+        qa = fetch(t0 + 128 + lane);
+        consume(qb, t0 + 64);
+    }
+#pragma unroll
+    for (int off = 32; off > 0; off >>= 1) {
+        n_real += __shfl_xor(n_real, off, 64);
+        mn = fminf(mn, __shfl_xor(mn, off, 64));
+    }
+    if (lane != 0) return;
+    int violate = 0;
+    if (prod2 < lo0 || prod2 > hi0) ++violate;
+    if (prod3 < lo1 || prod3 > hi1) ++violate;
+    if (level == 0) {
+        R[b] = (float)violate;
+        return;
+    }
+    float obj = (float)sum0 / (float)n_real;
+    obj = __fadd_rn(obj, 1.0f);
+    obj = __fsub_rn(obj, mn);
+    obj = obj / 2.0f;
+    const double v = (double)violate + (double)obj;
+    R[b] = (float)(rint(v * 1e5) / 1e5);
+}
+
+void gnnpn_launch_pick_prob(const PickProbArgs& pa, int n_nets, int64_t rows, int T, int K, const float* actions, float* R, int32_t B,
+                            int level, hipStream_t s);
diff --git a/gnnpn-sc_amd/csrc/decode_tail.hip b/gnnpn-sc_amd/csrc/decode_tail.hip
--- /dev/null
+++ b/gnnpn-sc_amd/csrc/decode_tail.hip
@@ -0,0 +1,36 @@
+#include "common.h"
+#include "decode_tail.h"
+
+__global__ __launch_bounds__(256) void pick_prob_kernel(PickProbArgs a, int64_t rows, int T, int K, unsigned prob_blocks, unsigned n_nets,
+                                                       const float* __restrict__ actions, float* __restrict__ R, int32_t B, int level) {
+    if (blockIdx.x < n_nets * prob_blocks) {
+        const int net = blockIdx.x >= prob_blocks;
+        pick_prob_block(a, rows, T, K, net, blockIdx.x - net * prob_blocks);
+    } else {
+        qos_reward_block(actions, R, B, T, level, blockIdx.x - n_nets * prob_blocks);
+    }
+}
+
+void gnnpn_launch_pick_prob(const PickProbArgs& pa, int n_nets, int64_t rows, int T, int K, const float* actions, float* R, int32_t B,
+                            int level, hipStream_t s) {
+    const unsigned prob_blocks = (unsigned)((rows + 255) / 256);
+    const unsigned reward_blocks = actions ? (unsigned)((B + 3) / 4) : 0u;
+    hipLaunchKernelGGL(pick_prob_kernel, dim3((unsigned)n_nets * prob_blocks + reward_blocks), dim3(256), 0, s, pa, rows, T, K, prob_blocks,
+                       (unsigned)n_nets, actions, R, B, level);
+}
+
+extern "C" int gnnpn_two_level_tail_f32(const float* win_low, const int32_t* idx_low, float* pick_prob_low, const float* win_high,
+                                        const int32_t* idx_high, float* pick_prob_high, const float* actions, float* R, int32_t B,
+                                        int32_t T, int32_t n_per, int level, void* stream) {
+    GNNPN_REQUIRE(B >= 0 && T > 0 && (level == 0 || level == 1), "two_level_tail: bad argument");
+    GNNPN_REQUIRE(n_per >= 1 && n_per <= 16, "two_level_tail: n_per must be in [1,16], got %d", n_per);
+    if (B == 0) return GNNPN_OK;
+    GNNPN_REQUIRE(win_low && idx_low && pick_prob_low && win_high && idx_high && pick_prob_high && actions && R, "two_level_tail: null operand");
+    GNNPN_REQUIRE(gnnpn_aligned(actions, 16), "two_level_tail: actions must be 16-byte aligned");
+    PickProbArgs pa = {};
+    pa.win[0] = win_low, pa.lat[0] = nullptr, pa.idx[0] = idx_low, pa.out[0] = pick_prob_low;
+    pa.win[1] = win_high, pa.lat[1] = win_low, pa.idx[1] = idx_high, pa.out[1] = pick_prob_high;
+    gnnpn_launch_pick_prob(pa, 2, (int64_t)B * T, T, n_per, actions, R, B, level, (hipStream_t)stream);
+    GNNPN_CHECK_LAUNCH("two_level_tail_f32");
+    return GNNPN_OK;
+}
diff --git a/gnnpn-sc_amd/csrc/dense.hip b/gnnpn-sc_amd/csrc/dense.hip
--- a/gnnpn-sc_amd/csrc/dense.hip
+++ b/gnnpn-sc_amd/csrc/dense.hip
@@ -1,58 +1,5 @@
 #include "common.h"
-
-typedef float f32x16 __attribute__((ext_vector_type(16)));
-
-template <int BM, int BN>
-struct DenseCfg {
-    static constexpr int BK = 32;
-    static constexpr int LDA = BM + 1;
-    static constexpr int LDB = BN + 1;
-    static constexpr int A_F4 = BM * BK / 4 / 256;
-    static constexpr int B_F4 = BN * BK / 4 / 256;
-    static constexpr int TM = BM / 64;
-    static constexpr int TN = BN / 64;
-};
-
-struct __attribute__((packed, aligned(4))) f4_align4 { float v[4]; };
-
-template <int NF4>
-__device__ __forceinline__ void tile_load(const float* __restrict__ P, int64_t ld, int64_t r0,
-                                          int64_t n_rows, int k0, int K, bool vec_ok, float4 (&reg)[NF4]) {
-#pragma unroll
-    for (int i = 0; i < NF4; ++i) {
-        int f = threadIdx.x + i * 256;
-        int r = f >> 3, kc = f & 7;
-        int64_t row = r0 + r;
-        int k = k0 + kc * 4;
-        float4 v = make_float4(0.f, 0.f, 0.f, 0.f);
-        if (row < n_rows) {
-            const float* src = P + row * ld + k;
-            if (vec_ok && k + 3 < K) {
-                const f4_align4 t = *reinterpret_cast<const f4_align4*>(src);
-                v = make_float4(t.v[0], t.v[1], t.v[2], t.v[3]);
-            } else {
-                if (k + 0 < K) v.x = src[0];
-                if (k + 1 < K) v.y = src[1];
-                if (k + 2 < K) v.z = src[2];
-                if (k + 3 < K) v.w = src[3];
-            }
-        }
-        reg[i] = v;
-    }
-}
-
-template <int NF4, int LD>
-__device__ __forceinline__ void tile_store(float* S, const float4 (&reg)[NF4]) {
-#pragma unroll
-    for (int i = 0; i < NF4; ++i) {
-        int f = threadIdx.x + i * 256;
-        int r = f >> 3, kc = f & 7;
-        S[(kc * 4 + 0) * LD + r] = reg[i].x;
-        S[(kc * 4 + 1) * LD + r] = reg[i].y;
-        S[(kc * 4 + 2) * LD + r] = reg[i].z;
-        S[(kc * 4 + 3) * LD + r] = reg[i].w;
-    }
-}
+#include "dense_tile.h"
 
 template <int BM, int BN>
 __global__ __launch_bounds__(256) void linear_f32_kernel(
diff --git a/gnnpn-sc_amd/csrc/dense_tile.h b/gnnpn-sc_amd/csrc/dense_tile.h
--- /dev/null
+++ b/gnnpn-sc_amd/csrc/dense_tile.h
@@ -0,0 +1,102 @@
+#pragma once
+#include "common.h"
+
+typedef float f32x16 __attribute__((ext_vector_type(16)));
+
+template <int BM, int BN>
+struct DenseCfg {
+    static constexpr int BK = 32;
+    static constexpr int LDA = BM + 1;
+    static constexpr int LDB = BN + 1;
+    static constexpr int A_F4 = BM * BK / 4 / 256;
+    static constexpr int B_F4 = BN * BK / 4 / 256;
+    static constexpr int TM = BM / 64;
+    static constexpr int TN = BN / 64;
+};
+
+struct __attribute__((packed, aligned(4))) f4_align4 { float v[4]; };
+
+template <int NF4>
+__device__ __forceinline__ void tile_load(const float* __restrict__ P, int64_t ld, int64_t r0,
+                                          int64_t n_rows, int k0, int K, bool vec_ok, float4 (&reg)[NF4]) {
+#pragma unroll
+    for (int i = 0; i < NF4; ++i) {
+        int f = threadIdx.x + i * 256;
+        int r = f >> 3, kc = f & 7;
+        int64_t row = r0 + r;
+        int k = k0 + kc * 4;
+        float4 v = make_float4(0.f, 0.f, 0.f, 0.f);
+        if (row < n_rows) {
+            const float* src = P + row * ld + k;
+            if (vec_ok && k + 3 < K) {
+                const f4_align4 t = *reinterpret_cast<const f4_align4*>(src);
+                v = make_float4(t.v[0], t.v[1], t.v[2], t.v[3]);
+            } else {
+                if (k + 0 < K) v.x = src[0];
+                if (k + 1 < K) v.y = src[1];
+                if (k + 2 < K) v.z = src[2];
+                if (k + 3 < K) v.w = src[3];
+            }
+        }
+        reg[i] = v;
+    }
+}
+
+template <int NF4, int LD>
+__device__ __forceinline__ void tile_store(float* S, const float4 (&reg)[NF4]) {
+#pragma unroll
+    for (int i = 0; i < NF4; ++i) {
+        int f = threadIdx.x + i * 256;
+        int r = f >> 3, kc = f & 7;
+        S[(kc * 4 + 0) * LD + r] = reg[i].x;
+        S[(kc * 4 + 1) * LD + r] = reg[i].y;
+        S[(kc * 4 + 2) * LD + r] = reg[i].z;
+        S[(kc * 4 + 3) * LD + r] = reg[i].w;
+    }
+}
+
+template <int BM, int BN>
+__device__ __forceinline__ void dense_tile_product(const float* __restrict__ A, int64_t lda, const float* __restrict__ W, int64_t ldw,
+                                                   int64_t m0, int64_t M, int n0, int N, int K, int vec_a, int vec_w,
+                                                   float* As, float* Bs, f32x16 (&acc)[DenseCfg<BM, BN>::TM][DenseCfg<BM, BN>::TN]) {
+    using Cfg = DenseCfg<BM, BN>;
+    const int wave = threadIdx.x >> 6, lane = threadIdx.x & 63;
+    const int wm = wave >> 1, wn = wave & 1;
+#pragma unroll
+    for (int i = 0; i < Cfg::TM; ++i)
+#pragma unroll
+        for (int j = 0; j < Cfg::TN; ++j)
+#pragma unroll
+            for (int r = 0; r < 16; ++r) acc[i][j][r] = 0.0f;
+
+    float4 ra[Cfg::A_F4], rb[Cfg::B_F4];
+    tile_load<Cfg::A_F4>(A, lda, m0, M, 0, K, vec_a, ra);
+    tile_load<Cfg::B_F4>(W, ldw, n0, N, 0, K, vec_w, rb);
+
+    const int half = lane >> 5, l32 = lane & 31;
+    for (int k0 = 0; k0 < K; k0 += Cfg::BK) {
+        tile_store<Cfg::A_F4, Cfg::LDA>(As, ra);
+        tile_store<Cfg::B_F4, Cfg::LDB>(Bs, rb);
+        __syncthreads();
+        if (k0 + Cfg::BK < K) {
+            tile_load<Cfg::A_F4>(A, lda, m0, M, k0 + Cfg::BK, K, vec_a, ra);
+            tile_load<Cfg::B_F4>(W, ldw, n0, N, k0 + Cfg::BK, K, vec_w, rb);
+        }
+#pragma unroll
+        for (int kk = 0; kk < Cfg::BK; kk += 2) {
+            float a[Cfg::TM], b[Cfg::TN];
+#pragma unroll
+            for (int i = 0; i < Cfg::TM; ++i)
+                a[i] = As[(kk + half) * Cfg::LDA + wm * (BM / 2) + i * 32 + l32];
+#pragma unroll
+            for (int j = 0; j < Cfg::TN; ++j)
+                b[j] = Bs[(kk + half) * Cfg::LDB + wn * (BN / 2) + j * 32 + l32];
+#pragma unroll
+            for (int i = 0; i < Cfg::TM; ++i)
+#pragma unroll
+                for (int j = 0; j < Cfg::TN; ++j)
+                    acc[i][j] = __builtin_amdgcn_mfma_f32_32x32x2f32(a[i], b[j], acc[i][j], 0, 0, 0);
+        }
+        __syncthreads();
+    }
+}
diff --git a/gnnpn-sc_amd/csrc/score_select.h b/gnnpn-sc_amd/csrc/score_select.h
--- /dev/null
+++ b/gnnpn-sc_amd/csrc/score_select.h
@@ -0,0 +1,124 @@
+#pragma once
+#include "common.h"
+#include "dense_tile.h"
+#include "select_shared.h"
+
+constexpr int SS_BM = 64, SS_COLS = 128;
+constexpr int SS_LD = SS_COLS + 1;
+constexpr int SS_PER_LANE = SS_COLS / 16;
+constexpr unsigned SS_LDS_BYTES = SS_BM * SS_LD * sizeof(float);
+
+struct ScoreTile {
+    const float* A;
+    int64_t lda;
+    const float* W;
+    int64_t ldw;
+    float* scores;
+    int64_t ld_scores;
+    const int32_t* tile_cat;
+    int32_t S, K;
+    int vec_a, vec_w;
+};
+
+__device__ __forceinline__ void score_select_tile(const ScoreTile& st, float* smem, const int32_t* __restrict__ cat_ptr,
+                                                  const double* __restrict__ qos, const double* __restrict__ local_bounds,
+                                                  const uint8_t* __restrict__ present, const double* __restrict__ global_bounds,
+                                                  float* __restrict__ out_rows, int32_t* __restrict__ out_ids, int32_t B, int32_t T,
+                                                  int32_t n_per) {
+    const float* __restrict__ A = st.A;
+    const float* __restrict__ W = st.W;
+    float* __restrict__ scores = st.scores;
+    const int32_t* __restrict__ tile_cat = st.tile_cat;
+    const int64_t lda = st.lda, ldw = st.ldw, ld_scores = st.ld_scores;
+    const int32_t S = st.S, K = st.K;
+    const int vec_a = st.vec_a, vec_w = st.vec_w;
+    using Cfg = DenseCfg<SS_BM, SS_COLS>;
+    static_assert(Cfg::BK * (Cfg::LDA + Cfg::LDB) <= SS_BM * SS_LD, "the operand tiles lie inside the score tile's LDS");
+    float* As = smem;
+    float* Bs = smem + Cfg::BK * Cfg::LDA;
+
+    const int wave = threadIdx.x >> 6, lane = threadIdx.x & 63;
+    const int wm = wave >> 1, wn = wave & 1;
+    const int64_t m0 = (int64_t)blockIdx.y * SS_BM;
+    const int c0 = min(max(tile_cat[blockIdx.x], 0), T), c1 = min(max(tile_cat[blockIdx.x + 1], c0), T);
+    const int n0 = min(max(cat_ptr[c0], 0), S), n1 = min(max(cat_ptr[c1], n0), min(S, n0 + SS_COLS));
+
+    f32x16 acc[Cfg::TM][Cfg::TN];
+    dense_tile_product<SS_BM, SS_COLS>(A, lda, W, ldw, m0, B, n0, n1, K, vec_a, vec_w, As, Bs, acc);
+
+    const int half = lane >> 5, l32 = lane & 31;
+#pragma unroll
+    for (int j = 0; j < Cfg::TN; ++j) {
+        const int lc = wn * (SS_COLS / 2) + j * 32 + l32;
+        const int col = n0 + lc;
+#pragma unroll
+        for (int i = 0; i < Cfg::TM; ++i) {
+#pragma unroll
+            for (int r = 0; r < 16; ++r) {
+                const int lr = wm * (SS_BM / 2) + i * 32 + (r & 3) + 8 * (r >> 2) + 4 * half;
+                const float v = apply_act(acc[i][j][r], GNNPN_ACT_SIGMOID);
+                smem[lr * SS_LD + lc] = v;
+                if (col < n1 && m0 + lr < B) scores[(m0 + lr) * ld_scores + col] = v;
+            }
+        }
+    }
+    __syncthreads();
+
+    const int sub = lane & 15;
+    const int n_groups = (c1 - c0) * SS_BM;
+    for (int g = threadIdx.x >> 4; g < n_groups; g += 16) {
+        const int p = g & (SS_BM - 1), c = c0 + (g >> 6);
+        const int64_t b = m0 + p;
+        if (b >= B) continue;
+        const int64_t seg = b * T + c;
+        const int s_begin = min(max(cat_ptr[c], n0), n1), s_end = min(max(cat_ptr[c + 1], s_begin), n1);
+        const bool pres = present[seg] != 0;
+        const double* lb = local_bounds + seg * 4;
+        const double lo_c = lb[0], hi_c = lb[1], lo_q = lb[2], hi_q = lb[3];
+        const float* srow = smem + p * SS_LD;
+
+        unsigned long long key[SS_PER_LANE];
+#pragma unroll
+        for (int i = 0; i < SS_PER_LANE; ++i) {
+            const int s = s_begin + sub + 16 * i;
+            key[i] = 0ull;
+            if (pres && s < s_end) {
+                const double cost = qos[(int64_t)s * 4 + 2], qual = qos[(int64_t)s * 4 + 3];
+                if (lo_c <= cost && cost <= hi_c && lo_q <= qual && qual <= hi_q) key[i] = rank_key(srow[s - n0], (uint32_t)s);
+            }
+        }
+        unsigned long long last = ~0ull;
+        int my_pick = -1;
+        int n_found = 0;
+        for (int r = 0; r < n_per; ++r) {
+            unsigned long long best = 0ull;
+#pragma unroll
+            for (int i = 0; i < SS_PER_LANE; ++i)
+                if (key[i] < last && key[i] > best) best = key[i];
+            best = row16_max_u64(best);
+            if (best == 0ull) break;
+            if (sub == r) my_pick = (int)(0xffffffffu - (uint32_t)(best & 0xffffffffu));
+            last = best;
+            ++n_found;
+        }
+        const int src_lane = (lane & ~15) + (n_found > 0 ? sub % n_found : 0);
+        const int id = __shfl(my_pick, src_lane, 64);
+        if (sub < n_per) {
+            float4 q = make_float4(0.f, 1.f, 1.f, 1.f);
+            if (n_found > 0) {
+                const double* qs = qos + (int64_t)id * 4;
+                q = make_float4((float)qs[0], (float)qs[1], (float)qs[2], (float)qs[3]);
+            }
+            const int64_t pos = b * T * n_per + (int64_t)c * n_per + sub;
+            float4 tail = make_float4(0.f, 0.f, 0.f, 0.f);
+            if (c == 0) {
+                const double* gb = global_bounds + b * 4;
+                tail = make_float4((float)gb[0], (float)gb[1], (float)gb[2], (float)gb[3]);
+            }
+            float4* dst = reinterpret_cast<float4*>(out_rows + pos * 8);
+            dst[0] = q;
+            dst[1] = tail;
+            out_ids[pos] = n_found > 0 ? id : -1;
+        }
+    }
+}
diff --git a/gnnpn-sc_amd/csrc/select.hip b/gnnpn-sc_amd/csrc/select.hip
--- a/gnnpn-sc_amd/csrc/select.hip
+++ b/gnnpn-sc_amd/csrc/select.hip
@@ -1,10 +1,8 @@
 #include <vector>
 
 #include "common.h"
-
-__device__ __forceinline__ unsigned long long rank_key(float score, uint32_t id) {
-    return ((unsigned long long)float_order_key(score) << 32) | (0xffffffffu - id);
-}
+#include "select_shared.h"
+#include "score_select.h"
 
 __global__ __launch_bounds__(256) void select_candidates_kernel(
     const float* __restrict__ scores, int64_t ld_scores, const int32_t* __restrict__ cat_ptr,
@@ -62,29 +60,19 @@
     }
 }
 
-__device__ __forceinline__ unsigned long long row16_max_u64(unsigned long long v) {
-#define GNNPN_MAX_STEP(CTRL)                                                                                       \
-    {                                                                                                              \
-        const unsigned lo = __builtin_amdgcn_update_dpp(0, (int)(unsigned)v, CTRL, 0xF, 0xF, true);                \
-        const unsigned hi = __builtin_amdgcn_update_dpp(0, (int)(unsigned)(v >> 32), CTRL, 0xF, 0xF, true);        \
-        const unsigned long long o = ((unsigned long long)hi << 32) | lo;                                          \
-        v = o > v ? o : v;                                                                                         \
-    }
-    GNNPN_MAX_STEP(0x121) GNNPN_MAX_STEP(0x122) GNNPN_MAX_STEP(0x124) GNNPN_MAX_STEP(0x128)
-    return v;
-}
-__device__ __forceinline__ unsigned long long row8_max_u64(unsigned long long v) {
-    GNNPN_MAX_STEP(0xB1) GNNPN_MAX_STEP(0x4E) GNNPN_MAX_STEP(0x141)
-    return v;
-#undef GNNPN_MAX_STEP
-}
-
 template <int W>
 __global__ __launch_bounds__(256) void select_candidates16_kernel(
     const float* __restrict__ scores, int64_t ld_scores, const int32_t* __restrict__ cat_ptr,
     const double* __restrict__ qos, const double* __restrict__ local_bounds, const uint8_t* __restrict__ present,
     const double* __restrict__ global_bounds, float* __restrict__ out_rows, int32_t* __restrict__ out_ids,
-    int32_t B, int32_t T, int32_t n_per) {
+    int32_t B, int32_t T, int32_t n_per, ScoreTile st) {
+    if constexpr (W == 16) {
+        if (st.A) {
+            extern __shared__ __attribute__((aligned(16))) float score_tile[];
+            score_select_tile(st, score_tile, cat_ptr, qos, local_bounds, present, global_bounds, out_rows, out_ids, B, T, n_per);
+            return;
+        }
+    }
     const int lane = threadIdx.x & 63, sub = lane & (W - 1);
     const int64_t seg = ((int64_t)blockIdx.x * 4 + (threadIdx.x >> 6)) * (64 / W) + lane / W;
     if (seg >= (int64_t)B * T) return;
@@ -174,16 +162,39 @@
     if (n_per <= 8 && ld_scores <= 8ll * T)
         hipLaunchKernelGGL(select_candidates16_kernel<8>, dim3((unsigned)((n_seg + 31) / 32)), dim3(256), 0,
                            (hipStream_t)stream, scores, ld_scores, cat_ptr, qos, local_bounds, present, global_bounds,
-                           out_rows, out_ids, B, T, n_per);
+                           out_rows, out_ids, B, T, n_per, ScoreTile{});
     else if (n_per <= 16)
         hipLaunchKernelGGL(select_candidates16_kernel<16>, dim3((unsigned)((n_seg + 15) / 16)), dim3(256), 0,
                            (hipStream_t)stream, scores, ld_scores, cat_ptr, qos, local_bounds, present, global_bounds,
-                           out_rows, out_ids, B, T, n_per);
+                           out_rows, out_ids, B, T, n_per, ScoreTile{});
     else
         hipLaunchKernelGGL(select_candidates_kernel, dim3((unsigned)((n_seg + 3) / 4)), dim3(256), 0,
                            (hipStream_t)stream, scores, ld_scores, cat_ptr, qos, local_bounds, present, global_bounds,
                            out_rows, out_ids, B, T, n_per);
     GNNPN_CHECK_LAUNCH("select_candidates");
+    return GNNPN_OK;
+}
+
+extern "C" int gnnpn_score_select_tile_cols(void) { return SS_COLS; }
+
+extern "C" int gnnpn_score_select_f32(const float* A, int64_t lda, const float* W, int64_t ldw, float* scores, int64_t ld_scores,
+                                      const int32_t* tile_cat, int32_t n_tiles, const int32_t* cat_ptr, const double* qos,
+                                      const double* local_bounds, const uint8_t* present, const double* global_bounds, float* out_rows,
+                                      int32_t* out_ids, int32_t B, int32_t S, int32_t T, int32_t K, int32_t n_per, void* stream) {
+    GNNPN_REQUIRE(B >= 0 && S > 0 && T > 0 && K > 0 && n_tiles > 0, "score_select: bad shape B=%d S=%d T=%d K=%d tiles=%d", B, S, T, K, n_tiles);
+    GNNPN_REQUIRE(n_per >= 1 && n_per <= 16, "score_select: n_per must be in [1,16], got %d (wider: gnnpn_linear_f32 + gnnpn_select_candidates)", n_per);
+    GNNPN_REQUIRE(lda >= K && ldw >= K && ld_scores >= S, "score_select: leading dimension too small");
+    if (B == 0) return GNNPN_OK;
+    GNNPN_REQUIRE(A && W && scores && tile_cat && cat_ptr && qos && local_bounds && present && global_bounds && out_rows && out_ids,
+                  "score_select: null operand");
+    GNNPN_REQUIRE(gnnpn_aligned(out_rows, 16), "score_select: out_rows must be 16-byte aligned");
+    ScoreTile st = {A, lda, W, ldw, scores, ld_scores, tile_cat, S, K, gnnpn_aligned(A, 4), gnnpn_aligned(W, 4)};
+    const void* func = (const void*)select_candidates16_kernel<16>;
+    const unsigned pad = gnnpn_front_lds_pad(func);
+    dim3 grid((unsigned)n_tiles, (unsigned)((B + SS_BM - 1) / SS_BM));
+    hipLaunchKernelGGL(select_candidates16_kernel<16>, grid, dim3(256), pad > SS_LDS_BYTES ? pad : SS_LDS_BYTES, (hipStream_t)stream, scores,
+                       ld_scores, cat_ptr, qos, local_bounds, present, global_bounds, out_rows, out_ids, B, T, n_per, st);
+    GNNPN_CHECK_LAUNCH("score_select_f32");
     return GNNPN_OK;
 }
 
diff --git a/gnnpn-sc_amd/csrc/select_shared.h b/gnnpn-sc_amd/csrc/select_shared.h
--- /dev/null
+++ b/gnnpn-sc_amd/csrc/select_shared.h
@@ -0,0 +1,23 @@
+#pragma once
+#include "common.h"
+
+__device__ __forceinline__ unsigned long long rank_key(float score, uint32_t id) {
+    return ((unsigned long long)float_order_key(score) << 32) | (0xffffffffu - id);
+}
+
+__device__ __forceinline__ unsigned long long row16_max_u64(unsigned long long v) {
+#define GNNPN_MAX_STEP(CTRL)                                                                                       \
+    {                                                                                                              \
+        const unsigned lo = __builtin_amdgcn_update_dpp(0, (int)(unsigned)v, CTRL, 0xF, 0xF, true);                \
+        const unsigned hi = __builtin_amdgcn_update_dpp(0, (int)(unsigned)(v >> 32), CTRL, 0xF, 0xF, true);        \
+        const unsigned long long o = ((unsigned long long)hi << 32) | lo;                                          \
+        v = o > v ? o : v;                                                                                         \
+    }
+    GNNPN_MAX_STEP(0x121) GNNPN_MAX_STEP(0x122) GNNPN_MAX_STEP(0x124) GNNPN_MAX_STEP(0x128)
+    return v;
+}
+__device__ __forceinline__ unsigned long long row8_max_u64(unsigned long long v) {
+    GNNPN_MAX_STEP(0xB1) GNNPN_MAX_STEP(0x4E) GNNPN_MAX_STEP(0x141)
+    return v;
+#undef GNNPN_MAX_STEP
+}
diff --git a/gnnpn-sc_amd/csrc/torch_ops.cpp b/gnnpn-sc_amd/csrc/torch_ops.cpp
--- a/gnnpn-sc_amd/csrc/torch_ops.cpp
+++ b/gnnpn-sc_amd/csrc/torch_ops.cpp
@@ -205,6 +205,32 @@
     return {rows, ids};
 }
 
+std::tuple<Tensor, Tensor, Tensor> score_select(const Tensor& a, const Tensor& weight, const OptTensor& tile_cat, const Tensor& cat_ptr,
+                                                const Tensor& qos, const Tensor& local_bounds, const Tensor& present,
+                                                const Tensor& global_bounds, int64_t n_per) {
+    if (!(tile_cat.has_value() && tile_cat->defined()) || n_per > 16) {
+        Tensor scores = linear(a, weight, std::nullopt, std::nullopt, std::nullopt, GNNPN_ACT_SIGMOID);
+        auto [rows, ids] = segment_topk_feasible(scores, cat_ptr, qos, local_bounds, present, global_bounds, n_per);
+        return {scores, rows, ids};
+    }
+    GNNPN_ON_DEVICE_OF(a);
+    rows2d(a, "score_select.a"), rows2d(weight, "score_select.weight");
+    const int64_t B = a.size(0), K = a.size(1), S = weight.size(0), T = cat_ptr.numel() - 1, n_tiles = tile_cat->numel() - 1;
+    TORCH_CHECK(weight.size(1) == K, "score_select: K mismatch ", a.sizes(), " x ", weight.sizes());
+    TORCH_CHECK(T >= 1 && n_tiles >= 1, "score_select: empty cat_ptr or tile plan");
+    TORCH_CHECK(qos.sizes() == at::IntArrayRef({S, 4}) && local_bounds.sizes() == at::IntArrayRef({B, T, 4}) &&
+                    present.sizes() == at::IntArrayRef({B, T}) && global_bounds.sizes() == at::IntArrayRef({B, 4}),
+                "score_select: inconsistent shapes");
+    Tensor scores = new_f32(a, {B, S}), rows = new_f32(a, {B, T * n_per, 8}), ids = new_i32(a, {B, T * n_per});
+    check_rc(gnnpn_score_select_f32(f32(a, "a"), K, f32(weight, "weight"), K, out_f32(scores), S, i32(*tile_cat, "tile_cat"), (int32_t)n_tiles,
+                                    i32(cat_ptr, "cat_ptr"), cptr<double>(qos, at::kDouble, "qos"),
+                                    cptr<double>(local_bounds, at::kDouble, "local_bounds"), cptr<uint8_t>(present, at::kByte, "present"),
+                                    cptr<double>(global_bounds, at::kDouble, "global_bounds"), out_f32(rows),
+                                    static_cast<int32_t*>(ids.data_ptr()), (int32_t)B, (int32_t)S, (int32_t)T, (int32_t)K, (int32_t)n_per,
+                                    cur_stream()), "gnnpn_score_select_f32");
+    return {scores, rows, ids};
+}
+
 Tensor rank_rows(const Tensor& scores) {
     GNNPN_ON_DEVICE_OF(scores);
     rows2d(scores, "rank_rows.scores");
@@ -243,6 +269,20 @@
     Tensor R = new_f32(actions, {B});
     check_rc(gnnpn_qos_reward_f32(f32(actions, "actions"), out_f32(R), (int32_t)B, (int32_t)T, (int)level, cur_stream()), "gnnpn_qos_reward_f32");
     return R;
+}
+
+std::tuple<Tensor, Tensor, Tensor> two_level_tail(const Tensor& win_low, const Tensor& idx_low, const Tensor& win_high, const Tensor& idx_high,
+                                                  const Tensor& actions, int64_t level) {
+    GNNPN_ON_DEVICE_OF(actions);
+    TORCH_CHECK(win_low.dim() == 3 && win_high.sizes() == win_low.sizes(), "two_level_tail: win_low / win_high must be [B, T, n_per]");
+    const int64_t B = win_low.size(0), T = win_low.size(1), K = win_low.size(2);
+    TORCH_CHECK(idx_low.sizes() == at::IntArrayRef({B, T}) && idx_high.sizes() == at::IntArrayRef({B, T}) &&
+                    actions.sizes() == at::IntArrayRef({B, T, 8}), "two_level_tail: inconsistent shapes");
+    Tensor pl = new_f32(actions, {B, T}), ph = new_f32(actions, {B, T}), R = new_f32(actions, {B});
+    check_rc(gnnpn_two_level_tail_f32(f32(win_low, "win_low"), i32(idx_low, "idx_low"), out_f32(pl), f32(win_high, "win_high"),
+                                      i32(idx_high, "idx_high"), out_f32(ph), f32(actions, "actions"), out_f32(R), (int32_t)B, (int32_t)T,
+                                      (int32_t)K, (int)level, cur_stream()), "gnnpn_two_level_tail_f32");
+    return {pl, ph, R};
 }
 
 int precision_code(const std::string& p, const char* what) {
@@ -319,7 +359,7 @@
 std::vector<Tensor> pointer_decode(const c10::List<OptTensor>& net_tensors, at::IntArrayRef latent_from, const Tensor& inputs, int64_t n_cat,
                                    int64_t n_per, double tanh_c, bool use_tanh, bool want_queries, std::string precision, int64_t impl,
                                    int64_t lds_kb, bool write_through, const OptTensor& workspace, const OptTensor& status,
-                                   at::IntArrayRef sample_seeds, bool paired_start) {
+                                   at::IntArrayRef sample_seeds, bool paired_start, bool want_pick_prob) {
     GNNPN_ON_DEVICE_OF(inputs);
     constexpr size_t NK = 16;
     const size_t n_nets = latent_from.size();
@@ -364,9 +404,9 @@
         const int64_t seed = i < sample_seeds.size() ? sample_seeds[i] : -1;
         a.sample = seed >= 0 ? 1 : 0;
         a.sample_seed = seed >= 0 ? (uint64_t)seed : 0;
-        Tensor idx = new_i32(inputs, {B, n_cat}), win = new_f32(inputs, {B, n_cat, n_per}), prob = new_f32(inputs, {B, n_cat});
+        Tensor idx = new_i32(inputs, {B, n_cat}), win = new_f32(inputs, {B, n_cat, n_per}), prob = new_f32(inputs, {want_pick_prob ? B : 0, n_cat});
         Tensor actions = new_f32(inputs, {B, n_cat, 8}), q = want_queries ? new_f32(inputs, {B, n_cat, H}) : new_f32(inputs, {0});
-        a.idx = static_cast<int32_t*>(idx.data_ptr()), a.win_logits = out_f32(win), a.pick_prob = out_f32(prob), a.actions = out_f32(actions);
+        a.idx = static_cast<int32_t*>(idx.data_ptr()), a.win_logits = out_f32(win), a.pick_prob = want_pick_prob ? out_f32(prob) : nullptr, a.actions = out_f32(actions);
         a.queries = want_queries ? out_f32(q) : nullptr;
         out.push_back(idx), out.push_back(win), out.push_back(prob), out.push_back(actions), out.push_back(q);
     }
@@ -401,6 +441,9 @@
           "Tensor w2, Tensor i2, Tensor? b2, Tensor? a2, Tensor? s2, Tensor? w3=None, Tensor? i3=None, Tensor? b3=None) -> Tensor");
     m.def("segment_topk_feasible(Tensor scores, Tensor cat_ptr, Tensor qos, Tensor local_bounds, Tensor present, Tensor global_bounds, "
           "int n_per) -> (Tensor, Tensor)");
+    m.def("score_select(Tensor a, Tensor weight, Tensor? tile_cat, Tensor cat_ptr, Tensor qos, Tensor local_bounds, Tensor present, "
+          "Tensor global_bounds, int n_per) -> (Tensor, Tensor, Tensor)");
+    m.def("two_level_tail(Tensor win_low, Tensor idx_low, Tensor win_high, Tensor idx_high, Tensor actions, int level) -> (Tensor, Tensor, Tensor)");
     m.def("rank_rows(Tensor scores) -> Tensor");
     m.def("precision_at_k(Tensor ranking, Tensor labels, int[] ks) -> Tensor");
     m.def("attention_logits(Tensor enc_out, Tensor queries, int step, Tensor idx, float tanh_c, bool use_tanh) -> Tensor");
@@ -409,7 +452,7 @@
           "Tensor? workspace=None, Tensor? status=None, bool paired_start=False) -> Tensor[]");
     m.def("pointer_decode(Tensor?[] net_tensors, int[] latent_from, Tensor inputs, int n_cat, int n_per, float tanh_c=10.0, "
           "bool use_tanh=True, bool want_queries=False, str precision='f32', int impl=0, int lds_kb=0, bool write_through=False, "
-          "Tensor? workspace=None, Tensor? status=None, int[] sample_seeds=[], bool paired_start=False) -> Tensor[]");
+          "Tensor? workspace=None, Tensor? status=None, int[] sample_seeds=[], bool paired_start=False, bool want_pick_prob=True) -> Tensor[]");
 }
 
 TORCH_LIBRARY_IMPL(gnnpn, CUDA, m) {
@@ -424,6 +467,8 @@
     m.impl("gin_layer", gin_layer);
     m.impl("gin_layer_split", gin_layer_split);
     m.impl("segment_topk_feasible", segment_topk_feasible);
+    m.impl("score_select", score_select);
+    m.impl("two_level_tail", two_level_tail);
     m.impl("rank_rows", rank_rows);
     m.impl("precision_at_k", precision_at_k);
     m.impl("attention_logits", attention_logits);
diff --git a/gnnpn-sc_amd/custom_ops.py b/gnnpn-sc_amd/custom_ops.py
--- a/gnnpn-sc_amd/custom_ops.py
+++ b/gnnpn-sc_amd/custom_ops.py
@@ -58,7 +58,7 @@
 
 @_gnnpn_errors
 def pointer_decode(nets, inputs, n_cat, n_per, tanh_c=10.0, use_tanh=True, want_queries=False, precision="f32", impl=0,
-                   lds_kb=0, write_through=False, ws=None, paired_start=False):
+                   lds_kb=0, write_through=False, ws=None, paired_start=False, pick_prob=True):
     flat = [d.get(k) for d in nets for k in DECODE_KEYS]
     lf = [int(d.get("latent_from", -1)) for d in nets]
     seeds = [int(d["sample_seed"]) & 0x7FFFFFFFFFFFFFFF if d.get("sample") else -1 for d in nets]
@@ -67,7 +67,7 @@
     out = torch.ops.gnnpn.pointer_decode(flat, lf, inputs, n_cat, n_per, float(tanh_c), bool(use_tanh), bool(want_queries),
                                          precision, impl, lds_kb, bool(write_through),
                                          None if wsp is None else wsp.decode(B, n_cat, n_per), None if wsp is None else wsp.status,
-                                         seeds, bool(paired_start))
+                                         seeds, bool(paired_start), bool(pick_prob))
     if wsp is not None:
         wsp.note_launch(1, _lib.load().gnnpn_last_launch_units())
     m = len(DECODE_OUTS)
@@ -76,6 +76,8 @@
         d = dict(zip(DECODE_OUTS, out[i * m:(i + 1) * m]))
         if d["queries"].numel() == 0 and not want_queries:
             d["queries"] = None
+        if not pick_prob:
+            d["pick_prob"] = None
         res.append(d)
     return res
 
diff --git a/gnnpn-sc_amd/modelML.py b/gnnpn-sc_amd/modelML.py
--- a/gnnpn-sc_amd/modelML.py
+++ b/gnnpn-sc_amd/modelML.py
@@ -216,13 +216,16 @@
 
     @torch.no_grad()
     def scores(self, x, wf_csr, seg_ptr, x_service, svc_csr, service_emb=None, max_nodes=0, dense_precision=None):
+        xr, xs = self.score_operands(x, wf_csr, seg_ptr, x_service, svc_csr, service_emb, max_nodes, dense_precision)
+        return torch.ops.gnnpn.linear(xr, xs, act=ACT_SIGMOID)
+
+    @torch.no_grad()
+    def score_operands(self, x, wf_csr, seg_ptr, x_service, svc_csr, service_emb=None, max_nodes=0, dense_precision=None):
         if service_emb is not None:
-            xr = self.request_embedding(x, wf_csr, seg_ptr, max_nodes, dense_precision)
-            return torch.ops.gnnpn.linear(xr, service_emb, act=ACT_SIGMOID)
+            return self.request_embedding(x, wf_csr, seg_ptr, max_nodes, dense_precision), service_emb
         if not self.parallel_branches:
             xr = self.request_embedding(x, wf_csr, seg_ptr, max_nodes, dense_precision)
-            xs = self.service_embedding(x_service, svc_csr)
-            return torch.ops.gnnpn.linear(xr, xs, act=ACT_SIGMOID)
+            return xr, self.service_embedding(x_service, svc_csr)
         cur = torch.cuda.current_stream(x.device)
         side = self._side_streams.get(x.device)
         if side is None:
@@ -233,7 +236,7 @@
         xr = self.request_embedding(x, wf_csr, seg_ptr, max_nodes, dense_precision)
         cur.wait_stream(side)
         xs.record_stream(cur)
-        return torch.ops.gnnpn.linear(xr, xs, act=ACT_SIGMOID)
+        return xr, xs
 
     def forward(self, data):
         if self.training:
diff --git a/gnnpn-sc_amd/modelPN.py b/gnnpn-sc_amd/modelPN.py
--- a/gnnpn-sc_amd/modelPN.py
+++ b/gnnpn-sc_amd/modelPN.py
@@ -8,6 +8,7 @@
 from . import custom_ops, ops
 
 FOLD_INPUT_PROJECTION = True
+FUSE_DECODE_TAIL = True
 
 qosandcons = 8
 qosNum = 4
@@ -342,13 +343,21 @@
     enc, h_n, c_n = custom_ops.lstm_encode([enc_l, enc_h], precision=precision, lds_kb=lds_kb, write_through=write_through, ws=ws,
                                            paired_start=paired_start)
     del enc_l, enc_h
-    dl, dh = custom_ops.pointer_decode([la.decode_args(emb_l, enc[0], h_n[0], c_n[0], fold=fold),
-                                 ha.decode_args(emb_h, enc[1], h_n[1], c_n[1], latent_from=0, fold=fold,
-                                                sample_seed=sample_high_seed)],
-                                inputs, la.serCategory, la.serNumber, la.C, la.use_tanh,
-                                precision="split" if precision == "split" else "f32", impl=decode_impl, lds_kb=lds_kb,
-                                write_through=write_through, ws=ws, paired_start=paired_start)
-    R = torch.ops.gnnpn.qos_reward(dh["actions"], 0 if high.level == "Low" else 1)
+    nets = [la.decode_args(emb_l, enc[0], h_n[0], c_n[0], fold=fold),
+            ha.decode_args(emb_h, enc[1], h_n[1], c_n[1], latent_from=0, fold=fold, sample_seed=sample_high_seed)]
+    fuse_tail = FUSE_DECODE_TAIL and sample_high_seed is None and ops.coop_supported(la.hidden_size, la.serNumber, decode_impl) and \
+        all(n.get("xw_fold") is not None for n in nets) and \
+        torch.cuda.get_device_properties(inputs.device).multi_processor_count >= 256
+    dl, dh = custom_ops.pointer_decode(nets, inputs, la.serCategory, la.serNumber, la.C, la.use_tanh,
+                                       precision="split" if precision == "split" else "f32", impl=decode_impl, lds_kb=lds_kb,
+                                       write_through=write_through, ws=ws, paired_start=paired_start,
+                                       **({"pick_prob": False} if fuse_tail else {}))
+    level = 0 if high.level == "Low" else 1
+    if fuse_tail:
+        dl["pick_prob"], dh["pick_prob"], R = torch.ops.gnnpn.two_level_tail(dl["win_logits"], dl["idx"], dh["win_logits"], dh["idx"],
+                                                                             dh["actions"], level)
+    else:
+        R = torch.ops.gnnpn.qos_reward(dh["actions"], level)
     return ({"idx_low": dl["idx"], "idx_high": dh["idx"], "R": R, "actions": dh["actions"],
              "action_probs": dh["pick_prob"], "win_low": dl["win_logits"], "win_high_raw": dh["win_logits"]},
             (enc[1], h_n[1], c_n[1], emb_h))
diff --git a/gnnpn-sc_amd/ops.py b/gnnpn-sc_amd/ops.py
--- a/gnnpn-sc_amd/ops.py
+++ b/gnnpn-sc_amd/ops.py
@@ -291,6 +291,21 @@
         dev_ptr(lin_w_packed, F32, "lin_w_packed"), dev_ptr(lin_b, F32, "lin_b"), dev_ptr(out, F32, "out"), stream_ptr()),
         "gnnpn_request_branch_f32")
     return out
+
+
+def score_select_plan(cat_ptr, n_services):
+    import numpy as np
+    cp = np.asarray(cat_ptr, dtype=np.int64).reshape(-1)
+    width = int(_lib.load().gnnpn_score_select_tile_cols())
+    if cp.size < 2 or cp[0] != 0 or cp[-1] != int(n_services) or (np.diff(cp) < 0).any() or (np.diff(cp) > width).any():
+        return None
+    tiles, first = [0], 0
+    for c in range(cp.size - 1):
+        if cp[c + 1] - cp[first] > width:
+            tiles.append(c)
+            first = c
+    tiles.append(cp.size - 1)
+    return np.asarray(tiles, dtype=np.int32)
 
 
 def select_candidates(scores, cat_ptr, qos, local_bounds, present, global_bounds, n_per):
diff --git a/gnnpn-sc_amd/pipeline.py b/gnnpn-sc_amd/pipeline.py
--- a/gnnpn-sc_amd/pipeline.py
+++ b/gnnpn-sc_amd/pipeline.py
@@ -16,15 +16,25 @@
     cat_ptr: torch.Tensor
     qos: torch.Tensor
     emb_cache: tuple = None
+    select_plan: tuple = None
 
     @staticmethod
     def from_table(table, device):
         ei = torch.from_numpy(np.ascontiguousarray(table.edge_index))
         ea = torch.from_numpy(np.ascontiguousarray(table.edge_attr))
         csr = graph.gcn_csr(ei, ea, table.n_services).to(device)
-        return DeviceServices(torch.from_numpy(table.x_service).to(device), csr,
-                              torch.from_numpy(np.ascontiguousarray(table.cat_ptr)).to(device),
-                              torch.from_numpy(np.ascontiguousarray(table.qos)).to(device))
+        svc = DeviceServices(torch.from_numpy(table.x_service).to(device), csr,
+                             torch.from_numpy(np.ascontiguousarray(table.cat_ptr)).to(device),
+                             torch.from_numpy(np.ascontiguousarray(table.qos)).to(device))
+        svc.score_select_plan(table.cat_ptr)
+        return svc
+
+    def score_select_plan(self, host_cat_ptr=None):
+        if self.select_plan is None:
+            cp = self.cat_ptr.cpu().numpy() if host_cat_ptr is None else host_cat_ptr
+            plan = ops.score_select_plan(cp, self.qos.shape[0])
+            self.select_plan = (None if plan is None else torch.from_numpy(plan).to(self.cat_ptr.device),)
+        return self.select_plan[0]
 
 
 @dataclass
@@ -126,6 +136,7 @@
         self.net, self.low, self.high, self.n_per = net, low, high, n_per
         self.precision = default_precision(low, high) if precision is None else precision
         self.cache_service_embedding = True
+        self.fuse_score_select = True
         self._side_streams = {}
         warn_partitioned_device(next(low.parameters()).device, self.precision)
 
@@ -144,14 +155,24 @@
                                max_nodes=batch.max_nodes, dense_precision="split" if self.precision == "split" else "f32")
 
     @torch.no_grad()
+    def scores_and_candidates(self, services, batch):
+        if not self.fuse_score_select:
+            scores = self.scores(services, batch)
+            return (scores, *self.candidates(services, batch, scores))
+        xr, xs = self.net.score_operands(batch.x, batch.wf_csr, batch.seg_ptr, services.x_service, services.csr,
+                                         service_emb=self.service_embedding(services) if self.cache_service_embedding else None,
+                                         max_nodes=batch.max_nodes, dense_precision="split" if self.precision == "split" else "f32")
+        return torch.ops.gnnpn.score_select(xr, xs, services.score_select_plan(), services.cat_ptr, services.qos, batch.local_bounds,
+                                            batch.present, batch.global_bounds, self.n_per)
+
+    @torch.no_grad()
     def candidates(self, services, batch, scores):
         return torch.ops.gnnpn.segment_topk_feasible(scores, services.cat_ptr, services.qos, batch.local_bounds,
                                                      batch.present, batch.global_bounds, self.n_per)
 
     @torch.no_grad()
     def run(self, services, batch, decode_impl=0, lds_kb=0, ws=None, paired_start=False, write_through=False):
-        scores = self.scores(services, batch)
-        rows, ids = self.candidates(services, batch, scores)
+        scores, rows, ids = self.scores_and_candidates(services, batch)
         if isinstance(ws, (tuple, list)):
             B = rows.shape[0]
             half = half_batch_split(B)
@@ -186,8 +207,7 @@
 
     @torch.no_grad()
     def best_of(self, services, batch, samples, seed=None, decode_impl=0, lds_kb=0, ws=None, write_through=False):
-        scores = self.scores(services, batch)
-        rows, ids = self.candidates(services, batch, scores)
+        scores, rows, ids = self.scores_and_candidates(services, batch)
         out = two_level_best_of(self.low, self.high, rows, samples, seed=seed, precision=self.precision, decode_impl=decode_impl,
                                 lds_kb=lds_kb, write_through=write_through, ws=ws)
         out.update(scores=scores, pn_inputs=rows, candidate_ids=ids)
diff --git a/include/gnnpn_hip.h b/include/gnnpn_hip.h
--- a/include/gnnpn_hip.h
+++ b/include/gnnpn_hip.h
@@ -104,6 +104,13 @@
                             const double* qos, const double* local_bounds,
                             const uint8_t* present, const double* global_bounds, float* out_rows,
                             int32_t* out_ids, int32_t B, int32_t T, int32_t n_per, void* stream);
+
+int gnnpn_score_select_tile_cols(void);
+int gnnpn_score_select_f32(const float* A, int64_t lda, const float* W, int64_t ldw, float* scores, int64_t ld_scores,
+                           const int32_t* tile_cat, int32_t n_tiles, const int32_t* cat_ptr, const double* qos,
+                           const double* local_bounds, const uint8_t* present, const double* global_bounds,
+                           float* out_rows, int32_t* out_ids, int32_t B, int32_t S, int32_t T, int32_t K,
+                           int32_t n_per, void* stream);
 
 int gnnpn_rank_rows(const float* scores, int64_t ld_scores, int32_t* ranking, int32_t B, int32_t S,
                     void* stream);
@@ -237,6 +244,10 @@
 
 int gnnpn_qos_reward_f32(const float* actions, float* R, int32_t B, int32_t T, int level,
                          void* stream);
+
+int gnnpn_two_level_tail_f32(const float* win_low, const int32_t* idx_low, float* pick_prob_low, const float* win_high,
+                             const int32_t* idx_high, float* pick_prob_high, const float* actions, float* R, int32_t B,
+                             int32_t T, int32_t n_per, int level, void* stream);
 
 typedef struct {
     const float* embedded;
```

After: 470,200. -1.3%, worse.
